# GregoryFaust/yaha

Hardware: AMD Instinct MI355X
Metric: aligned reads/s (whole node), 1 000 bp reads, OQC mode hot path (higher is better)
Workload: dtype int16

## Files before the change

yaha_amd/csrc/device/abi.hip:

```cpp
#include "ctx.h"
#include <memory>

std::atomic<int> gCtxPerDevice[64];
std::mutex gRowsMu[64];
hipEvent_t gRowsEv[64][4];
bool gRowsEvValid[64][4];
unsigned long long gRowsSeq[64];
std::atomic<int> gActiveRuns[64];
const char *const kStageNames[T_N] = {"seed_lookup", "hit_sort", "fragments_regions", "chain", "align_dp", "layout", "align_p1_gapfill", "ext_rows", "ext_trace",
                                      "align_p3_score_split", "ext_rows_device_clock", "ext_rows_packed16"};
thread_local const ygpu_ctx *tlsPfFailed = nullptr;

int runTo(ygpu_ctx *ctx, int stage)
{
    int rc;
    HIPCHK(hipSetDevice(ctx->device));
    if (ctx->stageDone < 1) {
        rc = stageSeed(ctx); if (rc) return rc;
        EV0(T_FRAGS); rc = buildFrags(ctx);
        if (rc == YD_RESORT) { rc = stageSeed(ctx); if (rc) return rc; EV0(T_FRAGS); rc = buildFrags(ctx);
            if (rc == YD_RESORT) { ctx->err = "hit sort: the sorted keys are not in ascending order"; rc = YGPU_EINTERNAL; } }
        if (rc) return rc;
        if (!ctx->nFrags) EV1(T_FRAGS);
        ctx->stageDone = 1;
    }
    if (stage >= 2 && ctx->stageDone < 2) { if (ctx->nFrags) { rc = stageChain(ctx); if (rc) return rc; } ctx->stageDone = 2; }
    if (stage >= 3 && ctx->stageDone < 3) { rc = stageAlign(ctx); if (rc) return rc; ctx->stageDone = 3; }
    uint32_t scanFail = 0; rc = fetchU32(ctx, ctx->counters.as<uint32_t>() + CNT_SCANFAIL, &scanFail); if (rc) return rc;
    if (scanFail) { if (ctx->scanState.p) HIPCHK(hipMemsetAsync(ctx->scanState.p, 0, ctx->scanState.cap, ctx->stream));
        ctx->err = "exclusive sum: a tile was not published within 30 s (look-back gave up)"; return YGPU_EINTERNAL; }
    return 0;
}
static int initCommon(ygpu_ctx *ctx, int device)
{
    const bool phases = getenv("YGPU_INIT_PHASES") != nullptr; double tPh = nowMs();
    auto phase = [&](const char *what) { if (phases) { const double t = nowMs(); fprintf(stderr, "[ygpu] ctx %p: %-20s %8.1f ms\n", (void *)ctx, what, t - tPh); tPh = t; } };
    HIPCHK(hipSetDevice(device));
    HIPCHK(hipStreamCreate(&ctx->stream)); HIPCHK(hipStreamCreate(&ctx->stream2));
    phase("two streams");
    for (int i = 0; i < YD_MAX_CHUNK_EV; i++) HIPCHK(hipEventCreateWithFlags(&ctx->evChunk[i], hipEventDisableTiming));
    HIPCHK(hipEventCreateWithFlags(&ctx->evTail, hipEventDisableTiming));
    if (const char *e = getenv("YGPU_LANE_CHUNKS")) ctx->laneChunks = atoi(e);
    if (const char *e = getenv("YGPU_TRACE_BUDGET_BLOCKS")) ctx->traceBudgetBlocks = atoll(e);
    ctx->segSortMax = ydSegSortMax();
    if (const char *e = getenv("YGPU_SEGSORT_MAX")) { long v = atol(e); if (v >= 1 && v <= (long)ydSegSortMax()) ctx->segSortMax = (uint32_t)v; }
    if (const char *e = getenv("YGPU_SPLIT_LANES")) ctx->splitLanes = atoi(e);
    if (const char *e = getenv("YGPU_ROWS2_PER_CU")) ctx->rows2PerCU = atoi(e);
    if (const char *e = getenv("YGPU_ALIGN_WAVES")) ctx->alignWavesPerCU = atoi(e);
    gCtxPerDevice[device & 63]++; ctx->counted = true;
    { int cu = 0; if (hipDeviceGetAttribute(&cu, hipDeviceAttributeMultiprocessorCount, device) != hipSuccess) { cu = 0; (void)hipGetLastError(); } ctx->nCU = cu > 0 ? cu : 256; }
    phase("device attribute");
    for (int t = 0; t < T_N; t++) { HIPCHK(hipEventCreate(&ctx->ev[t][0])); HIPCHK(hipEventCreate(&ctx->ev[t][1])); ctx->names[t] = kStageNames[t]; }
    if (hipEventCreateWithFlags(&ctx->evSync, hipEventBlockingSync | hipEventDisableTiming) != hipSuccess) { ctx->evSync = nullptr; (void)hipGetLastError(); }
    phase("events");
    if (hipHostMalloc((void **)&ctx->pinned, 256, hipHostMallocDefault) != hipSuccess) { ctx->pinned = nullptr; (void)hipGetLastError(); }
    ctx->pf.stream = ctx->stream2; ctx->pf.device = device;
    if (hipHostMalloc((void **)&ctx->pf.pinned, 256, hipHostMallocDefault) != hipSuccess) { ctx->pf.pinned = nullptr; (void)hipGetLastError(); }
    if (hipEventCreateWithFlags(&ctx->pf.evSync, hipEventBlockingSync | hipEventDisableTiming) != hipSuccess) { ctx->pf.evSync = nullptr; (void)hipGetLastError(); }
    HIPCHK(hipEventCreateWithFlags(&ctx->evSnap, hipEventDisableTiming));
    if (hipHostMalloc((void **)&ctx->snapCtr, sizeof(DevCounters), hipHostMallocDefault) != hipSuccess) { ctx->snapCtr = nullptr; (void)hipGetLastError(); }
    if (ctx->pf.counters.ensure(4 * CNT_N)) { ctx->err = "hipMalloc failed"; return YGPU_ENOMEM; }
    HIPCHK(hipMemsetAsync(ctx->pf.counters.p, 0, 4 * CNT_N, ctx->stream2));
    phase("pinned words");
    return 0;
}


namespace {
struct ImagePiece { size_t part; size_t off, bytes; };
struct ImagePlan {
    const char *src[3]; size_t bytes[3]; std::vector<ImagePiece> pieces;
    void build(const ygpu_index_view *ix, size_t pieceBytes)
    {
        const uint64_t HT = 1ull << (2 * ix->wordLen);
        src[0] = (const char *)ix->bases; bytes[0] = (size_t)ix->n_base_bytes; src[1] = (const char *)ix->startingOffs; bytes[1] = (size_t)(4 * (HT + 1));
            src[2] = (const char *)ix->ROA; bytes[2] = (size_t)(4ull * ix->totalMatches);
        for (size_t part = 0; part < 3; part++) for (size_t o = 0; o < bytes[part]; o += pieceBytes) pieces.push_back({part, o, std::min(pieceBytes, bytes[part] - o)});
    }
};
struct ImageState {
    std::unique_ptr<std::atomic<int>[]> done; std::atomic<int> failed{0}; char *dst[3] = {nullptr, nullptr, nullptr};
};

static void uploadFromHost(int device, const ImagePlan &plan, ImageState &me, int nt, bool staged)
{
    std::atomic<size_t> next(0);
    auto work = [&]() {
        if (hipSetDevice(device) != hipSuccess) { me.failed = 1; return; }
        hipStream_t st; if (hipStreamCreate(&st) != hipSuccess) { me.failed = 1; return; }
        char *buf[2] = {nullptr, nullptr}; hipEvent_t ev[2] = {nullptr, nullptr}; bool used[2] = {false, false}; size_t pend[2] = {0, 0}; size_t maxPiece = 0;
            for (auto &q : plan.pieces) maxPiece = std::max(maxPiece, q.bytes);
        if (staged) for (int k = 0; k < 2; k++) {
            if (hipHostMalloc((void **)&buf[k], maxPiece, hipHostMallocDefault) != hipSuccess) { buf[k] = nullptr; me.failed = 1; }
            if (hipEventCreateWithFlags(&ev[k], hipEventDisableTiming) != hipSuccess) { ev[k] = nullptr; me.failed = 1; }
        }
        for (int k = 0; !me.failed; k ^= 1) {
            const size_t i = next.fetch_add(1); if (i >= plan.pieces.size()) break;
            if (me.done[i].load(std::memory_order_acquire)) continue;
            const ImagePiece &q = plan.pieces[i]; char *d = me.dst[q.part] + q.off; const char *sp = plan.src[q.part] + q.off;
// ... 161 lines not shown
    std::vector<int> srcIndex(n, -1); const bool peer = !(getenv("YGPU_PEER_COPY") && atoi(getenv("YGPU_PEER_COPY")) == 0);
    for (int k = 1; k < n && peer; k++) {
        int can = devices[k] == devices[k - 1] ? 1 : 0;
        if (!can && hipDeviceCanAccessPeer(&can, devices[k], devices[k - 1]) != hipSuccess) { can = 0; (void)hipGetLastError(); }
        if (can && devices[k] != devices[k - 1]) { if (hipSetDevice(devices[k]) == hipSuccess) { const hipError_t e = hipDeviceEnablePeerAccess(devices[k - 1], 0);
            if (e != hipSuccess && e != hipErrorPeerAccessAlreadyEnabled) can = 0; } else can = 0; (void)hipGetLastError(); }
        if (can) srcIndex[k] = k - 1;
    }
    if (getenv("YGPU_INIT_PHASES")) { fprintf(stderr, "[ygpu] init: image sources:");
        for (int k = 0; k < n; k++) { if (srcIndex[k] < 0) fprintf(stderr, " device %d <- host;", devices[k]);
        else fprintf(stderr, " device %d <- device %d;", devices[k], devices[srcIndex[k]]); } fprintf(stderr, " %zu pieces\n", plan.pieces.size()); }
    std::vector<std::thread> th;
    for (int k = 1; k < n; k++) th.emplace_back([&, k]() { rcs[k] = initDevice(out[k], devices[k], srcIndex[k], srcIndex[k] >= 0 ? devices[srcIndex[k]] : -1, ix, plan,
        states.data(), k, ready.get(), all + k * cpd + 1, cpd - 1); });
    rcs[0] = initDevice(out[0], devices[0], -1, -1, ix, plan, states.data(), 0, ready.get(), all + 1, cpd - 1);
    for (auto &x : th) x.join();
    int rc = 0; for (int k = 0; k < n; k++) { if (rc_each) rc_each[k] = rcs[k]; if (rcs[k] && !rc) rc = rcs[k];
        if (rcs[k]) for (int j = 1; j < cpd; j++) if (all[k * cpd + j]->err.empty()) all[k * cpd + j]->err = "the device's first context failed: " + out[k]->err; }
    return rc;
}

int ygpu_device_count(void) { int n = 0; if (hipGetDeviceCount(&n) != hipSuccess) { (void)hipGetLastError(); return 0; } return n; }

int ygpu_init(int device, const ygpu_index_view *ix, const ygpu_params *p, ygpu_ctx **out)
{
    if (!out) return YGPU_EINVAL;
    return ygpu_init_multi(&device, 1, 1, ix, p, out, nullptr);
}

int ygpu_clone(const ygpu_ctx *parent, ygpu_ctx **out)
{
    *out = nullptr;
    if (!parent || !parent->stream) return YGPU_EINVAL;
    ygpu_ctx *ctx = new ygpu_ctx; *out = ctx; ctx->device = parent->device;
    int rc = initCommon(ctx, parent->device); if (rc) return rc;
    shareImage(ctx, parent);
    ENSURE(ctx->counters, 4 * CNT_N); ENSURE(ctx->ctr, sizeof(DevCounters)); ENSURE(ctx->errFlag, 64);
    HIPCHK(hipMemsetAsync(ctx->counters.p, 0, 4 * CNT_N, ctx->stream));
    HIPCHK(streamSync(ctx));
    return 0;
}

}
std::vector<DevBuf *> allBuffers(ygpu_ctx *ctx)
{
    DevBuf *all[] = {&ctx->dBases, &ctx->dSO, &ctx->dROA, &ctx->dLow, &ctx->dFwd, &ctx->dRev, &ctx->dFwd4, &ctx->dRev4, &ctx->dReadOff, &ctx->dKmerOff, &ctx->posS, &ctx->posC,
        &ctx->posRsI, &ctx->hitOff, &ctx->expandStart, &ctx->keysA, &ctx->keysB, &ctx->segOff, &ctx->bigB, &ctx->bigE, &ctx->isHead, &ctx->tileState,
                         &ctx->frags, &ctx->regStart, &ctx->multiList, &ctx->smallList, &ctx->bigList, &ctx->regionCount, &ctx->regionBase, &ctx->clumps, &ctx->clumpFrags,
                             &ctx->clumpFrags0, &ctx->order, &ctx->clumpsSorted, &ctx->rootPush, &ctx->rootBase, &ctx->outClumps,
                         &ctx->outClumps2, &ctx->outOps, &ctx->outRoot, &ctx->outPush, &ctx->dstIdx, &ctx->readCount, &ctx->readStart, &ctx->counters, &ctx->ctr, &ctx->errFlag,
                             &ctx->scanState, &ctx->bucketWork, &ctx->scratchAlign,
                         &ctx->segLists, &ctx->subB, &ctx->subE, &ctx->subLists, &ctx->subBigB, &ctx->subBigE, &ctx->sub2B, &ctx->sub2E, &ctx->sub2Lists, &ctx->sub3B, &ctx->sub3E,
                             &ctx->sub3Lists, &ctx->kmerParts, &ctx->scratchChain, &ctx->dpProbs, &ctx->dpRes, &ctx->dpOps, &ctx->rootState, &ctx->stateOps, &ctx->extProbs,
                             &ctx->rowsBound, &ctx->stripOff, &ctx->extRes, &ctx->extTrace, &ctx->chunkCnt, &ctx->memoKeys, &ctx->memoCount, &ctx->probs2, &ctx->rowsBound2,
                             &ctx->stripOff2, &ctx->extRes2, &ctx->extTrace2, &ctx->rowsClock, &ctx->splitScratch, &ctx->fallList, &ctx->keys2a, &ctx->keys2b, &ctx->vals2a,
                             &ctx->vals2b, &ctx->extKeys, &ctx->extVals, &ctx->extKeys2, &ctx->extOrder, &ctx->slowList, &ctx->gapScratch, &ctx->jointCount, &ctx->jointBase,
                             &ctx->joints, &ctx->sortKeys, &ctx->sortVals, &ctx->sortKeys2, &ctx->sortVals2, &ctx->gapOps, &ctx->waveChunks, &ctx->extOps, &ctx->traceCnt,
                         &ctx->oqCs, &ctx->oqCl, &ctx->oqOpsIn, &ctx->oqSeeds, &ctx->oqQlen, &ctx->pf.scanState, &ctx->pf.counters, &ctx->oqProf, &ctx->oqLists, &ctx->oqClsCnt,
                             &ctx->oqThr, &ctx->oqSeqStart, &ctx->oqSeqLen, &ctx->oqNeed, &ctx->oqPoolOff, &ctx->oqKeys, &ctx->oqStack, &ctx->oqNodes, &ctx->oqPrim, &ctx->oqPA,
                             &ctx->oqPfx, &ctx->oqPath, &ctx->oqPool, &ctx->oqPush, &ctx->oqOut, &ctx->oqOutCnt, &ctx->oqOutOps, &ctx->oqPrimCnt, &ctx->oqOutStart,
                             &ctx->oqOpsStart, &ctx->oqFClumps, &ctx->oqFOps};
    return std::vector<DevBuf *>(all, all + sizeof all / sizeof all[0]);
}
extern "C" {

void ygpu_destroy(ygpu_ctx *ctx)
{
    if (!ctx) return;
    if (ctx->worker.joinable()) { { std::lock_guard<std::mutex> lk(ctx->aMu); ctx->aQuit = true; } ctx->aCv.notify_all(); ctx->worker.join(); }
    if (ctx->counted) gCtxPerDevice[ctx->device & 63]--;
    if (ctx->stream) {
        hipSetDevice(ctx->device);
        {
            const int dv = ctx->device & 63; std::lock_guard<std::mutex> lk(gRowsMu[dv]);
            (void)hipStreamSynchronize(ctx->stream);
            if (gCtxPerDevice[dv].load() <= 0) for (int k = 0; k < 4; k++) if (gRowsEvValid[dv][k]) { (void)hipEventDestroy(gRowsEv[dv][k]); gRowsEvValid[dv][k] = false; }
        }
        if (ctx->sharedIndex) { ctx->dBases.p = nullptr; ctx->dBases.cap = 0; ctx->dSO.p = nullptr; ctx->dSO.cap = 0; ctx->dROA.p = nullptr; ctx->dROA.cap = 0;
            ctx->dLow.p = nullptr; ctx->dLow.cap = 0; }
        const std::vector<DevBuf *> all = allBuffers(ctx);
        for (auto b : all) b->release();
        for (int t = 0; t < T_N; t++) { hipEventDestroy(ctx->ev[t][0]); hipEventDestroy(ctx->ev[t][1]); }
        if (ctx->evSync) hipEventDestroy(ctx->evSync);
        if (ctx->pinned) hipHostFree(ctx->pinned);
        if (ctx->pf.pinned) hipHostFree(ctx->pf.pinned);
        if (ctx->snapCtr) hipHostFree(ctx->snapCtr);
        if (ctx->pf.evSync) hipEventDestroy(ctx->pf.evSync);
        if (ctx->evSnap) hipEventDestroy(ctx->evSnap);
        for (int i = 0; i < YD_MAX_CHUNK_EV; i++) hipEventDestroy(ctx->evChunk[i]);
        hipEventDestroy(ctx->evTail); hipStreamDestroy(ctx->stream2);
        hipStreamDestroy(ctx->stream);
    }
    delete ctx;
}
int ygpu_memory(ygpu_ctx *ctx, uint64_t *free_bytes, uint64_t *total_bytes, uint64_t *ctx_bytes)
{
    if (!ctx || !ctx->stream) return YGPU_EINVAL;
    HIPCHK(hipSetDevice(ctx->device));
    size_t fb = 0, tb = 0; HIPCHK(hipMemGetInfo(&fb, &tb));
    uint64_t mine = 0; for (DevBuf *b : allBuffers(ctx)) if (b->p && !(ctx->sharedIndex && (b == &ctx->dBases || b == &ctx->dSO || b == &ctx->dROA
        || b == &ctx->dLow))) mine += b->cap;
    if (free_bytes) *free_bytes = fb; if (total_bytes) *total_bytes = tb; if (ctx_bytes) *ctx_bytes = mine;
    return 0;
}
int ygpu_park(ygpu_ctx *ctx)
{
    if (!ctx || !ctx->stream) return YGPU_EINVAL;
    HIPCHK(hipSetDevice(ctx->device)); HIPCHK(streamSync(ctx));
    for (DevBuf *b : allBuffers(ctx)) if (b != &ctx->dBases && b != &ctx->dSO && b != &ctx->dROA && b != &ctx->dLow) b->release();
    if (ctx->counted) { gCtxPerDevice[ctx->device & 63]--; ctx->counted = false; }
    ctx->stageDone = 0; ctx->parked = true;
    return 0;
}
int ygpu_get_arena_profile(ygpu_ctx *ctx, ygpu_arena_profile *out)
{
    if (!ctx || !ctx->stream || !out) return YGPU_EINVAL;
    memset(out, 0, sizeof *out);
    const std::vector<DevBuf *> all = allBuffers(ctx);
    if (all.size() > sizeof out->cap / sizeof out->cap[0]) { ctx->err = "arena profile: more buffers than the profile holds"; return YGPU_EINTERNAL; }
    out->n = (uint32_t)all.size();
    for (size_t k = 0; k < all.size(); k++) { DevBuf *b = all[k];
        out->cap[k] = (b == &ctx->dBases || b == &ctx->dSO || b == &ctx->dROA || b == &ctx->dLow) ? 0ull : (uint64_t)b->cap; }
    out->trace_ratio = ctx->traceRatio; out->ops_ratio = ctx->opsRatio; out->last_clump_slots = ctx->lastClumpSlots; out->last_fall = ctx->lastFall; out->bases = ctx->totalBases;
    return 0;
}
int ygpu_presize(ygpu_ctx *ctx, const ygpu_arena_profile *prof)
{
    if (!ctx || !ctx->stream || !prof) return YGPU_EINVAL;
    if (ctx->parked) { ctx->err = "the context was parked (ygpu_park)"; return YGPU_EINVAL; }
    HIPCHK(hipSetDevice(ctx->device));
    const std::vector<DevBuf *> all = allBuffers(ctx);
    if (prof->n != all.size()) { ctx->err = "arena profile of another build"; return YGPU_EINVAL; }
    for (size_t k = 0; k < all.size(); k++) {
        DevBuf *b = all[k];
        if (b == &ctx->dBases || b == &ctx->dSO || b == &ctx->dROA || b == &ctx->dLow || b == &ctx->counters || b == &ctx->ctr || b == &ctx->errFlag
            || b == &ctx->pf.counters) continue;
        if (prof->cap[k] > b->cap && b->ensureExact((size_t)prof->cap[k])) { (void)hipGetLastError(); ctx->err = "hipMalloc failed while presizing the arenas"; return YGPU_ENOMEM;
            }
    }
    if (ctx->scanState.p) HIPCHK(hipMemsetAsync(ctx->scanState.p, 0, ctx->scanState.cap, ctx->stream));
    if (ctx->bucketWork.p) HIPCHK(hipMemsetAsync(ctx->bucketWork.p, 0, ctx->bucketWork.cap, ctx->stream));
    if (ctx->pf.scanState.p) HIPCHK(hipMemsetAsync(ctx->pf.scanState.p, 0, ctx->pf.scanState.cap, ctx->stream));
    if (ctx->runsDone == 0) { ctx->traceRatio = prof->trace_ratio; ctx->opsRatio = prof->ops_ratio > 0 ? prof->ops_ratio : ctx->opsRatio;
        ctx->lastClumpSlots = prof->last_clump_slots; ctx->lastFall = (long long)prof->last_fall; }
    HIPCHK(streamSync(ctx));
    return 0;
}
const char *ygpu_last_error(const ygpu_ctx *ctx) { return !ctx ? "null context" : (tlsPfFailed == ctx && !ctx->pf.err.empty()) ? ctx->pf.err.c_str() : ctx->err.c_str(); }

}
extern "C" {

int ygpu_run(ygpu_ctx *ctx)
{
    if (!ctx || !ctx->stream) return YGPU_EINVAL;
    ctx->stageDone = 0; const double t0 = nowMs(); ctx->statAttempts = 0; ctx->statRanges = 0;
    struct Active { int d; explicit Active(int dv) : d(dv) { gActiveRuns[d]++; } ~Active() { gActiveRuns[d]--; } } active(ctx->device & 63);
    int rc = runTo(ctx, 3);
    if (kStats) { size_t fb = 0, tb = 0; hipMemGetInfo(&fb, &tb);
        fprintf(stderr, "[ygpu] ctx %p run: %u reads, rc %d, %.1f ms; align attempts %d, ranges %d, trace arena %.2f GB (ratio %.3f), free %.1f GB\n", (void *)ctx, ctx->nReads, rc,
        nowMs() - t0, ctx->statAttempts, ctx->statRanges, ctx->extTrace.cap / 1e9, ctx->traceRatio, fb / 1e9); }
    if (rc) { (void)hipStreamSynchronize(ctx->stream); (void)hipGetLastError(); return rc; }
    if (ydCheckStateOn()) {
        if (getenv("YGPU_CHECK_STATE_INJECT") && ctx->scanState.p) (void)hipMemsetAsync((char *)ctx->scanState.p + 8, 0x01, 4, ctx->stream);
        const DevBuf *const bufs[2] = {&ctx->scanState, &ctx->bucketWork}; static const char *const names[2] = {"the sums' look-back state", "the orderings' bucket counters"};
        rc = ydCheckZero(ctx->stream, ctx->err, (unsigned int *)ctx->errFlag.p + 2, bufs, names, 2, "after ygpu_run");
        if (rc) { if (ctx->scanState.p) (void)hipMemsetAsync(ctx->scanState.p, 0, ctx->scanState.cap, ctx->stream); return rc; }
    }
    ctx->runsDone++;
    ctx->totalMs = 0;
    for (int t = 0; t < T_N; t++) {
        float m = 0; ctx->ms[t] = (ctx->evUsed[t] && hipEventElapsedTime(&m, ctx->ev[t][0], ctx->ev[t][1]) == hipSuccess) ? m : 0;
        if (t == T_XROWS_DEV) ctx->ms[t] = (ctx->evUsed[T_XROWS] && ctx->hRowsClock[1] > ctx->hRowsClock[0] && ctx->hRowsClock[0] != ~0ull)
            ? (float)((double)(ctx->hRowsClock[1] - ctx->hRowsClock[0]) / 1.0e5) : 0;
        if (t == T_XROWS_PK) ctx->ms[t] = ctx->rowsPacked ? 1.0f : 0.0f;
        if (t < T_TOP) ctx->totalMs += ctx->ms[t];
    }
    return 0;
}
void *ygpu_host_alloc(size_t bytes)
{
    void *p = nullptr;
    if (hipHostMalloc(&p, bytes ? bytes : 1, hipHostMallocDefault) != hipSuccess) { (void)hipGetLastError(); return nullptr; }
    return p;
}
void ygpu_host_free(void *p) { if (p) (void)hipHostFree(p); }
static void asyncWorker(ygpu_ctx *ctx)
{
    std::unique_lock<std::mutex> lk(ctx->aMu);
    for (;;) {
        ctx->aCv.wait(lk, [&] { return ctx->aQuit || (ctx->aOpen && !ctx->aDone && ctx->aBatch); });
        if (ctx->aQuit) return;
        const ygpu_read_batch *b = ctx->aBatch; ctx->aBatch = nullptr;
        lk.unlock();
        int rc = ygpu_upload(ctx, b); if (rc == 0) rc = ygpu_run(ctx); if (rc == 0) rc = ygpu_collect(ctx, &ctx->aOut);
        lk.lock();
        ctx->aRc = rc; ctx->aDone = true; ctx->aCv.notify_all();
    }
}
int ygpu_submit(ygpu_ctx *ctx, const ygpu_read_batch *batch, ygpu_ticket *ticket)
{
    if (!ctx || !ctx->stream || !batch || !ticket) return YGPU_EINVAL;
    std::unique_lock<std::mutex> lk(ctx->aMu);
    if (ctx->aOpen) return YGPU_EBUSY;
    if (!ctx->worker.joinable()) ctx->worker = std::thread(asyncWorker, ctx);
    ctx->aBatch = batch; ctx->aOpen = true; ctx->aDone = false; ctx->aRc = 0; *ticket = ++ctx->aTicket;
    ctx->aCv.notify_all();
    return 0;
}
int ygpu_poll(ygpu_ctx *ctx, ygpu_ticket ticket)
{
    if (!ctx) return YGPU_EINVAL;
    std::lock_guard<std::mutex> lk(ctx->aMu);
    if (!ctx->aOpen || ticket != ctx->aTicket) return YGPU_EINVAL;
    return ctx->aDone ? 1 : 0;
}
int ygpu_wait(ygpu_ctx *ctx, ygpu_ticket ticket, ygpu_result_batch *out)
{
    if (!ctx || !out) return YGPU_EINVAL;
    std::unique_lock<std::mutex> lk(ctx->aMu);
    if (!ctx->aOpen || ctx->aWaiting || ticket != ctx->aTicket) return YGPU_EINVAL;
    ctx->aWaiting = true;
    ctx->aCv.wait(lk, [&] { return ctx->aDone; });
    ctx->aOpen = false; ctx->aWaiting = false; *out = ctx->aOut;
    return ctx->aRc;
}

int ygpu_last_timing(ygpu_ctx *ctx, float *total_ms, int *n_stages, const char *const **names, const float **ms)
// ... 49 lines not shown
```

yaha_amd/csrc/device/ctx.h:

```cpp
#pragma once
#include <hip/hip_runtime.h>
#include <string>
#include <vector>
#include <cstring>
#include <cstdio>
#include <cstdlib>
#include <algorithm>
#include <array>
#include <atomic>
#include <chrono>
#include <thread>
#include <mutex>
#include <condition_variable>
#include <memory>
#include "common.h"
#include "../oqc_core.h"

#define HIPCHK(call) do { hipError_t e_ = (call); \
    if (e_ != hipSuccess) { ctx->err = std::string(#call) + ": " + hipGetErrorString(e_); return YGPU_ENODEV; } } while (0)

#define KL(kern, grid, block, shmem, st, ...) do { hipLaunchKernelGGL(kern, grid, block, shmem, st, __VA_ARGS__); hipError_t e_ = hipGetLastError(); \
    if (e_ != hipSuccess) { ctx->err = std::string("launch of " #kern " failed: ") + hipGetErrorString(e_); return YGPU_ENODEV; } } while (0)

#define YD_MAX_CHUNK_EV 16

struct DevBuf {
    void *p = nullptr;
    size_t cap = 0;
    int ensure(size_t bytes, bool keep = false, hipStream_t st = 0)
    {
        if (bytes <= cap) return 0;
        size_t ncap = bytes + bytes / 4 + 256; void *np = nullptr;
        if (hipMalloc(&np, ncap) != hipSuccess) return -1;
        if (keep && p && cap) { hipMemcpyAsync(np, p, cap, hipMemcpyDeviceToDevice, st); hipStreamSynchronize(st); }
        if (p) hipFree(p);
        p = np; cap = ncap; return 0;
    }
    void release() { if (p) hipFree(p); p = nullptr; cap = 0; }
    int ensureExact(size_t bytes)
    {
        if (bytes <= cap) return 0;
        release();
        void *np = nullptr;
        if (hipMalloc(&np, bytes) != hipSuccess) return -1;
        p = np; cap = bytes; return 0;
    }
    template <class T> T *as() const { return (T *)p; }
};

enum {
    CNT_NMULTI = 0, CNT_MAXN, CNT_CLUMPS, CNT_CFRAGS, CNT_QCHAIN, CNT_QALIGN, CNT_OUTCLUMPS, CNT_OUTOPS, CNT_QDP, CNT_DPOPS, CNT_NBIG, CNT_QBIG,
    CNT_STATEOPS, CNT_EXTOPS, CNT_QEXT, CNT_SLOW, CNT_NDP, CNT_NDP16, CNT_GAPOPS, CNT_PAD_EVEN, CNT_NMULTI2 ,
        CNT_NTINY, CNT_NSMALL, CNT_NMID, CNT_NB12, CNT_NB16,
        CNT_NB24,
    CNT_SEGC,
    CNT_NFRAGS = CNT_SEGC + 16,
    CNT_NREG = CNT_NFRAGS + 3,
    CNT_SCANFAIL = CNT_NREG + 2,
    CNT_N = CNT_NREG + 4
};
enum { T_SEED = 0, T_SORT, T_FRAGS, T_CHAIN, T_ALIGN, T_LAYOUT, T_TOP, T_P1 = T_TOP, T_XROWS, T_XTRACE, T_P3, T_XROWS_DEV, T_XROWS_PK, T_N };

extern std::atomic<int> gCtxPerDevice[64];
extern std::mutex gRowsMu[64];
extern hipEvent_t gRowsEv[64][4];
extern bool gRowsEvValid[64][4];
extern unsigned long long gRowsSeq[64];
extern std::atomic<int> gActiveRuns[64];
extern const char *const kStageNames[T_N];

struct PfSide {
    std::string err;
    hipStream_t stream = nullptr;
    uint32_t *pinned = nullptr;
    hipEvent_t evSync = nullptr;
    DevBuf scanState, counters;
    int device = 0;
};

struct DepthImage {
    int device = 0;
    DevBuf cov, stats, seqStart, seqLength, binBase;
    uint64_t nBins = 0;
    uint32_t bin = 0, minMapq = 0;
    std::vector<uint32_t> hSeqStart, hSeqLength;
    ~DepthImage() { (void)hipSetDevice(device); cov.release(); stats.release(); seqStart.release(); seqLength.release(); binBase.release(); }
};

struct EventsImage {
    int device = 0;
    DevBuf ev, stats, seqStart, seqLength, binBase;
    uint64_t nBins = 0;
    uint32_t bin = 0, minMapq = 0, minClip = 0;
    std::vector<uint32_t> hSeqStart, hSeqLength;
    ~EventsImage() { (void)hipSetDevice(device); ev.release(); stats.release(); seqStart.release(); seqLength.release(); binBase.release(); }
};

struct ygpu_ctx {
    int device = 0;
    hipStream_t stream = nullptr;
    DevParams P{};
    std::string err;
    int nCU = 256;
    DevBuf dBases, dSO, dROA, dLow;
    bool sharedIndex = false;
    uint32_t nReads = 0;
    int maxQ = 0;
    uint64_t totalBases = 0;
    uint32_t nKmers = 0;
    std::vector<uint32_t> hReadOff, hKmerOff;
    DevBuf dFwd, dRev, dFwd4, dRev4, dReadOff, dKmerOff;
    DevBuf bigB, bigE;
    DevBuf posS, posC, posRsI, hitOff, expandStart, keysA, keysB, segOff, isHead, tileState, frags;
    DevBuf segLists, subB, subE, subLists, subBigB, subBigE, sub2B, sub2E, sub2Lists, sub3B, sub3E, sub3Lists, kmerParts;
    DevBuf regStart, multiList, smallList, bigList, regionCount, regionBase;
    DevBuf clumps, clumpFrags, clumpFrags0, order, clumpsSorted, scratchChain;
    DevBuf rootPush, rootBase, outClumps, outClumps2, outOps, outRoot, outPush, dstIdx, readCount, readStart;
    DevBuf scratchAlign, dpProbs, dpRes, dpOps;
    DevBuf rootState, stateOps, extProbs, rowsBound, stripOff, extRes, extTrace, chunkCnt;
    DevBuf memoKeys, memoCount, probs2, rowsBound2, stripOff2, extRes2, extTrace2, splitScratch, fallList;
    DevBuf keys2a, keys2b, vals2a, vals2b, extKeys, extVals, extKeys2, extOrder, slowList;
    DevBuf gapScratch, jointCount, jointBase, joints, sortKeys, sortVals, sortKeys2, sortVals2, gapOps;
    DevBuf waveChunks, extOps, traceCnt, rowsClock;
    DevBuf counters, ctr, errFlag, scanState, bucketWork;
    bool evUsed[16] = {false};
    double traceT = 0;
    hipStream_t stream2 = nullptr;
    hipEvent_t evChunk[YD_MAX_CHUNK_EV], evTail;
    bool counted = false;
    bool parked = false;
    long long traceBudgetBlocks = 0;
    uint32_t lastClumpSlots = 0;
    bool keepAllFrags = false;
    unsigned long long hRowsClock[2] = {0, 0};
    int laneChunks = 0;
    uint32_t segSortMax = 0;
    int splitLanes = 1;
    int rows2PerCU = 0;
    int alignWavesPerCU = 0;
    int laneExt = 1;
    std::vector<unsigned long long> hStripOff;
    int runsDone = 0;
    double traceRatio = 0.0, opsRatio = 0.03;
    int statRanges = 0, statAttempts = 0;
    double statT0 = 0;
    DevBuf oqProf, oqLists, oqClsCnt, oqThr, oqSeqStart, oqSeqLen, oqNeed, oqPoolOff, oqKeys, oqStack, oqNodes, oqPrim, oqPA, oqPfx, oqPath, oqPool;
    DevBuf oqPush, oqOut, oqOutCnt, oqOutOps, oqPrimCnt, oqOutStart, oqOpsStart, oqFClumps, oqFOps;
    bool oqSet = false, oqDone = false;
    yoqc::Params oqP{};
    yoqc::Seqs oqG{};
    uint32_t nFOut = 0, nFOps = 0;
    PfSide pf;
    std::atomic<bool> pfSnap{false};
    hipEvent_t evSnap = nullptr;
    uint32_t snapN = 0, snapC = 0, snapOps = 0, pfN = 0;
    unsigned long long runGen = 0, snapGen = 0, filtGen = 0;
    ygpu_counters pfCounters{};
    DevCounters *snapCtr = nullptr;
    DevCounters snapCtrPlain{};
    unsigned long long snapHits = 0, snapFrags = 0, snapRegions = 0;
    DevBuf oqCs, oqCl, oqOpsIn, oqSeeds, oqQlen;
    std::shared_ptr<DepthImage> depth;
    std::shared_ptr<EventsImage> events;
    uint32_t hOutCounts[2] = {0, 0}, hOutEf = 0;
    bool hOutValid = false;
    uint32_t nHits = 0, nFrags = 0, nRegions = 0, nMulti = 0, nTiny = 0, nSmall = 0, nMid = 0, nBig = 0, maxN = 0;
    int sortRankUsed = 0;
    bool sortRankForced = false;
    uint32_t nClumpSlots = 0, nClumps = 0, nClumpFrags = 0, nOut = 0, nOutOps = 0;
    int stageDone = 0;
    std::vector<uint32_t> hClumpStart, hOps, hClumpFragStart, hClumpRS, hDpOps;
    std::vector<ygpu_clump> hClumps;
// ... 99 lines not shown
```

yaha_amd/csrc/device/ext_lanes.h:

```cpp
#pragma once
#include "align.h"

#define YD_REFILL_MIN 4
#define YD_LW 21
#define YD_LWORST (-(1 << 28))
#define YD_CHUNK_FLUSHES 16
#define YD_LANE_DWORDS (YD_CHUNK_FLUSHES * 32)
#define YD_CHUNK_DWORDS (64 * YD_LANE_DWORDS)
#define YD_LDS_STRIDE 33

typedef uint32_t yd_u32x4 __attribute__((ext_vector_type(4)));
struct ExtProb { uint32_t qBase, rOff; uint16_t qOff, qLen; uint32_t flags; };
enum { XP_STRAND = 1, XP_REV = 2, XP_VALID = 4 };
struct ExtRes { int score, maxi, maxj; uint32_t opsOff, nOps, where, rows, cells; };
static_assert(sizeof(ExtProb) == 16 && sizeof(ExtRes) == 32, "k_ext_rows_pk moves these as 16-byte vectors (non-temporal loads / stores)");
__device__ __forceinline__ const uint32_t *extOpsPtr(const uint32_t *traceBase, const ExtRes &r) {
    return traceBase + (long long)(((unsigned long long)r.where << 32) | (unsigned long long)r.opsOff); }

struct ExtArgs {
    DevParams P; const uint8_t *bases; const uint8_t *fwd, *rev;
    const uint8_t *fwd4, *rev4;
    const ExtProb *probs; uint32_t nProb;
    const uint32_t *order;
    unsigned long long *clock;
    uint32_t *trace; uint32_t nChunks;
    unsigned int *chunkCount;
    uint32_t *waveChunks; uint32_t maxCh;
    uint32_t *ops; unsigned int *opsCount; uint32_t opsCap;
    ExtRes *res; unsigned int *queue; DevCounters *ctr;
    int *errFlag; int dbgMode;
};
enum { YERR_TRACEMEM = 9 };

template <bool CAPS, bool SECOND>
__global__ void __launch_bounds__(256) __attribute__((amdgpu_waves_per_eu(CAPS ? 2 : 3, CAPS ? 2 : 3))) k_ext_rows(ExtArgs A)
{
    __shared__ uint32_t sBlk[256 * YD_LDS_STRIDE];
    if (!SECOND && A.clock && threadIdx.x == 0) atomicMin(&A.clock[0], (unsigned long long)wall_clock64());
    const int lane = laneId();
    const int GO = A.P.GO, GE = A.P.GE, GOE = A.P.GO + A.P.GE, XC = A.P.X, maxIntron = A.P.maxIntron, maxGap = A.P.maxGap;
    const int MSG = A.P.MS + GOE, RCG = GOE - A.P.RC, LWG = YD_LWORST - GOE;
    constexpr int bandwidth = YD_LBAND, leftR = YD_LBAND;
    const uint32_t maxROff = A.P.maxROff;
    YD_GLOBAL const uint8_t *gBases = toGlobal(A.bases);
    const unsigned long long lanesBelow = (1ull << lane) - 1ull;
    const unsigned wave = blockIdx.x * 4u + (threadIdx.x >> 6);
    uint32_t *const myBlk = &sBlk[threadIdx.x * YD_LDS_STRIDE];

    int PV[YD_LW], PF[YD_LW], PI[YD_LW];
    uint32_t w0 = 0, w1 = 0, w2 = 0;
    int p = -1, i = 0, qLen = 0, rLen = 0, maxScore = YD_LWORST, maxi = 0, maxj = 0, qStep = 0, qcNext = 0;
    uint32_t rOff = 0; bool rev = false, done = false;
    YD_GLOBAL const uint8_t *q = toGlobal(A.fwd);
    unsigned calls = 0, rows = 0, cells = 0;
#pragma unroll
    for (int j = 0; j < YD_LW; j++) { PV[j] = LWG; PF[j] = YD_LWORST; PI[j] = 0; }

    int poolCount = 0, poolNext = 0; bool exhausted = false;
    uint32_t eLens = 0, eROff = 0, eQ = 0, eMisc = 0, eW1 = 0, eW2 = 0, ePidx = 0;
    bool pendFlush = false; int pendRes = -1; unsigned pStart = 0;
    auto storeResult = [&]() {
        const unsigned m = i < leftR ? (unsigned)i : (unsigned)leftR, nCells = (unsigned)YD_LW * (unsigned)i - ((unsigned)(leftR + 1) * m - m * (m + 1u) / 2u);
        rows += (unsigned)i; cells += nCells;
        ExtRes r; r.score = maxScore > 0 ? maxScore : 0; r.maxi = maxi; r.maxj = maxj; r.opsOff = pStart >> 4; r.nOps = 0;
        r.where = (pStart & 15u) | ((uint32_t)lane << 4) | (wave << 10); r.rows = (unsigned)i; r.cells = nCells;
        A.res[pendRes] = r; pendRes = -1; i = 0;
    };
    int wslot = 0; unsigned flush = 0; bool dirty = false, justDone = false;
    YD_GLOBAL uint32_t *chunkPtr = toGlobal(A.trace); bool noMem = false;
    auto takeChunk = [&]() {
        unsigned c = 0;
        if (lane == 0) c = atomicAdd(A.chunkCount, 1u);
        c = uniU(c);
        const unsigned ci = flush / YD_CHUNK_FLUSHES;
        if (c >= A.nChunks || ci >= A.maxCh) { noMem = true; c = 0; if (lane == 0) atomicCAS(A.errFlag, 0, (int)YERR_TRACEMEM); }
        if (lane == 0 && ci < A.maxCh) A.waveChunks[(size_t)wave * A.maxCh + ci] = c;
        chunkPtr = toGlobal(A.trace) + (size_t)c * YD_CHUNK_DWORDS;
    };
    takeChunk();
    auto flushBlocks = [&]() {
        const unsigned long long f = __ballot(pendFlush);
        pendFlush = false;
// ... 126 lines not shown
        if (rv > maxScore) { maxScore = rv; maxi = i; maxj = rj; }
        const uint32_t nb = nbOdd == 2u ? 15u : (nbOdd ? (nbByte & 15u) : (nbByte >> 4));
        w0 = (w0 >> 4) | (w1 << 28); w1 = (w1 >> 4) | (w2 << 28); w2 = (w2 >> 4) | (nb << 16);
        const bool fin = busy && (rv < maxScore - XC || i >= qLen);
        if (busy) dirty = true;
        if (wslot == 9) { pendFlush = dirty; dirty = false; wslot = 0; } else wslot++;
        justDone = fin;
        if (fin) { pendRes = p; p = -1; qStep = 0; rLen = 0; qLen = 0; }
    }
    if (wslot != 0 && dirty) pendFlush = true;
    if (!noMem && __ballot(pendFlush) != 0ull) { flushBlocks(); nextFlush(); }
    if (pendRes >= 0) storeResult();
    if (!SECOND && A.clock && lane == 0) atomicMax(&A.clock[1], (unsigned long long)wall_clock64());
    unsigned c0 = (unsigned)waveSumI((int)calls), c1 = (unsigned)waveSumI((int)rows);
    unsigned long long cc = cells;
#pragma unroll
    for (int d = 32; d >= 1; d >>= 1) { cc += (unsigned long long)__shfl_xor((long long)cc, d, 64); }
    if (lane == 0 && !SECOND && A.ctr) {
        unsigned long long *c = A.ctr->v;
        atomicAdd(&c[C_EXT_CALLS], (unsigned long long)c0); atomicAdd(&c[C_EXT_ROWS], (unsigned long long)c1); atomicAdd(&c[C_EXT_CELLS], cc);
        atomicAdd(&c[C_TOUCHED], (unsigned long long)c1 + (unsigned long long)c0 * (unsigned long long)(4 * A.P.bandWidth + 1));
    }
}

struct ExtRowBits { uint32_t a, b, c; };
__device__ __forceinline__ uint32_t extNib(const ExtRowBits &r, int x) { const uint32_t w = x < 8 ? r.a : (x < 16 ? r.b : r.c); return (w >> ((x & 7) * 4)) & 15u; }

__device__ unsigned int gTraceDbg[8];
struct ExtStrip {
    YD_GLOBAL uint32_t *arena; YD_GLOBAL const uint32_t *tab; unsigned f0, laneOff; int cIdx; YD_GLOBAL uint32_t *cBase; int limit; bool wild;
    __device__ __forceinline__ YD_GLOBAL uint32_t *at(int d)
    {
        if ((unsigned)d >= (unsigned)limit) { wild = true; d = 0; }
        const unsigned f = f0 + (unsigned)(d >> 5); const int ci = (int)(f / YD_CHUNK_FLUSHES);
        if (ci != cIdx) { cIdx = ci; cBase = arena + (size_t)tab[ci] * YD_CHUNK_DWORDS + laneOff; }
        return cBase + (f % YD_CHUNK_FLUSHES) * 32u + (unsigned)(d & 31);
    }
};

__device__ __forceinline__ int extRowWord(int y) { return ((y - 1) / 10) * 32 + ((y - 1) % 10) * 3; }
#define YD_TRACE_DEPTH 8
__global__ void __launch_bounds__(256) k_ext_trace(ExtArgs A)
{
    YD_HIGH_PRIO();
    const uint32_t t = blockIdx.x * blockDim.x + threadIdx.x; const int lane = laneId();
    if (*toGlobal(A.errFlag) != 0) return;
    const bool live = t < A.nProb;
    const uint32_t p = live ? ((A.order && !(A.dbgMode & 2)) ? A.order[t] : t) : 0u;
    ExtRes r; r.score = 0; r.nOps = 0;
    if (live) r = A.res[p];
    const bool walk = live && r.score > 0;
    constexpr int leftR = YD_LBAND;
    int n = 0; bool bad = false; int E = 0;
    ExtStrip S; S.arena = toGlobal(A.trace); S.cIdx = -1; S.cBase = S.arena; S.f0 = 0; S.laneOff = 0; S.tab = toGlobal(A.waveChunks); S.limit = 0; S.wild = false;
    if (walk) {
        const int ph = (int)(r.where & 15u);
        S.f0 = r.opsOff; S.laneOff = ((r.where >> 4) & 63u) * YD_LANE_DWORDS; S.tab = toGlobal(A.waveChunks) + (size_t)(r.where >> 10) * A.maxCh;
        E = extRowWord(r.maxi + 1 + ph) + 3; S.limit = E;
        int y = r.maxi, x = r.maxj, prev = -1, acc = 0;
        struct Cur { YD_GLOBAL uint32_t *cp; int rr, w; unsigned fb; };
        Cur c; c.rr = (y - 1 + ph) % 10; c.w = ((y - 1 + ph) / 10) * 32 + c.rr * 3; c.fb = S.f0 + (unsigned)((y - 1 + ph) / 10); c.cp = S.at(c.w);
        auto stepUp = [&](Cur &u) {
            if (u.rr != 0) { u.rr--; u.w -= 3; u.cp -= 3; return; }
            u.rr = 9; u.w -= 5; u.fb--;
            if (u.fb % YD_CHUNK_FLUSHES == YD_CHUNK_FLUSHES - 1u) u.cp = S.arena + (size_t)S.tab[u.fb / YD_CHUNK_FLUSHES] * YD_CHUNK_DWORDS + S.laneOff + (YD_CHUNK_FLUSHES - 1u) *
                32u + 27u;
            else u.cp -= 5;
        };
        const int row0w = extRowWord(1 + ph) - 3;
        auto flush = [&]() { const int wp = E - 1 - n; if (wp < c.w + 3) bad = true; else *S.at(wp) = opMake(prev, acc); n++; };
        auto put = [&](int code, int len) { if (prev != code) { if (prev >= 0) flush(); prev = code; acc = len; } else acc += len; };
        for (int guard = 0; guard < 70000 && y > 0 && x >= 0 && x < YD_LW; guard++) {
            const int ws = x >> 3, sh = (x & 7) * 4;
            uint32_t d[YD_TRACE_DEPTH];
            int lim = (int)(c.fb % YD_CHUNK_FLUSHES) * 10 + c.rr + 1; lim = lim < y ? lim : y; lim = lim < YD_TRACE_DEPTH ? lim : YD_TRACE_DEPTH;
            { YD_GLOBAL uint32_t *up = c.cp; int ur = c.rr;
#pragma unroll
              for (int k = 0; k < YD_TRACE_DEPTH; k++) { d[k] = up[ws]; const bool go = k + 1 < lim; const int dec = ur == 0 ? 5 : 3; up -= go ? dec : 0;
                  ur = go ? (ur == 0 ? 9 : ur - 1) : ur; } }
            uint32_t nib = (d[0] >> sh) & 15u; int took = 0;
#pragma unroll
            for (int k = 0; k < YD_TRACE_DEPTH; k++) {
                if (k >= lim) break;
                nib = (d[k] >> sh) & 15u;
                const int op = (int)(nib & 3u);
                if (op >= OP_D || y <= 0) break;
                if (prev != op) { if (prev >= 0) flush(); prev = op; acc = 1; } else acc++;
                y--; took++;
                if (took < lim) { const int dec = c.rr == 0 ? 5 : 3; c.cp -= dec; c.w -= dec; c.fb -= c.rr == 0 ? 1u : 0u; c.rr = c.rr == 0 ? 9 : c.rr - 1; }
            }
            if (took == lim) { if (y > 0) stepUp(c); else c.w = row0w; continue; }
            if ((nib & 3u) == (uint32_t)OP_D) {
                ExtRowBits rb; rb.a = c.cp[0]; rb.b = c.cp[1]; rb.c = c.cp[2];
                int run = 1, xx = x;
                while (extNib(rb, xx) & 4u) { xx--; if (xx < 0) break; run++; }
                put(OP_D, run); x -= run;
            } else {
                int run = 1, yy = y, xx = x; Cur u = c; uint32_t nb2 = nib;
                while (nb2 & 8u) {
                    yy--; xx++; if (yy <= 0 || xx >= YD_LW) break;
                    run++; stepUp(u);
                    nb2 = (u.cp[xx >> 3] >> ((xx & 7) * 4)) & 15u;
                }
                put(OP_I, run); y -= run; x += run;
                if (y > 0) { for (int k = 0; k < run; k++) stepUp(c); } else c.w = row0w;
            }
        }
        if (y <= 0 && x > leftR) put(OP_D, x - leftR);
        if (prev >= 0) { const int wp = E - 1 - n; if (wp < 0) bad = true; else *S.at(wp) = opMake(prev, acc); n++; }
        if (bad || S.wild) { bad = true; atomicCAS(A.errFlag, 0, (int)YERR_TRACE); n = 0; if (S.wild && atomicCAS(&gTraceDbg[5], 0u, 1u) == 0u) { gTraceDbg[6] = p;
            gTraceDbg[7] = r.where; } }
    }
    if (A.dbgMode & 1) n = 0;
    const bool inPlace = walk && !bad && n > 0 && (S.f0 + (unsigned)((E - n) >> 5)) / YD_CHUNK_FLUSHES == (S.f0 + (unsigned)((E - 1) >> 5)) / YD_CHUNK_FLUSHES;
    const int nCopy = (walk && !bad && !inPlace) ? n : 0;
    int incl = nCopy;
#pragma unroll
    for (int d2 = 1; d2 < 64; d2 <<= 1) { const int v = __shfl_up(incl, d2, 64); if (lane >= d2) incl += v; }
    const int total = __shfl(incl, 63, 64); unsigned ob = 0;
    if (lane == 63 && total) ob = atomicAdd(A.opsCount, (unsigned)total);
    ob = (unsigned)__shfl((int)ob, 63, 64);
    if (walk && !bad) {
        long long place;
        if (inPlace) place = (long long)(S.at(E - n) - S.arena);
        else {
            const unsigned off = ob + (unsigned)(incl - nCopy);
            if ((unsigned long long)off + (unsigned)n > (unsigned long long)A.opsCap) { atomicCAS(A.errFlag, 0, (int)YERR_OUT); return; }
            YD_GLOBAL uint32_t *dst = toGlobal(A.ops) + off;
            for (int k0 = 0; k0 < n; k0 += 8) {
                uint32_t v[8];
#pragma unroll
                for (int j = 0; j < 8; j++) v[j] = (k0 + j < n) ? *S.at(E - n + k0 + j) : 0u;
#pragma unroll
                for (int j = 0; j < 8; j++) if (k0 + j < n) dst[k0 + j] = v[j];
            }
            place = (long long)(dst - S.arena);
        }
        r.opsOff = (uint32_t)(unsigned long long)place; r.where = (uint32_t)((unsigned long long)place >> 32); r.nOps = (uint32_t)n; A.res[p] = r;
    }
}

__global__ void k_trace_keys(const ExtRes *res, const uint32_t *order, uint32_t n, const uint32_t *waveChunks, uint32_t maxCh, int regionLog, int lenShift, int lenBits,
    uint32_t *keys, uint32_t *vals)
{
    YD_HIGH_PRIO();
    const uint32_t t = blockIdx.x * blockDim.x + threadIdx.x;
    if (t >= n) return;
    const uint32_t p = order ? order[t] : t;
    const ExtRes r = res[p];
    const uint32_t top = (1u << lenBits) - 1u;
    const uint32_t len = r.score > 0 ? min((uint32_t)r.maxi >> lenShift, top) : 0u;
    const uint32_t ci = r.opsOff / YD_CHUNK_FLUSHES;
    const uint32_t phys = (regionLog < 20 && r.score > 0 && ci < maxCh) ? waveChunks[(size_t)(r.where >> 10) * maxCh + ci] : 0u;
    keys[t] = (min(phys >> regionLog, 0xFFFFFFu) << lenBits) | (top - len);
    vals[t] = p;
}

__global__ void __launch_bounds__(256) k_trace_volume(const ExtRes *res, uint32_t n, unsigned long long *out)
{
    const uint32_t t = blockIdx.x * blockDim.x + threadIdx.x;
    unsigned long long w = 0, v = 0, np = 0, nw = 0;
    if (t < n) { const ExtRes r = res[t]; if (r.rows) { w = r.rows + 1ull; np = 1; if (r.score > 0) { v = (unsigned long long)r.maxi + 1ull; nw = 1; } } }
#pragma unroll
    for (int d = 32; d >= 1; d >>= 1) {
        w += (unsigned long long)__shfl_xor((long long)w, d, 64); v += (unsigned long long)__shfl_xor((long long)v, d, 64);
        np += (unsigned long long)__shfl_xor((long long)np, d, 64); nw += (unsigned long long)__shfl_xor((long long)nw, d, 64);
    }
    if ((threadIdx.x & 63u) == 0u && np) { atomicAdd(&out[0], w); atomicAdd(&out[1], v); atomicAdd(&out[2], np); atomicAdd(&out[3], nw); }
}

__global__ void k_rebase_u32(uint32_t *v, uint32_t n, uint32_t sub)
{
    YD_HIGH_PRIO();
    const uint32_t i = blockIdx.x * blockDim.x + threadIdx.x;
    if (i < n) v[i] -= sub;
}

__global__ void k_prob_keys(const ExtProb *probs, uint32_t n, uint32_t *keys, uint32_t *vals)
{
    YD_HIGH_PRIO();
    const uint32_t p = blockIdx.x * blockDim.x + threadIdx.x;
    if (p < n) { keys[p] = (probs[p].flags & XP_VALID) ? 0xFFFFu - probs[p].qLen : 0xFFFFu; vals[p] = p; }
}
```

yaha_amd/csrc/device/ext_lanes_pk.h:

```cpp
#pragma once
#include "ext_lanes.h"

typedef short yd_s16x2 __attribute__((ext_vector_type(2)));
#define YD_LW16 (-16000)
#define YD_NP 11
#define YD_RCREAL 0x7FF0u

__device__ __forceinline__ yd_s16x2 pkS(uint32_t v) { return __builtin_bit_cast(yd_s16x2, v); }
__device__ __forceinline__ uint32_t pkU(yd_s16x2 v) { return __builtin_bit_cast(uint32_t, v); }
__device__ __forceinline__ uint32_t pkAdd(uint32_t a, uint32_t b) { return pkU(__builtin_elementwise_add_sat(pkS(a), pkS(b))); }
__device__ __forceinline__ uint32_t pkSub(uint32_t a, uint32_t b) { return pkU(__builtin_elementwise_sub_sat(pkS(a), pkS(b))); }
__device__ __forceinline__ uint32_t pkMax(uint32_t a, uint32_t b) { return pkU(__builtin_elementwise_max(pkS(a), pkS(b))); }
__device__ __forceinline__ uint32_t pkMin(uint32_t a, uint32_t b) { return pkU(__builtin_elementwise_min(pkS(a), pkS(b))); }
__device__ __forceinline__ uint32_t pkMinU(uint32_t a, uint32_t b) { uint32_t d; asm("v_pk_min_u16 %0, %1, %2" : "=v"(d) : "v"(a), "v"(b)); return d; }
__device__ __forceinline__ uint32_t pkMad(uint32_t a, uint32_t b, uint32_t c) { uint32_t d; asm("v_pk_mad_i16 %0, %1, %2, %3" : "=v"(d) : "v"(a), "v"(b), "v"(c)); return d; }
__device__ __forceinline__ uint32_t pkSignMask(uint32_t a) { return pkU(pkS(a) >> (yd_s16x2)(15)); }
__device__ __forceinline__ uint32_t pkSignMaskAsm(uint32_t a, uint32_t c15) { uint32_t d; asm("v_pk_ashrrev_i16 %0, %1, %2" : "=v"(d) : "v"(c15), "v"(a)); return d; }
__device__ __forceinline__ uint32_t bfi(uint32_t mask, uint32_t a, uint32_t b) { return (a & mask) | (b & ~mask); }
__device__ __forceinline__ uint32_t pk2(int v) { return ((uint32_t)v & 0xFFFFu) * 0x10001u; }

#ifndef YD_ROWS_LDSWIN
#define YD_ROWS_LDSWIN 0
#endif
#ifndef YD_ROWS_RESBATCH
// ... 343 lines not shown
        if (fin) { pendRes = p; p = -1; rowsFin = row; }
#ifdef YD_PROF
        if (__ballot(snap) != 0ull) pfSnap++; pfBusy += (unsigned)__builtin_popcountll(__ballot(busy));
#endif
    }
    if (wslot != 0 && dirty) pendFlush = true;
    { const unsigned long long f = __ballot(pendFlush); if (!noMem && f != 0ull) { flushBlocks(f, chunkPtr + (size_t)(flush % YD_CHUNK_FLUSHES) * 32u); nextFlush(); } }
    if (!SECOND && A.clock && lane == 0) atomicMax(&A.clock[1], (unsigned long long)wall_clock64());
    unsigned c0 = calls, c1 = (unsigned)waveSumI((int)rows);
    unsigned long long cc = cells;
#pragma unroll
    for (int d = 32; d >= 1; d >>= 1) { cc += (unsigned long long)__shfl_xor((long long)cc, d, 64); }
#ifdef YD_PROF
    if (lane == 0 && !SECOND) { const unsigned v[7] = {pfPass, pfRes, pfRefill, pfSnap, pfBusy, pfFlush, pfPool};
        for (int k = 0; k < 7; k++) atomicAdd(&gRowsProf[k], (unsigned long long)v[k]); }
#endif
    if (lane == 0 && !SECOND && A.ctr) {
        unsigned long long *c = A.ctr->v;
        atomicAdd(&c[C_EXT_CALLS], (unsigned long long)c0); atomicAdd(&c[C_EXT_ROWS], (unsigned long long)c1); atomicAdd(&c[C_EXT_CELLS], cc);
        atomicAdd(&c[C_TOUCHED], (unsigned long long)c1 + (unsigned long long)c0 * (unsigned long long)(4 * A.P.bandWidth + 1));
    }
}

struct PkRec { uint32_t a, m, ab2, b; };
__device__ __forceinline__ PkRec pkLoadRec(YD_GLOBAL const uint32_t *cp) { const yd_u32x4 v = *(YD_GLOBAL const yd_u32x4 *)cp; PkRec r; r.ab2 = v.x; r.m = v.y; r.a = v.z;
    r.b = v.w; return r; }
__device__ __forceinline__ int pkRecWord(int n) { return ((n - 1) >> 3) * 32 + ((n - 1) & 7) * 4; }
__device__ __forceinline__ bool pkContE(const PkRec &r, int k, int h) { const uint32_t d = k < 8 ? r.b : r.ab2; const int bit = k < 8 ? k : k - 6;
    return ((d >> (8 * h + bit)) & 1u) == 0u; }
__device__ __forceinline__ bool pkContF(const PkRec &r, int k, int h) { const uint32_t d = k < 8 ? r.b : r.ab2; const int bit = k < 8 ? k : k - 6;
    return ((d >> (16 + 8 * h + bit)) & 1u) == 0u; }
#define YD_TSTRIDE 36
#ifndef YD_TRACE_SWZ
#define YD_TRACE_SWZ 0
#endif
#define YD_TSWZ(problem) (YD_TRACE_SWZ ? (((problem) >> 3) & 3) : 0)
#ifndef YD_TRACE_BS
#define YD_TRACE_BS 256
#endif
__global__ void __launch_bounds__(YD_TRACE_BS) k_ext_trace_pk(ExtArgs A)
{
    YD_HIGH_PRIO();
    __shared__ uint32_t sBlkT[YD_TRACE_BS / 64][64 * YD_TSTRIDE];
    const uint32_t t = blockIdx.x * blockDim.x + threadIdx.x; const int lane = laneId();
    uint32_t *const wBlk = sBlkT[threadIdx.x >> 6]; const uint32_t *const myRec = wBlk + lane * YD_TSTRIDE;
    if (*toGlobal(A.errFlag) != 0) return;
    const bool live = t < A.nProb;
    const uint32_t p = live ? ((A.order && !(A.dbgMode & 2)) ? A.order[t] : t) : 0u;
    ExtRes r; r.score = 0; r.nOps = 0;
    if (live) r = A.res[p];
    const bool walk = live && r.score > 0;
    constexpr int leftR = YD_LBAND;
    int n = 0; bool bad = false; int E = 0;
    ExtStrip S; S.arena = toGlobal(A.trace); S.cIdx = -1; S.cBase = S.arena; S.f0 = 0; S.laneOff = 0; S.tab = toGlobal(A.waveChunks); S.limit = 0; S.wild = false;
    struct Cur { YD_GLOBAL uint32_t *cp; int rr, w; unsigned fb; };
    int y = 0, x = 0, prev = -1, acc = 0, row0w = 0;
    Cur u; u.cp = S.arena; u.rr = 0; u.w = 0; u.fb = 0;
    if (walk) {
        const int ph = (int)(r.where & 15u);
        S.f0 = r.opsOff; S.laneOff = ((r.where >> 4) & 63u) * YD_LANE_DWORDS; S.tab = toGlobal(A.waveChunks) + (size_t)(r.where >> 10) * A.maxCh;
        E = pkRecWord(r.maxi + 2 + ph) + 4; S.limit = E;
        y = r.maxi; x = r.maxj;
        { const int idx = y + (x >= YD_NP ? 1 : 0) - 1 + ph; u.rr = idx & 7; u.w = (idx >> 3) * 32 + u.rr * 4; u.fb = S.f0 + (unsigned)(idx >> 3); u.cp = S.at(u.w); }
        row0w = pkRecWord(1 + ph) - 4;
    }
    {
        auto stepUp = [&](Cur &c) {
            c.w -= 4;
            if (c.rr != 0) { c.rr--; c.cp -= 4; return; }
            c.rr = 7; c.fb--;
            if (c.fb % YD_CHUNK_FLUSHES == YD_CHUNK_FLUSHES - 1u) c.cp = S.arena + (size_t)S.tab[c.fb / YD_CHUNK_FLUSHES] * YD_CHUNK_DWORDS + S.laneOff + (YD_CHUNK_FLUSHES - 1u) *
                32u + 28u;
            else c.cp -= 4;
        };
        auto flush = [&]() { const int wp = E - 1 - n; if (wp < u.w + 8) bad = true; else *S.at(wp) = opMake(prev, acc); n++; };
        auto put = [&](int code, int len) { if (prev != code) { if (prev >= 0) flush(); prev = code; acc = len; } else acc += len; };
#ifdef YD_PROF
        unsigned tpPass = 0, tpAct = 0, tpRounds = 0, tpFlushR = 0, tpDel = 0, tpIns = 0, tpRows = 0; const bool tpWalks = __ballot(walk) != 0ull;
#endif
        for (int guard = 0;; guard++) {
            const bool act = walk && guard < 70000 && y > 0 && x >= 0 && x < YD_LW;
            if (__ballot(act) == 0ull) break;
#ifdef YD_PROF
            tpPass++; tpAct += (unsigned)__builtin_popcountll(__ballot(act));
#endif
            {
                const unsigned long long myBase = (unsigned long long)(act ? u.cp - u.rr * 4 : S.arena);
#pragma unroll
                for (int g = 0; g < 8; g++) {
                    const int src = g * 8 + (lane >> 3);
                    const unsigned long long b = ((unsigned long long)(uint32_t)__shfl((int)(uint32_t)(myBase >> 32), src, 64) << 32) | (uint32_t)__shfl((int)(uint32_t)myBase, src,
                        64);
                    const yd_u32x4 v = *(YD_GLOBAL const yd_u32x4 *)((YD_GLOBAL const uint32_t *)b + (lane & 7) * 4);
                    yd_u32x4 sw; { const uint32_t c[4] = {v.x, v.y, v.z, v.w}; constexpr int z = YD_TRACE_SWZ ? 3 : 0; sw.x = c[(0 ^ g) & z]; sw.y = c[1 ^ (g & z)];
                        sw.z = c[2 ^ (g & z)]; sw.w = c[3 ^ (g & z)]; }
                    *(yd_u32x4 *)(wBlk + src * YD_TSTRIDE + (lane & 7) * 4) = sw;
                }
                __builtin_amdgcn_wave_barrier();
            }
            if (!act) continue;
            const int rr0 = u.rr;
            const int swz = YD_TSWZ(lane);
            auto blkRec = [&](int slot, YD_GLOBAL const uint32_t *cp) -> PkRec {
                if (slot >= 0) { const uint32_t *q = myRec + slot * 4; PkRec r2; r2.ab2 = q[0 ^ swz]; r2.m = q[1 ^ swz]; r2.a = q[2 ^ swz]; r2.b = q[3 ^ swz]; return r2; }
                return pkLoadRec(cp);
            };
            const int h = x >= YD_NP ? 1 : 0, k = x - YD_NP * h;
            const int second = k < 8 ? 0 : 1, bt = k < 8 ? k : k - 3, sT = 8 * h + bt, sU = 16 + sT, sM = 16 * h + 10 - k;
            int lim = u.rr + 1; lim = lim < y ? lim : y;
            uint32_t diag = 0u, mis = 0u;
            const int iTU = (second ? 0 : 2) ^ swz, iM = 1 ^ swz;
#pragma unroll
            for (int d = 0; d < YD_TRACE_DEPTH; d++) {
                const int sl = rr0 - d < 0 ? 0 : rr0 - d;
                const uint32_t tu = myRec[sl * 4 + iTU], mw = myRec[sl * 4 + iM];
                diag |= (((tu >> sT) & (tu >> sU)) & 1u) << d; mis |= ((mw >> sM) & 1u) << d;
            }
            const uint32_t inLim = (1u << lim) - 1u;
            const int took = __builtin_ctz(~diag | ~inLim);
            int op = 0;
            if (took < lim) { const int sl = rr0 - took; const uint32_t tu = myRec[sl * 4 + iTU]; op = ((tu >> sU) & 1u) == 0u ? OP_I : OP_D; }
            y -= took;
            if (took > 0) {
                const int mv = took < lim ? took : took - 1;
                u.cp -= 4 * mv; u.w -= 4 * mv; u.rr -= mv;
            }
            {
                const uint32_t m = mis & ((1u << took) - 1u); int pos = 0;
// ... 2 lines not shown
                    tpRounds++;
#endif
                    const uint32_t cur = (m >> pos) & 1u;
                    const uint32_t same = (cur ? ~m : m) >> pos;
                    const int g = __builtin_ctz(same | (1u << (took - pos)));
                    const int code = cur ? OP_R : OP_M;
                    if (prev != code) { if (prev >= 0) flush(); prev = code; acc = g; } else acc += g;
                    pos += g;
                }
            }
#ifdef YD_PROF
            tpRows += (unsigned)took;
            if (took != lim) { if (op == OP_D) tpDel++; else tpIns++; }
#endif
            if (took == lim) { if (y > 0) stepUp(u); else u.w = row0w; continue; }
            if (op == OP_D) {
                int sl = rr0 - took;
                PkRec rb = blkRec(sl, u.cp);
                int run = 1, xx = x, hh = h; Cur v = u;
                for (;;) {
                    if (!pkContE(rb, xx - YD_NP * hh, hh)) break;
                    xx--; if (xx < 0) break;
                    run++;
                    if (hh && xx < YD_NP) { hh = 0; stepUp(v); rb = blkRec(--sl, v.cp); }
                }
                put(OP_D, run); x -= run;
                if (h && x < YD_NP) stepUp(u);
            } else {
                int run = 1, yy = y, xx = x, hh = h; Cur v = u;
                int sl = rr0 - took;
                PkRec rb = blkRec(sl, v.cp);
                while (pkContF(rb, xx - YD_NP * hh, hh)) {
                    yy--; xx++; if (yy <= 0 || xx >= YD_LW) break;
                    run++;
                    if (!hh && xx >= YD_NP) hh = 1;
                    else { stepUp(v); rb = blkRec(--sl, v.cp); }
                }
                put(OP_I, run); y -= run; x += run;
                const int h2 = x >= YD_NP ? 1 : 0, steps = run - (h2 - h);
                if (y > 0) { for (int s = 0; s < steps; s++) stepUp(u); } else u.w = row0w;
            }
        }
#ifdef YD_PROF
        if (tpWalks) {
            const unsigned r4 = (unsigned)waveSumI((int)tpRounds), d4 = (unsigned)waveSumI((int)tpDel), i4 = (unsigned)waveSumI((int)tpIns), w4 = (unsigned)waveSumI((int)tpRows);
            if (lane == 0) { atomicAdd(&gTraceProf[0], 1ull); atomicAdd(&gTraceProf[1], (unsigned long long)tpPass); atomicAdd(&gTraceProf[2], (unsigned long long)tpAct);
                atomicAdd(&gTraceProf[3], (unsigned long long)r4); atomicAdd(&gTraceProf[5], (unsigned long long)d4); atomicAdd(&gTraceProf[6], (unsigned long long)i4);
                atomicAdd(&gTraceProf[7], (unsigned long long)w4); }
        }
        (void)tpFlushR;
#endif
        if (walk) {
        if (y <= 0 && x > leftR) put(OP_D, x - leftR);
        if (prev >= 0) { const int wp = E - 1 - n; if (wp < 0) bad = true; else *S.at(wp) = opMake(prev, acc); n++; }
        if (bad || S.wild) { bad = true; atomicCAS(A.errFlag, 0, (int)YERR_TRACE); n = 0; }
        }
    }
    if (A.dbgMode & 1) n = 0;
    const bool inPlace = walk && !bad && n > 0 && (S.f0 + (unsigned)((E - n) >> 5)) / YD_CHUNK_FLUSHES == (S.f0 + (unsigned)((E - 1) >> 5)) / YD_CHUNK_FLUSHES;
    const int nCopy = (walk && !bad && !inPlace) ? n : 0;
    int incl = nCopy;
#pragma unroll
    for (int d2 = 1; d2 < 64; d2 <<= 1) { const int v = __shfl_up(incl, d2, 64); if (lane >= d2) incl += v; }
    const int total = __shfl(incl, 63, 64); unsigned ob = 0;
    if (lane == 63 && total) ob = atomicAdd(A.opsCount, (unsigned)total);
    ob = (unsigned)__shfl((int)ob, 63, 64);
    if (walk && !bad) {
        long long place;
        if (inPlace) place = (long long)(S.at(E - n) - S.arena);
        else {
            const unsigned off = ob + (unsigned)(incl - nCopy);
            if ((unsigned long long)off + (unsigned)n > (unsigned long long)A.opsCap) { atomicCAS(A.errFlag, 0, (int)YERR_OUT); return; }
            YD_GLOBAL uint32_t *dst = toGlobal(A.ops) + off;
            for (int k0 = 0; k0 < n; k0 += 8) {
                uint32_t v[8];
#pragma unroll
                for (int j = 0; j < 8; j++) v[j] = (k0 + j < n) ? *S.at(E - n + k0 + j) : 0u;
#pragma unroll
                for (int j = 0; j < 8; j++) if (k0 + j < n) dst[k0 + j] = v[j];
            }
            place = (long long)(dst - S.arena);
        }
        r.opsOff = (uint32_t)(unsigned long long)place; r.where = (uint32_t)((unsigned long long)place >> 32); r.nOps = (uint32_t)n; A.res[p] = r;
    }
}
```

yaha_amd/csrc/device/phase_lanes.h:

```cpp
#pragma once
#include "ext_lanes.h"

struct RootState { uint32_t sro, listOff; int32_t score; uint16_t sqo, eqo, refLen, len; uint8_t status, pad[3]; uint32_t pad2[2]; };
enum { JK_NONE = 0, JK_D, JK_I, JK_R, JK_DIAG, JK_DP };
struct JointRec {
    uint32_t nsro, qBase; uint16_t nsqo, qGap, rGap; uint8_t kind, flags;
    uint32_t opsOff; uint16_t nOps, pad; int32_t score; uint32_t cells;
};
struct PhaseArgs {
    RootState *state; uint32_t *stateOps; unsigned int *stateOpsCount; uint32_t stateOpsCap;
    ExtProb *probs; unsigned long long *rowsBound;
    const ExtRes *res; const uint32_t *extOps;
    uint32_t *slowList; unsigned int *slowCount;
    int useList;
    uint32_t rootBegin;
    const uint32_t *p3Order;
    uint32_t *memoKeys; unsigned int *memoCount; ExtProb *probs2; unsigned long long *rowsBound2; unsigned int *nProb2; uint32_t probs2Cap;
    uint32_t *jointCount; const uint32_t *jointBase; JointRec *joints; uint32_t nJoints;
    uint32_t *sortKeys, *sortVals; const uint32_t *sortedVals; unsigned int *nDP, *nDPb; uint32_t band24;
    uint32_t *gapOps; unsigned int *gapOpsCount; uint32_t gapOpsCap;
    uint32_t *extKeys, *extVals;
    uint8_t *gapScratch;
};

__device__ __forceinline__ unsigned waveSumU(unsigned v) { return (unsigned)waveSumI((int)v); }
__device__ __forceinline__ unsigned waveReserve(unsigned long long mask, unsigned int *counter, int lane, unsigned each = 1u)
{
    if (!mask) return 0u;
    const int first = __builtin_ctzll(mask); unsigned base = 0;
    if (lane == first) base = atomicAdd(counter, each * (unsigned)__builtin_popcountll(mask));
    base = (unsigned)__builtin_amdgcn_readlane((int)base, first);
    return base + each * (unsigned)__builtin_popcountll(mask & ((1ull << lane) - 1ull));
}


template <int N> __device__ __forceinline__ void blockCounters(unsigned long long *const (&dst)[N], const unsigned (&val)[N])
{
    __shared__ unsigned sAcc[N];
    if (threadIdx.x < (unsigned)N) sAcc[threadIdx.x] = 0;
    __syncthreads();
    if (laneId() == 0) { for (int k = 0; k < N; k++) if (val[k]) atomicAdd(&sAcc[k], val[k]); }
    __syncthreads();
    if (threadIdx.x < (unsigned)N && sAcc[threadIdx.x]) atomicAdd(dst[threadIdx.x], (unsigned long long)sAcc[threadIdx.x]);
}

template <int N> __device__ __forceinline__ void blockCountersU32(unsigned int *const (&dst)[N], const unsigned (&val)[N])
{
    __shared__ unsigned sAcc32[N];
    if (threadIdx.x < (unsigned)N) sAcc32[threadIdx.x] = 0;
    __syncthreads();
    if (laneId() == 0) { for (int k = 0; k < N; k++) if (val[k]) atomicAdd(&sAcc32[k], val[k]); }
    __syncthreads();
    if (threadIdx.x < (unsigned)N && sAcc32[threadIdx.x]) atomicAdd(dst[threadIdx.x], sAcc32[threadIdx.x]);
}

__device__ __forceinline__ unsigned blockReserve(unsigned int *counter, unsigned waveTotal)
{
    __shared__ unsigned sTot[4], sBase;
    const int wv = (int)(threadIdx.x >> 6);
    if (laneId() == 0) sTot[wv] = waveTotal;
    __syncthreads();
    if (threadIdx.x == 0) { const unsigned t = sTot[0] + sTot[1] + sTot[2] + sTot[3]; sBase = t ? atomicAdd(counter, t) : 0u; }
    __syncthreads();
    unsigned b = sBase; for (int k = 0; k < wv; k++) b += sTot[k];
    return b;
}

#define YD_GROWS 60
#define YD_GREF 64
// ... 91 lines not shown
#undef GPV
#undef GPF
#undef GPI
    return V;
}

__global__ void k_joint_counts(AlignArgs A, PhaseArgs X)
{
    YD_HIGH_PRIO();
    const uint32_t r = blockIdx.x * blockDim.x + threadIdx.x;
    if (r < A.nRoots) X.jointCount[r] = YD_ROOT_REC(A, r).nFrags - 1u;
    if (r == A.nRoots) X.jointCount[r] = 0u;
}

typedef unsigned long long yd_u64u __attribute__((aligned(1)));
template <int DIR>
__device__ __forceinline__ int matchRun(YD_GLOBAL const uint8_t *q, int qi, YD_GLOBAL const uint8_t *gB, uint32_t ro, int maxLen)
{
    int m = 0;
    while (maxLen - m >= 8) {
        const int qa = DIR > 0 ? qi + m : qi - m - 7; const uint32_t ra = DIR > 0 ? ro + (uint32_t)m : ro - (uint32_t)m - 7u;
        unsigned long long qx = *(YD_GLOBAL const yd_u64u *)(q + qa);
        qx = (qx | (qx >> 4)) & 0x00FF00FF00FF00FFull; qx = (qx | (qx >> 8)) & 0x0000FFFF0000FFFFull;
        const uint32_t qs = (uint32_t)(qx | (qx >> 16));
        unsigned long long rx = *(YD_GLOBAL const yd_u64u *)(gB + (ra >> 1));
        rx = ((rx & 0x0F0F0F0F0F0F0F0Full) << 4) | ((rx >> 4) & 0x0F0F0F0F0F0F0F0Full);
        const uint32_t rs = (uint32_t)(rx >> (4u * (ra & 1u)));
        const uint32_t diff = qs ^ rs;
        if (diff) return m + (DIR > 0 ? (__builtin_ctz(diff) >> 2) : (__builtin_clz(diff) >> 2));
        m += 8;
    }
    for (; m < maxLen; m++) {
        const uint32_t off = DIR > 0 ? ro + (uint32_t)m : ro - (uint32_t)m; const uint32_t b = gB[off >> 1];
        if ((uint32_t)q[DIR > 0 ? qi + m : qi - m] != ((off & 1u) ? (b & 15u) : (b >> 4))) break;
    }
    return m;
}

#define YD_JKEY_NONE 0xFFFu
#define YD_JKEY_BITS 12
__host__ __device__ __forceinline__ uint32_t gapJointClass(uint32_t key) { return key >> 10; }
__host__ __device__ __forceinline__ uint32_t gapJointKey(const DevParams &P, bool banded, int qGap, int rGap)
{
    const int lenDiff = qGap > rGap ? qGap - rGap : rGap - qGap;
    const int W = banded ? 2 * P.bandWidth + lenDiff + 1 : rGap + 1;
    uint32_t cls = W <= 16 ? 2u : 3u;
    const bool lim = banded && P.bandWidth >= 5 && P.maxGap >= 16 && qGap <= YD_GROWS && rGap <= YD_GREF;
    if (lim && W <= 16) cls = W <= 12 ? 0u : 1u;
    uint32_t wf = (uint32_t)(W < 31 ? W : 31);
    if (cls == 3u) wf = (lim && W <= 24) ? (uint32_t)(W - 17) : 8u + (uint32_t)(W - 17 < 23 ? W - 17 : 23);
    return (cls << 10) | (wf << 5) | (uint32_t)((qGap >> 1) < 30 ? (qGap >> 1) : 30);
}
__host__ __device__ __forceinline__ bool gapJointBand24(uint32_t key) { return (key >> 10) == 3u && ((key >> 5) & 31u) < 8u; }

template <int BS = 256>
__device__ __forceinline__ uint32_t wgDeal(uint32_t root, uint32_t cls)
{
    __shared__ uint32_t sHist[65], sOrder[BS];
    const int lane = laneId();
    if (threadIdx.x < 65u) sHist[threadIdx.x] = 0u;
    __syncthreads();
    const uint32_t inCls = atomicAdd(&sHist[cls], 1u);
    __syncthreads();
    if (threadIdx.x < 64u) {
        const uint32_t c = sHist[lane]; uint32_t incl = c;
#pragma unroll
        for (int d = 1; d < 64; d <<= 1) { const uint32_t y = (uint32_t)__shfl_up((int)incl, d, 64); if (lane >= d) incl += y; }
        sHist[lane] = incl - c; if (lane == 63) sHist[64] = incl;
    }
    __syncthreads();
    sOrder[sHist[cls] + inCls] = cls < 64u ? root : 0xFFFFFFFFu;
    __syncthreads();
    return sOrder[threadIdx.x];
}

__global__ void __launch_bounds__(256) k_p1_joints(AlignArgs A, PhaseArgs X)
{
    YD_HIGH_PRIO();
    const uint32_t r = blockIdx.x * blockDim.x + threadIdx.x;
    const bool live = r < A.nRoots; const DevParams &P = A.P;
    unsigned perfect = 0, touched = 0, nDP = 0, nDP16 = 0, nB12 = 0, nB16 = 0, nB24 = 0;
    if (live) {
        const ChainClumpRec rec = YD_ROOT_REC(A, r); const int n = (int)rec.nFrags;
        if (n > 1) {
            const uint32_t read = rec.rs >> 1, r0 = A.B.readOff[read];
            YD_GLOBAL const uint8_t *q = toGlobal((rec.rs & 1u) ? A.B.rev : A.B.fwd) + r0; YD_GLOBAL const uint8_t *gB = toGlobal(A.bases);
            auto refAt = [&](uint32_t off) -> uint32_t { const uint32_t b = gB[off >> 1]; return (off & 1u) ? (b & 15u) : (b >> 4); };
            DevFrag *F = A.clumpFrags + rec.fragOff; const uint32_t jb = X.jointBase[r];
            DevFrag cur = F[0];
            for (int k = 1; k < n; k++) {
                DevFrag nxt = F[k];
                int gap = (int)min(gapI(cur.eqo, nxt.sqo), gapU(cur.sro + (uint32_t)cur.refLen - 1u, nxt.sro));
                { const int c = matchRun<-1>(q, (int)nxt.sqo - 1, gB, nxt.sro - 1u, gap);
                  perfect += c; touched += c + (c < gap);
                  if (c > 0) { nxt.sqo = (uint16_t)(nxt.sqo - c); nxt.sro -= (uint32_t)c; nxt.refLen = (uint16_t)(nxt.refLen + c); } gap -= c; }
                { const uint32_t eRO = cur.sro + (uint32_t)cur.refLen - 1u; const int c = matchRun<1>(q, (int)cur.eqo + 1, gB, eRO + 1u, gap);
                  perfect += c; touched += c + (c < gap);
                  if (c > 0) { cur.eqo = (uint16_t)(cur.eqo + c); cur.refLen = (uint16_t)(cur.refLen + c); } }
                F[k - 1] = cur;
                const uint32_t eRO = cur.sro + (uint32_t)cur.refLen - 1u;
                const int qGap = (int)(gapI(cur.eqo, nxt.sqo) & 0xFFFF), rGap = (int)(gapU(eRO, nxt.sro) & 0xFFFF);
                JointRec j; j.nsro = eRO + 1u; j.qBase = r0; j.nsqo = (uint16_t)((cur.eqo + 1) & 0xFFFF); j.qGap = (uint16_t)qGap; j.rGap = (uint16_t)rGap;
                j.flags = (uint8_t)(rec.rs & 1u); j.opsOff = 0; j.nOps = 0; j.pad = 0; j.score = 0; j.cells = 0; j.kind = JK_NONE;
                uint32_t key = YD_JKEY_NONE;
                if (qGap == 0 && rGap == 0) { }
                else if (qGap == 0) j.kind = JK_D;
                else if (rGap == 0) j.kind = JK_I;
                else if (rGap == 1 && qGap == 1) j.kind = JK_R;
                else {
                    const int lenDiff = qGap > rGap ? qGap - rGap : rGap - qGap;
                    const bool banded = lenDiff + P.bandWidth * 2 + 1 < rGap;
                    j.flags |= banded ? 2u : 0u; j.kind = JK_DP;
                    if (qGap == rGap) {
                        int mm = 0;
                        for (int t = 0; t < qGap; t++) mm += (uint32_t)q[(int)cur.eqo + 1 + t] != refAt(eRO + 1u + (uint32_t)t);
                        if (mm * (P.MS + P.RC) <= P.MS + 2 * (P.GO + P.GE)) { j.kind = JK_DIAG; j.score = P.MS * (qGap - mm) - P.RC * mm; }
                    }
                    if (j.kind == JK_DP) { key = gapJointKey(P, banded, qGap, rGap); const uint32_t cls = gapJointClass(key); nDP++; nDP16 += cls <= 2u; nB12 += cls == 0u;
                        nB16 += cls <= 1u; nB24 += gapJointBand24(key) ? 1u : 0u; }
                }
                X.joints[jb + (uint32_t)(k - 1)] = j; X.sortKeys[jb + (uint32_t)(k - 1)] = key; X.sortVals[jb + (uint32_t)(k - 1)] = jb + (uint32_t)(k - 1);
                cur = nxt;
            }
            F[n - 1] = cur;
        }
    }
    perfect = waveSumU(perfect); touched = waveSumU(touched); nDP = waveSumU(nDP); nDP16 = waveSumU(nDP16); nB12 = waveSumU(nB12); nB16 = waveSumU(nB16); nB24 = waveSumU(nB24);
// ... 47 lines not shown

__global__ void __launch_bounds__(64) k_gap_wave(AlignArgs A, PhaseArgs X)
{
    YD_HIGH_PRIO();
    const int lane = laneId();
    WaveMem M = carveScratch(A.scratch + (size_t)blockIdx.x * A.scratchPerWave, A.maxQ, A.traceRows, A.listCap, A.genCap);
    __shared__ uint16_t sTrace[YD_LDS_CELLS];
    int err = 0; WaveScratch S; S.ldsTrace = sTrace; S.trace = M.trace; S.traceRows = A.traceRows; S.tmpOps = M.tmpOps; S.tmpCap = 2 * A.maxQ + 512; S.gen = M.gen;
        S.genCap = A.genCap; S.err = &err;
    const unsigned n = uniU(*X.slowCount);
    for (;;) {
        if (__ballot(1) != ~0ull) { atomicCAS(A.errFlag, 0, (int)YERR_EXEC); break; }
        unsigned t = 0; if (lane == 0) t = atomicAdd(A.queueHead, 1u);
        const unsigned i = uniU(t);
        if (i >= n) break;
        const uint32_t ji = uniU(X.slowList[i]); const JointRec j = X.joints[ji];
        const uint8_t *q = ((j.flags & 1u) ? A.B.rev : A.B.fwd) + j.qBase;
        DPOut o = dpWave(A.P, A.bases, q, (j.flags & 2u) ? YGPU_DP_BANDED : YGPU_DP_FULL, j.nsro, (int)j.rGap, (int)j.nsqo, (int)j.qGap, S);
        if (UNI_B(err != 0)) { if (lane == 0) atomicCAS(A.errFlag, 0, err); break; }
        const int nT = uni(o.nOps); unsigned ob = 0;
        if (lane == 0) ob = atomicAdd(X.gapOpsCount, (unsigned)nT); ob = uniU(ob);
        if (UNI_B((unsigned long long)ob + (unsigned)nT > (unsigned long long)X.gapOpsCap)) { if (lane == 0) atomicCAS(A.errFlag, 0, (int)YERR_OUT); break; }
        for (int k = lane; k < nT; k += 64) X.gapOps[ob + k] = dpOp(S, o, false, k);
        if (lane == 0) { JointRec *jp = X.joints + ji; jp->opsOff = ob; jp->nOps = (uint16_t)nT; jp->score = uni(o.score); jp->cells = (uint32_t)uni(o.cells); }
    }
}

__global__ void __launch_bounds__(256) k_p1_assemble(AlignArgs A, PhaseArgs X)
{
    YD_HIGH_PRIO();
    const int lane = laneId(); const uint32_t r = blockIdx.x * blockDim.x + threadIdx.x;
    const bool live = r < A.nRoots; const DevParams &P = A.P;
    ChainClumpRec rec; rec.nFrags = 0; rec.rs = 0; rec.fragOff = 0;
    if (live) rec = YD_ROOT_REC(A, r);
    const int n = (int)rec.nFrags; const uint32_t jb = live ? X.jointBase[r] : 0u;
    unsigned want = 0;
    if (live) { want = (unsigned)n + 1u; for (int k = 0; k + 1 < n; k++) { const JointRec &j = X.joints[jb + (uint32_t)k];
        want += j.kind == JK_DP ? (unsigned)j.nOps : (j.kind == JK_DIAG ? (unsigned)j.qGap : (j.kind != JK_NONE ? 1u : 0u)); } }
    unsigned incl = want;
#pragma unroll
    for (int d = 1; d < 64; d <<= 1) { unsigned t = (unsigned)__shfl_up((int)incl, d, 64); if (lane >= d) incl += t; }
    const unsigned total = (unsigned)__shfl((int)incl, 63, 64);
    const unsigned base = blockReserve(X.stateOpsCount, total);
    const unsigned slot = base + incl - want;
    unsigned perfect = 0, touched = 0, gapCalls = 0, gapRows = 0, gapCells = 0;
    if (live) {
        if ((unsigned long long)slot + want > (unsigned long long)X.stateOpsCap) atomicCAS(A.errFlag, 0, (int)YERR_OUT);
        else {
            const uint32_t read = rec.rs >> 1, r0 = A.B.readOff[read]; const int qlen = (int)(A.B.readOff[read + 1] - r0);
            YD_GLOBAL const uint8_t *q = toGlobal((rec.rs & 1u) ? A.B.rev : A.B.fwd) + r0; YD_GLOBAL const uint8_t *gB = toGlobal(A.bases);
            auto refAt = [&](uint32_t off) -> uint32_t { const uint32_t b = gB[off >> 1]; return (off & 1u) ? (b & 15u) : (b >> 4); };
            const DevFrag *F = A.clumpFrags + rec.fragOff;
            uint32_t *ops = X.stateOps + slot; int nOut = 0, pc = -1, pl = 0, score = 0;
            auto put = [&](int code, int len) { if (pc == code) { pl = (pl + len) & 0xFFFF; return; } if (pc >= 0) { ops[nOut] = opMake(pc, pl); nOut++; } pc = code;
                pl = len & 0xFFFF; };
            const DevFrag firstF = F[0]; DevFrag cur = firstF;
            for (int k = 1; k <= n; k++) {
                { const int ql = fragQLen(cur.sqo, cur.eqo); put(OP_M, ql); score += P.MS * ql; }
                if (k == n) break;
                const JointRec j = X.joints[jb + (uint32_t)(k - 1)]; const int qGap = j.qGap, rGap = j.rGap;
                if (j.kind == JK_D) { put(OP_D, rGap); score -= P.GO + rGap * P.GE; }
                else if (j.kind == JK_I) { put(OP_I, qGap); score -= P.GO + qGap * P.GE; }
                else if (j.kind == JK_R) { put(OP_R, 1); score -= P.RC; }
                else if (j.kind == JK_DIAG) {
                    const int g = qGap;
                    for (int t = 0; t < g; t++) put((uint32_t)q[(int)j.nsqo + t] == refAt(j.nsro + (uint32_t)t) ? OP_M : OP_R, 1);
                    score += j.score; gapCalls++; gapRows += (unsigned)g; touched += (unsigned)g;
                    if (P.bandWidth * 2 + 1 < g) { const int bw = P.bandWidth, W = 2 * bw + 1; for (int i = 1; i <= g; i++) { int sc = bw + 1 - i; if (sc < 0) sc = 0;
                        int ec = bw + g - i; if (ec > W - 1) ec = W - 1; if (ec >= sc) gapCells += (unsigned)(ec - sc + 1); } }
                    else gapCells += (unsigned)(g * g);
                } else if (j.kind == JK_DP) {
                    for (int t = 0; t < (int)j.nOps; t++) { const uint32_t op = X.gapOps[j.opsOff + (uint32_t)t]; put(opCode(op), opLen(op)); }
                    score += j.score; gapCalls++; gapRows += (unsigned)qGap; gapCells += j.cells; touched += (unsigned)rGap;
                }
                cur = F[k];
            }
            uint32_t sro = firstF.sro; int sqo = firstF.sqo, eqo = cur.eqo; int refLen = (int)((1u + (cur.sro + (uint32_t)cur.refLen - 1u) - firstF.sro) & 0xFFFFu);
            int firstAdd = 0;
            int backLen = (int)((uint32_t)sqo < sro ? (uint32_t)sqo : sro), forwLen;
            if (backLen > 0) {
                const int m = matchRun<-1>(q, sqo - 1, gB, sro - 1u, backLen);
                perfect += m; touched += m + (m < backLen);
                if (m > 0) { firstAdd = m; score += m * P.MS; backLen -= m; sqo -= m; sro -= (uint32_t)m; refLen = (refLen + m) & 0xFFFF; }
            }
            {
                const uint32_t eRO = sro + (uint32_t)refLen - 1u;
                const uint32_t qrem = (uint32_t)(((qlen - 1) - eqo) & 0xFFFF), rrem = P.maxROff - eRO;
                forwLen = (int)(qrem < rrem ? qrem : rrem);
                if (forwLen > 0) {
                    const int m = matchRun<1>(q, eqo + 1, gB, eRO + 1u, forwLen);
                    perfect += m; touched += m + (m < forwLen);
                    if (m > 0) { pl = (pl + m) & 0xFFFF; score += m * P.MS; forwLen -= m; eqo += m; refLen = (refLen + m) & 0xFFFF; }
                }
            }
            if (nOut == 0) pl = (pl + firstAdd) & 0xFFFF;
            ops[nOut] = opMake(pc, pl); nOut++;
            if (nOut > 1 && firstAdd) ops[0] = opMake(opCode(ops[0]), (opLen(ops[0]) + firstAdd) & 0xFFFF);
            RootState s; memset(&s, 0, sizeof s);
            s.sro = sro; s.sqo = (uint16_t)sqo; s.eqo = (uint16_t)eqo; s.refLen = (uint16_t)refLen; s.score = score; s.status = (rec.rs & 1u) ? stReversed : 0;
                s.len = (uint16_t)nOut;
            s.listOff = slot;
            X.state[r] = s;
            const uint32_t strand = (rec.rs & 1u) ? XP_STRAND : 0u; const bool vb = backLen >= P.minExtLength, vf = forwLen >= P.minExtLength;
            ExtProb pb; pb.qBase = r0; pb.rOff = sro - 1u; pb.qOff = (uint16_t)((sqo - 1) & 0xFFFF); pb.qLen = (uint16_t)(backLen & 0xFFFF);
                pb.flags = strand | XP_REV | (vb ? XP_VALID : 0u);
            ExtProb pf; pf.qBase = r0; pf.rOff = sro + (uint32_t)refLen; pf.qOff = (uint16_t)((eqo + 1) & 0xFFFF); pf.qLen = (uint16_t)(forwLen & 0xFFFF);
                pf.flags = strand | (vf ? XP_VALID : 0u);
            X.probs[2 * (size_t)r] = pb; X.probs[2 * (size_t)r + 1] = pf;
            X.extKeys[2 * (size_t)r] = vb ? 0xFFFFu - pb.qLen : 0xFFFFu; X.extKeys[2 * (size_t)r + 1] = vf ? 0xFFFFu - pf.qLen : 0xFFFFu;
            X.extVals[2 * (size_t)r] = 2u * r; X.extVals[2 * (size_t)r + 1] = 2u * r + 1u;
            X.rowsBound[2 * (size_t)r] = vb ? (unsigned long long)((pb.qLen + 19u) / 10u) : 0ull;
                X.rowsBound[2 * (size_t)r + 1] = vf ? (unsigned long long)((pf.qLen + 19u) / 10u) : 0ull;
        }
    }
    perfect = waveSumU(perfect); touched = waveSumU(touched); gapCalls = waveSumU(gapCalls); gapRows = waveSumU(gapRows); gapCells = waveSumU(gapCells);
    { unsigned long long *c = A.ctr->v; unsigned long long *const dst[5] = {&c[C_PERFECT], &c[C_TOUCHED], &c[C_GAP_CALLS], &c[C_GAP_ROWS], &c[C_GAP_CELLS]};
      const unsigned val[5] = {perfect, touched, gapCalls, gapRows, gapCells}; blockCounters<5>(dst, val); }
}

__device__ __forceinline__ int opScore(const DevParams &P, int code, int len) { return len * (code == OP_M ? P.MS : (code == OP_R ? -P.RC : -P.GE)) + (code >= OP_D ? -P.GO : 0); }
#define YD_OP_COUNT(code, len, m, r, i, d) \
    do { m += (code) == OP_M ? (len) : 0; r += (code) == OP_R ? (len) : 0; i += (code) == OP_I ? (len) : 0; d += (code) == OP_D ? (len) : 0; } while (0)
typedef uint32_t yd_u32x4u __attribute__((ext_vector_type(4), aligned(4)));
struct MergedOps {
    const uint32_t *a, *b, *c; int na, nb, nc; int jab, jbc;
    mutable const uint32_t *wp = nullptr; mutable uint32_t w0 = 0, w1 = 0, w2 = 0, w3 = 0;
    __device__ __forceinline__ uint32_t fetch(const uint32_t *seg, int idx) const
    {
        const uint32_t *base = seg + (idx & ~3);
        if (base != wp) { const yd_u32x4u v = *(YD_GLOBAL const yd_u32x4u *)toGlobal(base); w0 = v.x; w1 = v.y; w2 = v.z; w3 = v.w; wp = base; }
        const int sl = idx & 3;
        return sl == 0 ? w0 : (sl == 1 ? w1 : (sl == 2 ? w2 : w3));
    }
    __device__ int count() const { return (na - jab) + nb + (nc - jbc); }
    int lenA0 = 0, lenC0 = 0;
    __device__ __forceinline__ void setJunctions()
    {
        jab = (na > 0 && opCode(a[0]) == opCode(b[0])) ? 1 : 0; lenA0 = jab ? opLen(a[0]) : 0;
        jbc = (nc > 0 && opCode(c[0]) == opCode(b[nb - 1])) ? 1 : 0; lenC0 = jbc ? opLen(c[0]) : 0;
    }
    __device__ uint32_t at(int k) const
    {
        const int ka = na - jab;
        if (k < ka) return fetch(a, na - 1 - k);
        k -= ka;
        if (k < nb) {
            uint32_t op = fetch(b, k); int len = opLen(op);
            if (k == 0 && jab) len += lenA0;
            if (k == nb - 1 && jbc) len += lenC0;
            return opMake(opCode(op), len & 0xFFFF);
// ... 35 lines not shown
            if (maxMatch < P.wordLen || minItem < 0) f.phase = 4;
            else {
                f.minItem = minItem; f.maxItem = maxItem; f.sQO = sQO; f.eQO = eQO; f.sRO = sRO; f.eRO = eRO; f.phase = 1;
                bool has = false;
                if (minItem != 0) for (int k = 0; k < minItem && !has; k++) { const uint32_t op = L.at(f.start + k); has = opCode(op) == OP_M && opLen(op) >= P.wordLen; }
                if (has) {
                    if (depth >= 5) return nOut;
                    PredFrame c; c.start = f.start; c.len = minItem; c.sqo = f.sqo; c.eqo = (sQO - 1) & 0xFFFF; c.sro = f.sro;
                        c.refLen = (int)((1u + (sRO - 1u) - f.sro) & 0xFFFFu); c.phase = 0;
                    st[depth++] = f; f = c;
                }
            }
            continue;
        }
        if (f.phase == 1) {
            f.phase = 2;
            const int t0 = f.maxItem + 1, tl = f.len - t0; bool has = false;
            if (f.maxItem != f.len - 1) for (int k = 0; k < tl && !has; k++) { const uint32_t op = L.at(f.start + t0 + k); has = opCode(op) == OP_M && opLen(op) >= P.wordLen; }
            if (has) {
                if (depth >= 5) return nOut;
                PredFrame c; c.start = f.start + t0; c.len = tl; c.sqo = (f.eQO + 1) & 0xFFFF; c.eqo = f.eqo; c.sro = f.eRO + 1u;
                c.refLen = (int)((1u + (f.sro + (uint32_t)f.refLen - 1u) - (f.eRO + 1u)) & 0xFFFFu); c.phase = 0;
                st[depth++] = f; f = c;
            }
            continue;
        }
        if (f.phase == 2) {
            int sqo = f.sQO, eqo = f.eQO, refLen = (int)((1u + f.eRO - f.sRO) & 0xFFFFu); uint32_t sro = f.sRO;
            const bool cutB = f.sQO != wS, cutF = f.eQO != wE;
            const bool goBack = cutB, goForw = cutF || !cutB;
            if (goBack) {
                int backLen = (int)((uint32_t)sqo < sro ? (uint32_t)sqo : sro);
                if (backLen > 0) { const int m = matchRun<-1>(q, sqo - 1, gB, sro - 1u, backLen); backLen -= m; sqo -= m; sro -= (uint32_t)m; refLen = (refLen + m) & 0xFFFF; }
                if (backLen >= P.minExtLength && nOut < YD_MEMO) { ExtProb p; p.qBase = qBase; p.rOff = sro - 1u; p.qOff = (uint16_t)((sqo - 1) & 0xFFFF);
                    p.qLen = (uint16_t)(backLen & 0xFFFF); p.flags = strand | XP_REV | XP_VALID; out[nOut++] = p; }
            }
            if (goForw) {
                const uint32_t eRO = sro + (uint32_t)refLen - 1u;
                const uint32_t qrem = (uint32_t)(((qlen - 1) - eqo) & 0xFFFF), rrem = P.maxROff - eRO;
                int forwLen = (int)(qrem < rrem ? qrem : rrem);
                if (forwLen > 0) { const int m = matchRun<1>(q, eqo + 1, gB, eRO + 1u, forwLen); forwLen -= m; eqo += m; refLen = (refLen + m) & 0xFFFF; }
                if (forwLen >= P.minExtLength && nOut < YD_MEMO) { ExtProb p; p.qBase = qBase; p.rOff = sro + (uint32_t)refLen; p.qOff = (uint16_t)((eqo + 1) & 0xFFFF);
                    p.qLen = (uint16_t)(forwLen & 0xFFFF); p.flags = strand | XP_VALID; out[nOut++] = p; }
            }
            f.phase = 4; continue;
        }
        if (depth == 0) break;
        f = st[--depth];
    }
    return nOut;
}

struct P3Root { MergedOps L; uint32_t sro; int sqo, eqo, refLen, status, score; };
__device__ __forceinline__ P3Root p3Merged(const PhaseArgs &X, uint32_t r)
{
    P3Root o; MergedOps &L = o.L; L.a = L.b = L.c = nullptr; L.na = L.nb = L.nc = L.jab = L.jbc = 0;
    const RootState S = X.state[r];
    o.sro = S.sro; o.sqo = S.sqo; o.eqo = S.eqo; o.refLen = S.refLen; o.status = S.status; o.score = S.score;
    L.b = X.stateOps + S.listOff; L.nb = S.len;
    const ExtRes rb = X.res[2 * (size_t)r], rf = X.res[2 * (size_t)r + 1];
    if (rb.score > 0) {
        const int aQ = rb.maxi, aR = rb.maxi + (rb.maxj - YD_LBAND);
        L.a = extOpsPtr(X.extOps, rb); L.na = (int)rb.nOps;
        o.score += rb.score; o.sqo = (o.sqo - aQ) & 0xFFFF; o.sro -= (uint32_t)aR; o.refLen = (o.refLen + aR) & 0xFFFF;
    }
    if (rf.score > 0) {
        const int aQ = rf.maxi, aR = rf.maxi + (rf.maxj - YD_LBAND);
        L.c = extOpsPtr(X.extOps, rf); L.nc = (int)rf.nOps;
        o.score += rf.score; o.eqo = (o.eqo + aQ) & 0xFFFF; o.refLen = (o.refLen + aR) & 0xFFFF;
    }
    L.setJunctions();
    return o;
}

__global__ void __launch_bounds__(256) k_p3_keys(PhaseArgs X, uint32_t rootEnd, uint32_t *keys)
{
    YD_HIGH_PRIO();
    const uint32_t r = X.rootBegin + blockIdx.x * blockDim.x + threadIdx.x;
    if (r >= rootEnd) return;
    const RootState S = X.state[r]; const ExtRes rb = X.res[2 * (size_t)r], rf = X.res[2 * (size_t)r + 1];
    const uint32_t n = (uint32_t)S.len + (rb.score > 0 ? rb.nOps : 0u) + (rf.score > 0 ? rf.nOps : 0u);
    keys[r - X.rootBegin] = 4095u - min(n, 4095u);
}

#ifndef YD_P3_LOCAL_SORT
#define YD_P3_LOCAL_SORT 1
#endif
#ifndef YD_P3_BS
#define YD_P3_BS 256
#endif
__global__ void __launch_bounds__(YD_P3_BS) k_p3_lanes(AlignArgs A, PhaseArgs X)
{
    YD_HIGH_PRIO();
    const int lane = laneId(); const uint32_t t = X.rootBegin + blockIdx.x * blockDim.x + threadIdx.x;
    const DevParams &P = A.P;
#if YD_P3_LOCAL_SORT
    uint32_t r; bool live;
    {
        const bool in = t < A.nRoots;
        uint32_t cls = 64u;
        if (in) {
            const RootState S = X.state[t]; const ExtRes rb = X.res[2 * (size_t)t], rf = X.res[2 * (size_t)t + 1];
            const uint32_t n0 = (uint32_t)S.len + (rb.score > 0 ? rb.nOps : 0u) + (rf.score > 0 ? rf.nOps : 0u);
            cls = 63u - min(n0 >> 2, 63u);
        }
        r = wgDeal<YD_P3_BS>(t, cls); live = r != 0xFFFFFFFFu;
    }
#else
    const bool live = t < A.nRoots;
    const uint32_t r = (live && X.p3Order) ? X.p3Order[t - X.rootBegin] : t;
#endif
    int verdict = -1;
    MergedOps L; L.a = L.b = L.c = nullptr; L.na = L.nb = L.nc = L.jab = L.jbc = 0;
    uint32_t sro = 0; int sqo = 0, eqo = 0, refLen = 0, status = 0, n = 0;
    int matches = 0, mism = 0, ins = 0, del = 0, AGS = 0;
    if (live) {
        const P3Root R0 = p3Merged(X, r);
        L = R0.L; sro = R0.sro; sqo = R0.sqo; eqo = R0.eqo; refLen = R0.refLen; status = R0.status; const int score = R0.score;
        status |= stAligned;
        n = L.count(); const int aligned = score; int maxAGS = 0; verdict = 0;
        {
            for (int k = 0; k < n; k++) {
                const uint32_t op = L.atLean(k); const int code = opCode(op), len = opLen(op);
                YD_OP_COUNT(code, len, matches, mism, ins, del);
                AGS += opScore(P, code, len);
                if (AGS <= 0 || (AGS >= aligned && k != n - 1)) { verdict = 1; break; }
                maxAGS = AGS > maxAGS ? AGS : maxAGS;
            }
        }
        if (verdict == 0) {
            if (matches >= P.minRawScore && maxAGS > AGS) verdict = 1;
            else if (matches >= P.minRawScore) {
                const int tot = (matches + mism + ins + del) & 0xFFFF;
                const double percent = (double)(matches & 0xFFFF) / (double)tot;
                if (!(percent < (double)P.minIdentity)) verdict = 2;
            }
        }
    }
    { const unsigned long long sm = __ballot(verdict == 1); const unsigned slot = waveReserve(sm, X.slowCount, lane); if (verdict == 1) X.slowList[slot] = r; }
    const bool acc = verdict == 2;
    const unsigned long long am = __ballot(acc);
    unsigned nOpsTot = 0;
    if (am) {
        const unsigned ci = waveReserve(am, &A.outCounts[0], lane);
        int incl = acc ? n : 0;
#pragma unroll
        for (int d = 1; d < 64; d <<= 1) { int t = __shfl_up(incl, d, 64); if (lane >= d) incl += t; }
        const int total = __shfl(incl, 63, 64); unsigned ob = 0;
        if (lane == 63) ob = atomicAdd(&A.outCounts[1], (unsigned)total);
        ob = (unsigned)__shfl((int)ob, 63, 64);
        const unsigned oi = ob + (unsigned)(incl - (acc ? n : 0));
        if (acc) {
            if (ci >= A.outClumpCap || (unsigned long long)oi + (unsigned)n > (unsigned long long)A.outOpsCap) atomicCAS(A.errFlag, 0, (int)YERR_OUT);
            else {
                const char codes[4] = {'M', 'R', 'D', 'I'};
                for (int k = 0; k < n; k++) { const uint32_t op = L.atLean(k); A.outOps[oi + k] = ((uint32_t)(uint8_t)codes[opCode(op) & 3] << 16) | (uint32_t)opLen(op); }
                ygpu_clump c; c.sro = sro; c.sqo = (uint16_t)sqo; c.eqo = (uint16_t)eqo; c.refLen = (uint16_t)refLen; c.totScore = (uint16_t)(AGS & 0xFFFF);
                c.totLength = (uint16_t)((matches + mism + ins + del) & 0xFFFF); c.matchedBases = (uint16_t)(matches & 0xFFFF); c.mismatchedBases = (uint16_t)(mism & 0xFFFF);
                c.gapBases = (uint16_t)((ins + del) & 0xFFFF); c.status = (uint8_t)(status | stScored); c.reserved = 0; c.op_start = oi; c.n_ops = (uint32_t)n;
                A.outClumps[ci] = c; A.outRoot[ci] = r; A.outPush[ci] = 0;
                A.rootPushCount[r] = 1; nOpsTot = (unsigned)n;
            }
        }
    }
    const unsigned nAcc = (unsigned)__builtin_popcountll(am); nOpsTot = waveSumU(nOpsTot);
    if (lane == 0 && nAcc) { atomicAdd(&A.ctr->v[C_SCORED], (unsigned long long)nAcc); atomicAdd(&A.ctr->v[C_OPS], (unsigned long long)nOpsTot); }
}


__global__ void __launch_bounds__(64) k_p3_predict(AlignArgs A, PhaseArgs X)
{
    YD_HIGH_PRIO();
    const int lane = laneId(); const DevParams &P = A.P; const uint32_t nSlow = *X.slowCount;
    for (uint32_t base = blockIdx.x * 64u; base < nSlow; base += gridDim.x * 64u) {
        const uint32_t slot = base + (uint32_t)lane; const bool live = slot < nSlow;
        ExtProb pp[YD_MEMO]; int np = 0;
        if (live) {
            const uint32_t r = X.slowList[slot]; const P3Root R0 = p3Merged(X, r);
            const ChainClumpRec rec = YD_ROOT_REC(A, r); const uint32_t r0 = A.B.readOff[rec.rs >> 1]; const int qlen = (int)(A.B.readOff[(rec.rs >> 1) + 1] - r0);
            np = predictCarefulDPs(P, R0.L, R0.L.count(), R0.sqo, R0.eqo, R0.sro, R0.refLen, toGlobal((rec.rs & 1u) ? A.B.rev : A.B.fwd) + r0, qlen, toGlobal(A.bases), pp, r0,
                (rec.rs & 1u) ? XP_STRAND : 0u);
        }
        int incl = np;
#pragma unroll
        for (int d = 1; d < 64; d <<= 1) { int t = __shfl_up(incl, d, 64); if (lane >= d) incl += t; }
        const int total = __shfl(incl, 63, 64); unsigned pb = 0;
        if (lane == 63 && total) pb = atomicAdd(X.nProb2, (unsigned)total);
        pb = (unsigned)__shfl((int)pb, 63, 64);
        if (live) {
            const unsigned first = pb + (unsigned)(incl - np); int kept = 0;
            for (int k = 0; k < np; k++) {
                const unsigned idx = first + (unsigned)k; if (idx >= X.probs2Cap) break;
                X.probs2[idx] = pp[k]; X.rowsBound2[idx] = (unsigned long long)((pp[k].qLen + 19u) / 10u);
                uint32_t *key = X.memoKeys + ((size_t)slot * YD_MEMO + (size_t)k) * 3;
                key[0] = pp[k].rOff; key[1] = (uint32_t)pp[k].qOff | ((uint32_t)pp[k].qLen << 16); key[2] = ((pp[k].flags & XP_REV) ? 1u : 0u) | (idx << 1);
                kept++;
            }
            X.memoCount[slot] = (unsigned)kept;
        }
    }
}

__global__ void __launch_bounds__(64) k_align_p3(AlignArgs A, PhaseArgs X)
{
    YD_HIGH_PRIO();
    const unsigned wave = blockIdx.x; const int lane = laneId();
    WaveMem M = carveScratch(A.scratch + (size_t)wave * A.scratchPerWave, A.maxQ, A.traceRows, A.listCap, A.genCap);
    __shared__ uint16_t sTrace[YD_LDS_CELLS];
    Aligner al(A, M, sTrace);
    PROF_INIT();
    const unsigned nRoots = X.useList ? uniU(*X.slowCount) : uniU(A.nRoots);
    for (;;) {
        if (__ballot(1) != ~0ull) { atomicCAS(A.errFlag, 0, (int)YERR_EXEC); break; }
        unsigned t = 0;
        if (lane == 0) t = atomicAdd(A.queueHead, 4u);
        const unsigned r0 = uniU(t);
        if (r0 >= nRoots) break;
        const unsigned r1 = min(r0 + 4u, nRoots);
        for (unsigned ri = r0; ri < r1; ri++) {
// ... 33 lines not shown
```

yaha_amd/csrc/device/stage_align.hip:

```cpp
#include "ctx.h"
#include "phase_lanes.h"
#include "gap_band_lanes.h"
#include "gap_band_pk.h"
#include "ext_lanes_pk.h"
#include "split_lanes.h"
#include "dp_stage.h"
#include "align_kernels.h"
#include "layout.h"

static bool extRowsPacked(const ygpu_ctx *ctx, bool caps)
{
    const bool force32 = getenv("YGPU_EXT32") != nullptr;
    const DevParams &P = ctx->P;
    return !force32 && !caps && P.MS >= 0 && (long long)P.MS * std::max(1, ctx->maxQ) <= 15000 && P.RC >= 0 && P.GO >= 0 && P.GE >= 0 && P.X >= 0
        && (long long)P.RC + P.X + P.GO + 21ll * P.GE <= 4000;
}

static bool gapBandPacked(const ygpu_ctx *ctx)
{
    const DevParams &P = ctx->P;
    return getenv("YGPU_EXT32") == nullptr && getenv("YGPU_GAP32") == nullptr && P.MS >= 0 && P.RC >= 0 && P.GO >= 0 && P.GE >= 0 && 64ll * std::max(P.MS,
        P.RC) + P.GO + 64ll * P.GE <= 12000;
}

static void alignDims(ygpu_ctx *ctx, int &listCap, int &front, int &genCap, int &traceRows)
{
    front = 2 * ctx->maxQ + 8 * ctx->P.bandWidth + 64; listCap = 2 * front + 3 * ctx->maxQ + 1024;
    const long long md = std::min<long long>(ctx->P.maxDesert, 32000), g = std::min<long long>(ctx->P.maxGap, 32000), wMax = md + g + 2 * ctx->P.bandWidth + 3;
    genCap = (int)std::max<long long>(1024, wMax + 1);
    const long long wExt = 4ll * ctx->P.bandWidth + 1;
    traceRows = (int)std::max<long long>((ctx->maxQ + 2) * ((wExt + 63) / 64), ((md + 2) * wMax + 63) / 64 + 1);
}


static int alignWithLaneExtensions(ygpu_ctx *ctx, AlignArgs &A, unsigned waves, uint32_t stateOpsCap, uint32_t gapOpsPerJoint)
{
    const uint32_t NC = ctx->nClumps; const uint32_t nProb = 2 * NC; int rc;
    uint32_t *cnt = ctx->counters.as<uint32_t>();
    ENSURE(ctx->rootState, sizeof(RootState) * (uint64_t)NC); ENSURE(ctx->stateOps, 4ull * stateOpsCap); ENSURE(ctx->extProbs, sizeof(ExtProb) * (uint64_t)nProb);
    ENSURE(ctx->rowsBound, 8ull * (nProb + 1)); ENSURE(ctx->stripOff, 8ull * (nProb + 1)); ENSURE(ctx->extRes, sizeof(ExtRes) * (uint64_t)nProb);
    ENSURE(ctx->slowList, 4ull * (NC + 1));
    HIPCHK(hipMemsetAsync(cnt + CNT_STATEOPS, 0, 16, ctx->stream));
    HIPCHK(hipMemsetAsync(cnt + CNT_QALIGN, 0, 4, ctx->stream));
    HIPCHK(hipMemsetAsync((unsigned long long *)ctx->rowsBound.p + nProb, 0, 8, ctx->stream));
    PhaseArgs X; X.state = ctx->rootState.as<RootState>(); X.stateOps = ctx->stateOps.as<uint32_t>(); X.stateOpsCount = cnt + CNT_STATEOPS; X.stateOpsCap = stateOpsCap;
    X.probs = ctx->extProbs.as<ExtProb>(); X.rowsBound = ctx->rowsBound.as<unsigned long long>(); X.res = ctx->extRes.as<ExtRes>(); X.extOps = nullptr; X.rootBegin = 0;
        X.p3Order = nullptr; X.band24 = 0;
    TRACE("lanes: ensure");
    X.slowList = ctx->slowList.as<uint32_t>(); X.slowCount = cnt + CNT_SLOW; X.useList = 1;
    EV0(T_P1);
    ENSURE(ctx->jointCount, 4ull * (NC + 2)); ENSURE(ctx->jointBase, 4ull * (NC + 2));
    X.jointCount = ctx->jointCount.as<uint32_t>(); X.jointBase = ctx->jointBase.as<uint32_t>();
    KL(k_joint_counts, dim3(gridFor(NC + 1, 256)), dim3(256), 0, ctx->stream, A, X);
    rc = cubScan(ctx, ctx->jointCount.as<uint32_t>(), ctx->jointBase.as<uint32_t>(), NC + 1); if (rc) return rc;
    uint32_t J = 0; rc = fetchU32(ctx, ctx->jointBase.as<uint32_t>() + NC, &J); if (rc) return rc;
    const uint32_t gapOpsCap = (uint32_t)std::min<uint64_t>(0x7FFFFFF0ull, (uint64_t)gapOpsPerJoint * J + (1u << 20));
    ENSURE(ctx->joints, sizeof(JointRec) * (uint64_t)(J + 1)); ENSURE(ctx->sortKeys, 4ull * (J + 1)); ENSURE(ctx->sortVals, 4ull * (J + 1)); ENSURE(ctx->sortKeys2, 4ull * (J + 1));
        ENSURE(ctx->sortVals2, 4ull * (J + 1));
    ENSURE(ctx->gapOps, 4ull * gapOpsCap); ENSURE(ctx->slowList, 4ull * (std::max(NC, J) + 1));
    X.slowList = ctx->slowList.as<uint32_t>();
    X.joints = ctx->joints.as<JointRec>(); X.nJoints = J; X.sortKeys = ctx->sortKeys.as<uint32_t>(); X.sortVals = ctx->sortVals.as<uint32_t>();
        X.sortedVals = ctx->sortVals2.as<uint32_t>();
    X.nDP = cnt + CNT_NDP; X.nDPb = cnt + CNT_NB12; X.gapOps = ctx->gapOps.as<uint32_t>(); X.gapOpsCount = cnt + CNT_GAPOPS; X.gapOpsCap = gapOpsCap;
    HIPCHK(hipMemsetAsync(cnt + CNT_NDP, 0, 12, ctx->stream)); HIPCHK(hipMemsetAsync(cnt + CNT_NB12, 0, 12, ctx->stream));
    if (J) {
        KL(k_p1_joints, dim3(gridFor(NC, 256)), dim3(256), 0, ctx->stream, A, X);
        rc = bucketOrder(ctx, X.sortKeys, X.sortVals, 0, J, 0, 0, 1u << YD_JKEY_BITS, ctx->sortVals2.as<uint32_t>(), ctx->stream); if (rc) return rc;
        const unsigned gBlocks16 = (unsigned)std::min<uint64_t>(gridFor(J, 64), (uint64_t)ctx->nCU * 9), gBlocks32 = (unsigned)std::min<uint64_t>(gridFor(J, 64),
            (uint64_t)ctx->nCU * 6);
        ENSURE(ctx->gapScratch, (size_t)YD_GAP_SCRATCH * 64 * std::max(gBlocks16, gBlocks32)); X.gapScratch = ctx->gapScratch.as<uint8_t>();
        X.band24 = (gapBandPacked(ctx) && !getenv("YGPU_GAP24_OFF")) ? 1u : 0u;
        if (gapBandPacked(ctx)) {
            KL(k_gap_band_pk<12>, dim3(gBlocks16), dim3(64), 0, ctx->stream, A, X); KL(k_gap_band_pk<16>, dim3(gBlocks16), dim3(64), 0, ctx->stream, A, X);
            if (X.band24) KL(k_gap_band_pk<24>, dim3(gBlocks16), dim3(64), 0, ctx->stream, A, X);
        }
        else { KL(k_gap_band<12>, dim3(gBlocks16), dim3(64), 0, ctx->stream, A, X); KL(k_gap_band<16>, dim3(gBlocks16), dim3(64), 0, ctx->stream, A, X); }
        KL(k_gap_lanes<16>, dim3(gBlocks16), dim3(64), 0, ctx->stream, A, X);
        KL(k_gap_lanes<32>, dim3(gBlocks32), dim3(64), 0, ctx->stream, A, X);
        KL(k_gap_wave, dim3(std::min(waves, 512u)), dim3(64), 0, ctx->stream, A, X);
    }
    ENSURE(ctx->extKeys, 4ull * (nProb + 1)); ENSURE(ctx->extVals, 4ull * (nProb + 1)); ENSURE(ctx->extKeys2, 4ull * (nProb + 1)); ENSURE(ctx->extOrder, 4ull * (nProb + 1));
    X.extKeys = ctx->extKeys.as<uint32_t>(); X.extVals = ctx->extVals.as<uint32_t>();
    KL(k_p1_assemble, dim3(gridFor(NC, 256)), dim3(256), 0, ctx->stream, A, X);
    rc = cubScan64(ctx, ctx->rowsBound.as<unsigned long long>(), ctx->stripOff.as<unsigned long long>(), nProb + 1); if (rc) return rc;
    EV1(T_P1);
    TRACE("lanes: p1+scan");
    if (kTrace) { uint32_t v[3] = {0, 0, 0}; fetchU32(ctx, cnt + CNT_SLOW, &v[0]); uint32_t w[3] = {0, 0, 0}; fetchU32(ctx, cnt + CNT_NDP, w, 3); v[1] = w[0]; v[2] = w[2];
        fprintf(stderr, "[ygpu] roots %u, joints %u, DP joints %u (W<=16: %u, wave fallback %u), gap ops %u\n", NC, J, v[1], w[1], v[0], v[2]); }
    if (kTrace && getenv("YGPU_JOINT_HIST")) {
        std::vector<JointRec> hj(J); hipMemcpy(hj.data(), ctx->joints.p, sizeof(JointRec) * (size_t)J, hipMemcpyDeviceToHost);
        unsigned long long nj[4] = {0, 0, 0, 0}, cj[4] = {0, 0, 0, 0}, b3 = 0, b3lim = 0, c3lim = 0, f3 = 0, wh[5] = {0, 0, 0, 0, 0};
        for (auto &j : hj) if (j.kind == JK_DP) {
            const bool banded = (j.flags & 2u) != 0; const int q = j.qGap, r = j.rGap, ld = q > r ? q - r : r - q, W = banded ? 2 * ctx->P.bandWidth + ld + 1 : r + 1;
            const uint32_t cls = gapJointClass(gapJointKey(ctx->P, banded, q, r)); nj[cls]++; cj[cls] += (unsigned long long)q * (unsigned long long)std::min(W, r + 1);
            if (cls == 3) { if (banded) { b3++; if (W <= 32 && q <= YD_GROWS - 1 && r <= YD_GREF) { b3lim++; c3lim += (unsigned long long)q * W; } } else f3++;
                wh[std::min(4, (W - 17) / 8)]++; }
        }
        fprintf(stderr, "[ygpu] DP joints by class (band <= 12 / band <= 16 / other W <= 16 / the rest): %llu %llu %llu %llu; strip cells %llu %llu %llu %llu; "
                        "the rest: banded %llu (W <= 32 within the band kernels' limits: %llu, %llu cells), full %llu; "
                        "W 17-24 / 25-32 / 33-40 / 41-48 / more: %llu %llu %llu %llu %llu\n",
// ... 54 lines not shown
                while (lo < hi) { uint32_t mid = lo + (hi - lo + 1) / 2; if ((double)(ctx->hStripOff[2 * (size_t)mid] - ctx->hStripOff[2 * (size_t)r0]) <= perRange) lo = mid;
                    else hi = mid - 1; }
                cuts.push_back(lo); r0 = lo;
            }
        }
        nRanges = cuts.size() - 1;
        const unsigned long long minChunks = maxWavesK + 64ull;
        nChunksArena = std::min<unsigned long long>(std::max<unsigned long long>(nChunksArena, minChunks), 0xFFFFFFF0ull);
        {
            const unsigned long long capChunks = ctx->extTrace.cap > 256 ? (unsigned long long)((ctx->extTrace.cap - 256) / (YD_CHUNK_DWORDS * 4ull)) : 0ull;
            if (nRanges == 1 && capChunks > minChunks && nChunksArena > capChunks && (double)nChunksArena <= 1.3 * (double)capChunks) nChunksArena = capChunks;
        }
        if (ctx->extTrace.ensureExact((size_t)nChunksArena * YD_CHUNK_DWORDS * 4ull + 256) == 0) break;
        (void)hipGetLastError();
        if (nChunksArena <= minChunks) { ctx->err = "hipMalloc failed for the extension trace arena (not even one chunk per wave fits)"; return YGPU_ENOMEM; }
        budgetChunks = std::max<unsigned long long>(minChunks, nChunksArena / 2);
        if (kTrace) fprintf(stderr, "[ygpu] trace arena of %llu chunks refused by the device: retrying with %llu and ranges\n", nChunksArena, budgetChunks);
    }
    ctx->statRanges = (int)nRanges;
    nChunksArena = std::min<unsigned long long>(0xFFFFFFF0ull, (unsigned long long)((ctx->extTrace.cap - 256) / (YD_CHUNK_DWORDS * 4ull)));
    const uint32_t maxCh = (uint32_t)std::min<unsigned long long>(nChunksArena, std::max<unsigned long long>(64ull, 4ull * nChunksArena / std::max(1u, maxWavesK) + 64ull));
    ENSURE(ctx->waveChunks, 4ull * (size_t)maxWavesK * maxCh + 64);
    const uint32_t extOpsCap = (uint32_t)std::min<double>(2.0e9, (double)boundBlocks * 10.0 * ctx->opsRatio + 4.0e6);
    ENSURE(ctx->extOps, 4ull * extOpsCap + 64);
    ENSURE(ctx->chunkCnt, 32ull * (nRanges + 2));
    HIPCHK(hipMemsetAsync(ctx->chunkCnt.p, 0, 32ull * (nRanges + 2), ctx->stream));
    ENSURE(ctx->traceCnt, 64); HIPCHK(hipMemsetAsync(ctx->traceCnt.p, 0, 64, ctx->stream));
    TRACE("lanes: trace arena");
    if (kTrace && getenv("YGPU_COUNT_DUPS")) {
        std::vector<ExtProb> hp(nProb); hipMemcpy(hp.data(), ctx->extProbs.p, sizeof(ExtProb) * (size_t)nProb, hipMemcpyDeviceToHost);
        std::vector<std::array<uint32_t, 4>> keys; keys.reserve(nProb);
        for (auto &e : hp) if (e.flags & XP_VALID) keys.push_back({e.qBase, e.rOff, (uint32_t)e.qOff | ((uint32_t)e.qLen << 16), e.flags & 3u});
        std::sort(keys.begin(), keys.end()); size_t dup = 0, sameStart = 0;
        for (size_t k = 1; k < keys.size(); k++) { dup += keys[k] == keys[k - 1];
            sameStart += keys[k][0] == keys[k - 1][0] && keys[k][1] == keys[k - 1][1] && (keys[k][2] & 0xFFFF) == (keys[k - 1][2] & 0xFFFF) && keys[k][3] == keys[k - 1][3]; }
        fprintf(stderr, "[ygpu] extension problems: %zu valid, %zu exact duplicates (%.2f%%), %zu share (read, strand, direction, rOff, qOff) with their predecessor (%.2f%%)\n",
            keys.size(), dup, 100.0 * dup / std::max<size_t>(1, keys.size()), sameStart, 100.0 * sameStart / std::max<size_t>(1, keys.size()));
    }
    if (kTrace) fprintf(stderr, "[ygpu] trace bound %.2f GB, arena %.2f GB (%llu chunks, ratio %.3f), %zu range(s); ext ops cap %u\n", boundBlocks * 128.0 / 1e9,
        nChunksArena * (YD_CHUNK_DWORDS * 4.0) / 1e9, nChunksArena, ctx->traceRatio, nRanges, extOpsCap);
    ENSURE(ctx->rowsClock, 16); { const unsigned long long init[2] = {~0ull, 0ull}; HIPCHK(hipMemcpyAsync(ctx->rowsClock.p, init, 16, hipMemcpyHostToDevice, ctx->stream)); }
    E.clock = ctx->rowsClock.as<unsigned long long>();
    E.trace = ctx->extTrace.as<uint32_t>(); E.nChunks = (uint32_t)nChunksArena; E.chunkCount = ctx->traceCnt.as<unsigned int>(); E.waveChunks = ctx->waveChunks.as<uint32_t>();
        E.maxCh = maxCh;
    E.ops = ctx->extOps.as<uint32_t>(); E.opsCount = ctx->traceCnt.as<unsigned int>() + 1; E.opsCap = extOpsCap;
    E.ctr = ctx->ctr.as<DevCounters>(); E.errFlag = ctx->errFlag.as<int>(); E.dbgMode = getenv("YGPU_TRACE_MODE") ? atoi(getenv("YGPU_TRACE_MODE")) : 0;
    X.extOps = ctx->extTrace.as<uint32_t>();
    uint32_t *cc = ctx->chunkCnt.as<uint32_t>();
    unsigned long long usedChunksMax = 0;
    EV0(T_XROWS);
    for (size_t c = 0; c < nRanges; c++) {
        const uint32_t r0 = cuts[c], r1 = cuts[c + 1], p0 = 2 * r0, np = 2 * (r1 - r0);
        E.probs = ctx->extProbs.as<ExtProb>() + p0; E.nProb = np; E.res = ctx->extRes.as<ExtRes>() + p0;
        E.queue = cc + 8 * c;
        HIPCHK(hipMemsetAsync(ctx->traceCnt.p, 0, 4, ctx->stream));
        HIPCHK(hipMemsetAsync(E.res, 0, sizeof(ExtRes) * (uint64_t)np, ctx->stream));
        {
            const uint32_t sub = 0xFFFFu - (uint32_t)std::min(ctx->maxQ, 0xFFFF); int shift = 0; while (((uint32_t)ctx->maxQ >> shift) >= kBucketMax - 1u) shift++;
            uint32_t *v1 = ctx->extOrder.as<uint32_t>() + p0;
            rc = bucketOrder(ctx, ctx->extKeys.as<uint32_t>() + p0, nullptr, 0, np, sub, shift, ((uint32_t)ctx->maxQ >> shift) + 2u, v1, ctx->stream); if (rc) return rc;
            E.order = v1;
        }
        const unsigned blocks = (unsigned)std::min<uint64_t>(((uint64_t)np + rowsBS - 1) / rowsBS, (uint64_t)maxBlocksK);
        static const int rowsSerial = getenv("YGPU_ROWS_SERIAL") ? atoi(getenv("YGPU_ROWS_SERIAL")) : 1;
        if (rowsSerial && rowsShare && ctx->maxQ <= 4096) {
            std::lock_guard<std::mutex> lk(gRowsMu[ctx->device & 63]); const int dv = ctx->device & 63;
            const int depth = std::min(4, std::max(1, rowsSerial)); const int slot = (int)(gRowsSeq[dv]++ % (unsigned long long)depth);
            if (!gRowsEvValid[dv][slot]) { if (hipEventCreateWithFlags(&gRowsEv[dv][slot], hipEventDisableTiming) == hipSuccess) gRowsEvValid[dv][slot] = true; }
            else HIPCHK(hipStreamWaitEvent(ctx->stream, gRowsEv[dv][slot], 0));
            KL(rowsKernel, dim3(blocks), dim3(rowsBS), 0, ctx->stream, E);
            if (gRowsEvValid[dv][slot]) HIPCHK(hipEventRecord(gRowsEv[dv][slot], ctx->stream));
        } else
        KL(rowsKernel, dim3(blocks), dim3(rowsBS), 0, ctx->stream, E);
        if (c + 1 == nRanges) EV1(T_XROWS);
        TRACE("lanes: ext_rows");
        if (c == 0) { ctx->evUsed[T_XTRACE] = true; hipEventRecord(ctx->ev[T_XTRACE][0], ctx->stream); }
        if (kTrace && getenv("YGPU_TRACE_LENS")) {
            HIPCHK(streamSync(ctx));
            std::vector<ExtRes> hr(np); std::vector<uint32_t> ho(np);
            hipMemcpy(hr.data(), E.res, sizeof(ExtRes) * (size_t)np, hipMemcpyDeviceToHost); hipMemcpy(ho.data(), E.order, 4ull * np, hipMemcpyDeviceToHost);
            unsigned long long walkers = 0, sumLen = 0, sumWaveMax = 0, sumRows = 0, hist[8] = {0}; std::vector<uint32_t> lens; lens.reserve(np);
            for (uint32_t w = 0; w < np; w += 64) { uint32_t mx = 0; for (uint32_t k = w; k < std::min(np, w + 64); k++) { const ExtRes &r = hr[ho[k]];
                const uint32_t len = r.score > 0 ? (uint32_t)r.maxi : 0u; walkers += r.score > 0; sumLen += len; sumRows += r.rows; mx = std::max(mx, len); int b = 0;
                while (b < 7 && (len >> (b + 3))) b++; hist[len ? b : 0] += 1; } sumWaveMax += mx; }
            fprintf(stderr, "[ygpu] traceback: %u problems, %llu walk (%.1f%%), mean walk %.1f rows (all) / %.1f (walkers), rows computed mean %.1f; sum over waves of "
                "the longest walk %llu = %.1f x the lanes' mean\n",
                    np, walkers, 100.0 * walkers / np, (double)sumLen / np, (double)sumLen / std::max(1ull, walkers), (double)sumRows / np, sumWaveMax,
                        (double)sumWaveMax * 64.0 / std::max(1ull, sumLen));
            fprintf(stderr, "[ygpu] walk length histogram (0..7, 8.., 16.., 32.., 64.., 128.., 256.., 512..):"); for (int b = 0; b < 8; b++) fprintf(stderr, " %llu", hist[b]);
                fprintf(stderr, "\n");
        }
        if (traceSort > 0 && np > 4096u) {
            uint32_t *k0 = ctx->extKeys.as<uint32_t>() + p0, *v0 = ctx->extVals.as<uint32_t>() + p0, *v1 = ctx->extKeys2.as<uint32_t>() + p0;
            static const int lenBits = getenv("YGPU_TRACE_LENBITS") ? std::min(8, std::max(1, atoi(getenv("YGPU_TRACE_LENBITS")))) : 7;
            int lenShift = 0; while ((ctx->maxQ >> lenShift) > (1 << lenBits) - 1) lenShift++;
            int keyBits = lenBits; while (keyBits < 32 && ((unsigned long long)E.nChunks >> std::min(traceSort, 31)) >> (keyBits - lenBits)) keyBits++;
            KL(k_trace_keys, dim3(gridFor(np, 256)), dim3(256), 0, ctx->stream, E.res, E.order, np, E.waveChunks, E.maxCh, std::min(traceSort, 31), lenShift, lenBits, k0, v0);
            rc = bucketOrder(ctx, k0, v0, 0, np, 0, std::max(0, keyBits - 12), 1u << std::min(keyBits, 12), v1, ctx->stream); if (rc) return rc;
            E.order = v1;
        }
        KL(traceKernel, dim3(gridFor(np, traceBS)), dim3(traceBS), 0, ctx->stream, E);
        if (c + 1 == nRanges) hipEventRecord(ctx->ev[T_XTRACE][1], ctx->stream);
        TRACE("lanes: ext_trace");
        if (kTrace) { unsigned w8[8]; hipMemcpyFromSymbol(w8, HIP_SYMBOL(gTraceDbg), sizeof w8); if (w8[0]) { ExtRes rr;
            hipMemcpy(&rr, E.res + w8[6], sizeof rr, hipMemcpyDeviceToHost); ExtProb pp; hipMemcpy(&pp, E.probs + w8[6], sizeof pp, hipMemcpyDeviceToHost);
            fprintf(stderr, "[ygpu] k_ext_trace left its strip: dword %d of %u, f0 %u, laneOff %u; problem %u where %08x (wave %u lane %u phase %u) score %d maxi %d maxj "
                "%d rows %u qLen %u flags %u\n", (int)w8[1], w8[2], w8[3], w8[4], w8[6], w8[7], w8[7] >> 10, (w8[7] >> 4) & 63, w8[7] & 15, rr.score, rr.maxi, rr.maxj, rr.rows,
                    pp.qLen, pp.flags);
            memset(w8, 0, sizeof w8); hipMemcpyToSymbol(HIP_SYMBOL(gTraceDbg), w8, sizeof w8); } }
        AlignArgs Ac = A; Ac.nRoots = r1; Ac.queueHead = cc + 8 * c + 1;
        PhaseArgs Xc = X; Xc.rootBegin = r0; Xc.slowList = ctx->slowList.as<uint32_t>() + r0; Xc.slowCount = cc + 8 * c + 2; Xc.useList = 1;
        if (c == 0) { ctx->evUsed[T_P3] = true; hipEventRecord(ctx->ev[T_P3][0], ctx->stream); }
        const uint32_t nr = r1 - r0, cap2 = nr / 4 + 1024;
        if (ctx->splitLanes) {
            ENSURE(ctx->memoKeys, 12ull * YD_MEMO * (nr + 1)); ENSURE(ctx->memoCount, 4ull * (nr + 1)); ENSURE(ctx->probs2, sizeof(ExtProb) * (uint64_t)cap2);
            ENSURE(ctx->rowsBound2, 8ull * (cap2 + 1)); ENSURE(ctx->extRes2, sizeof(ExtRes) * (uint64_t)cap2); ENSURE(ctx->fallList, 4ull * (nr + 1));
            HIPCHK(hipMemsetAsync(ctx->memoCount.p, 0, 4ull * (nr + 1), ctx->stream)); HIPCHK(hipMemsetAsync(ctx->rowsBound2.p, 0, 8ull * (cap2 + 1), ctx->stream));
            Xc.memoKeys = ctx->memoKeys.as<uint32_t>(); Xc.memoCount = ctx->memoCount.as<unsigned int>(); Xc.probs2 = ctx->probs2.as<ExtProb>();
                Xc.rowsBound2 = ctx->rowsBound2.as<unsigned long long>();
            Xc.nProb2 = cc + 8 * c + 3; Xc.probs2Cap = cap2;
        } else { Xc.memoKeys = nullptr; Xc.memoCount = nullptr; Xc.probs2 = nullptr; Xc.rowsBound2 = nullptr; Xc.nProb2 = nullptr; Xc.probs2Cap = 0; }
        {
            static const bool p3Sort = getenv("YGPU_P3_SORT") && atoi(getenv("YGPU_P3_SORT")) != 0;
            Xc.p3Order = nullptr;
            if (p3Sort && nr > 4096u) {
                uint32_t *kk = ctx->extKeys.as<uint32_t>() + p0, *oo = ctx->extVals.as<uint32_t>() + p0;
                KL(k_p3_keys, dim3(gridFor(nr, 256)), dim3(256), 0, ctx->stream, Xc, r1, kk);
                rc = bucketOrder(ctx, kk, nullptr, r0, nr, 0, 0, 4096u, oo, ctx->stream); if (rc) return rc;
                Xc.p3Order = oo;
            }
        }
        KL(k_p3_lanes, dim3(gridFor(nr, YD_P3_BS)), dim3(YD_P3_BS), 0, ctx->stream, Ac, Xc);
        if (ctx->splitLanes) KL(k_p3_predict, dim3((unsigned)std::min<uint64_t>(gridFor(nr, 64), (uint64_t)ctx->nCU * 8)), dim3(64), 0, ctx->stream, Ac, Xc);
        PhaseArgs Xw = Xc;
        unsigned int used[2] = {0, 0}; uint32_t three[3] = {0, 0, 0};
        HIPCHK(hipMemcpyAsync(used, ctx->traceCnt.p, 8, hipMemcpyDeviceToHost, ctx->stream));
        if (ctx->splitLanes) HIPCHK(hipMemcpyAsync(three, cc + 8 * c + 2, 8, hipMemcpyDeviceToHost, ctx->stream));
        HIPCHK(streamSync(ctx));
        usedChunksMax = std::max<unsigned long long>(usedChunksMax, used[0]);
        if (ctx->splitLanes) {
            const uint32_t nSlow = three[0], n2 = std::min(three[1], cap2);
            if (kTrace) fprintf(stderr, "[ygpu] range %zu: chunks used %u, ext ops %u; split roots %u, careful extensions listed %u\n", c, used[0], used[1], nSlow, n2);
            if (nSlow) {
                ExtArgs E2 = E;
                if (n2) {
                    E2.probs = ctx->probs2.as<ExtProb>(); E2.nProb = n2;
                    HIPCHK(hipMemsetAsync(ctx->extRes2.p, 0, sizeof(ExtRes) * (uint64_t)n2, ctx->stream));
                    {
                        ENSURE(ctx->keys2a, 4ull * (cap2 + 1)); ENSURE(ctx->keys2b, 4ull * (cap2 + 1)); ENSURE(ctx->vals2a, 4ull * (cap2 + 1));
                            ENSURE(ctx->vals2b, 4ull * (cap2 + 1));
                        KL(k_prob_keys, dim3(gridFor(n2, 256)), dim3(256), 0, ctx->stream, ctx->probs2.as<ExtProb>(), n2, ctx->keys2a.as<uint32_t>(), ctx->vals2a.as<uint32_t>());
                        { const uint32_t sub = 0xFFFFu - (uint32_t)std::min(ctx->maxQ, 0xFFFF); int shift = 0; while (((uint32_t)ctx->maxQ >> shift) >= kBucketMax - 1u) shift++;
                          rc = bucketOrder(ctx, ctx->keys2a.as<uint32_t>(), nullptr, 0, n2, sub, shift, ((uint32_t)ctx->maxQ >> shift) + 2u, ctx->vals2b.as<uint32_t>(),
                              ctx->stream); if (rc) return rc; }
                    }
                    E2.order = ctx->vals2b.as<uint32_t>(); E2.res = ctx->extRes2.as<ExtRes>(); E2.queue = cc + 8 * c + 4; E2.ctr = nullptr;
                    {
                        const uint64_t blocks2 = ctx->rows2PerCU > 0 ? (uint64_t)ctx->rows2PerCU : (uint64_t)ctx->nCU;
                        const uint64_t b2 = rows2BS == 512u ? std::max<uint64_t>(1, blocks2 / 2) : blocks2;
                        KL(rowsKernel2, dim3((unsigned)std::min<uint64_t>(std::min<uint64_t>(((uint64_t)n2 + rows2BS - 1) / rows2BS, b2), (uint64_t)maxBlocksK)), dim3(rows2BS), 0,
                            ctx->stream, E2); }
                    KL(traceKernel, dim3(gridFor(n2, traceBS)), dim3(traceBS), 0, ctx->stream, E2);
                }
                ENSURE(ctx->splitScratch, (size_t)YD_SL_BYTES * (((size_t)nSlow + 63) / 64 * 64));
                SplitArgs Sx; Sx.scratch = ctx->splitScratch.as<uint8_t>(); Sx.memoKeys = ctx->memoKeys.as<uint32_t>(); Sx.memoCount = ctx->memoCount.as<unsigned int>();
                Sx.res2 = ctx->extRes2.as<ExtRes>(); Sx.ops2 = ctx->extTrace.as<uint32_t>(); Sx.nProb2 = n2;
                Sx.fallList = ctx->fallList.as<uint32_t>(); Sx.fallCount = cc + 8 * c + 5; Sx.nSlots = nSlow;
                KL(k_split_lanes, dim3(gridFor(nSlow, 64)), dim3(64), 0, ctx->stream, Ac, Xc, Sx);
                Xw.slowList = ctx->fallList.as<uint32_t>(); Xw.slowCount = cc + 8 * c + 5;
                if (kTrace) { uint32_t fc = 0; HIPCHK(hipMemcpyAsync(&fc, cc + 8 * c + 5, 4, hipMemcpyDeviceToHost, ctx->stream)); HIPCHK(streamSync(ctx)); unsigned w8[8];
                    hipMemcpyFromSymbol(w8, HIP_SYMBOL(gFallWhy), sizeof w8);
                    fprintf(stderr, "[ygpu] roots left to the wave kernel %u (other %u, DP not listed %u, second split %u, depth/list %u)\n", fc, w8[0], w8[1], w8[2], w8[3]);
                    memset(w8, 0, sizeof w8); hipMemcpyToSymbol(HIP_SYMBOL(gFallWhy), w8, sizeof w8); }
            }
        }
        {
            unsigned p3Waves = std::min<unsigned>(waves, std::max<unsigned>(64u, (r1 - r0) / 8u));
            if (ctx->splitLanes && ctx->lastFall >= 0) p3Waves = std::min<unsigned>(p3Waves, std::max<unsigned>(64u, (unsigned)std::min<long long>(1ll << 20,
                2ll * ctx->lastFall)));
            KL(k_align_p3, dim3(p3Waves), dim3(64), 0, ctx->stream, Ac, Xw);
            if (ctx->splitLanes && c + 1 == nRanges) HIPCHK(hipMemcpyAsync(&ctx->hFall, Xw.slowCount, 4, hipMemcpyDeviceToHost, ctx->stream));
        }
        if (c + 1 == nRanges) hipEventRecord(ctx->ev[T_P3][1], ctx->stream);
        TRACE("lanes: p3");
        if (kTrace && getenv("YGPU_LIST_HIST")) {
            const uint32_t nr2 = r1 - r0; std::vector<ExtRes> hr2(2 * (size_t)nr2); std::vector<RootState> hs(nr2);
            hipMemcpy(hr2.data(), ctx->extRes.as<ExtRes>() + 2 * (size_t)r0, sizeof(ExtRes) * hr2.size(), hipMemcpyDeviceToHost);
                hipMemcpy(hs.data(), ctx->rootState.as<RootState>() + r0, sizeof(RootState) * nr2, hipMemcpyDeviceToHost);
            unsigned long long hx[8] = {0}, hb[8] = {0}, ht[8] = {0}, sumx = 0, sumb = 0; const unsigned edges[7] = {0, 1, 2, 4, 8, 16, 32};
            auto bin = [&](unsigned v) { int k = 0; while (k < 7 && v > edges[k]) k++; return k; };
            for (uint32_t k = 0; k < nr2; k++) {
                const unsigned a = hr2[2 * k].score > 0 ? hr2[2 * k].nOps : 0u, c2 = hr2[2 * k + 1].score > 0 ? hr2[2 * k + 1].nOps : 0u, b = hs[k].len; hx[bin(a)]++;
                hx[bin(c2)]++; hb[bin(b)]++; ht[bin(a + b + c2)]++; sumx += a + c2; sumb += b; }
            fprintf(stderr, "[ygpu] list lengths over %u roots (bins: 0, 1, 2, 3-4, 5-8, 9-16, 17-32, more): extension lists", nr2);
                for (int k = 0; k < 8; k++) fprintf(stderr, " %llu", hx[k]);
            fprintf(stderr, "; phase-1 lists"); for (int k = 0; k < 8; k++) fprintf(stderr, " %llu", hb[k]); fprintf(stderr, "; merged");
                for (int k = 0; k < 8; k++) fprintf(stderr, " %llu", ht[k]);
// ... 135 lines not shown
    uint32_t no = 0, ef = 0; int rc = fetchU32(ctx, cnt + CNT_DPOPS, &no); if (rc) return rc; rc = fetchU32(ctx, ctx->errFlag.p, &ef); if (rc) return rc;
    if (ef) { char b[64]; snprintf(b, sizeof b, "dp batch failed with device error %u", ef); ctx->err = b; return YGPU_EINTERNAL; }
    ctx->hDpRes.resize(n); ctx->hDpOps.resize(no);
    if (n) HIPCHK(hipMemcpy(ctx->hDpRes.data(), ctx->dpRes.p, sizeof(ygpu_dp_result) * (uint64_t)n, hipMemcpyDeviceToHost));
    if (no) HIPCHK(hipMemcpy(ctx->hDpOps.data(), ctx->dpOps.p, 4ull * no, hipMemcpyDeviceToHost));
    *results = ctx->hDpRes.data(); *ops = ctx->hDpOps.data(); *n_ops = no;
    return 0;
}

static int dpBatchLanes(ygpu_ctx *ctx, const ygpu_dp_problem *problems, uint32_t n, bool second, const ygpu_dp_result **results, const uint32_t **ops, uint64_t *n_ops)
{
    std::vector<ExtProb> xp; std::vector<uint32_t> xdst; std::vector<unsigned long long> xrows; std::vector<JointRec> jp; std::vector<uint32_t> jdst;
    uint64_t gapOpsBound = 64;
    for (uint32_t k = 0; k < n; k++) {
        const ygpu_dp_problem &p = problems[k]; const uint32_t base = ctx->hReadOff[p.read];
        if (p.mode >= YGPU_DP_EXT_FWD) {
            ExtProb e; e.qBase = base; e.rOff = p.rOff; e.qOff = p.qOff; e.qLen = p.qLen;
                e.flags = (p.strand ? XP_STRAND : 0u) | (p.mode == YGPU_DP_EXT_REV ? XP_REV : 0u) | XP_VALID;
            xp.push_back(e); xdst.push_back(k); xrows.push_back((unsigned long long)((p.qLen + 19u) / 10u));
        } else {
            JointRec j; memset(&j, 0, sizeof j); j.nsro = p.rOff; j.qBase = base; j.nsqo = p.qOff; j.qGap = p.qLen; j.rGap = p.rLen; j.kind = JK_DP;
                j.flags = (uint8_t)((p.strand ? 1u : 0u) | (p.mode == YGPU_DP_BANDED ? 2u : 0u));
            jp.push_back(j); jdst.push_back(k); gapOpsBound += (uint64_t)p.qLen + p.rLen + 2;
        }
    }
    const uint32_t nX = (uint32_t)xp.size(), nJ = (uint32_t)jp.size(); int rc;
    uint32_t *cnt = ctx->counters.as<uint32_t>(); DevBatch B = devBatch(ctx);
    HIPCHK(hipMemsetAsync(ctx->errFlag.p, 0, 4, ctx->stream));
    std::vector<ExtRes> hres(nX); std::vector<JointRec> hj(nJ); std::vector<uint32_t> xOff(nX + 1, 0), jOff(nJ + 1, 0);
    if (nX) {
        ENSURE(ctx->extProbs, sizeof(ExtProb) * (uint64_t)nX); ENSURE(ctx->extRes, sizeof(ExtRes) * (uint64_t)nX); ENSURE(ctx->chunkCnt, 64);
        HIPCHK(hipMemcpyAsync(ctx->extProbs.p, xp.data(), sizeof(ExtProb) * (uint64_t)nX, hipMemcpyHostToDevice, ctx->stream));
        HIPCHK(hipMemsetAsync(ctx->chunkCnt.p, 0, 64, ctx->stream)); HIPCHK(hipMemsetAsync(ctx->extRes.p, 0, sizeof(ExtRes) * (uint64_t)nX, ctx->stream));
        unsigned long long blocks = 0, opsBound = 64; for (uint32_t k = 0; k < nX; k++) { blocks += xrows[k]; opsBound += 2ull * xp[k].qLen + 4; }
        const bool caps = ctx->P.maxGap < YD_LW || ctx->P.maxIntron < YD_LW;
        const bool pk = extRowsPacked(ctx, caps);
        auto rowsKernel = pk ? k_ext_rows_pk<false> : (caps ? k_ext_rows<true, false> : k_ext_rows<false, false>);
        auto rowsKernel2 = pk ? k_ext_rows_pk<true> : (caps ? k_ext_rows<true, true> : k_ext_rows<false, true>);
        auto traceKernel = pk ? k_ext_trace_pk : k_ext_trace;
        int perCU = 2; if (hipOccupancyMaxActiveBlocksPerMultiprocessor(&perCU, rowsKernel, 256, 0) != hipSuccess || perCU < 1) perCU = 2;
        const unsigned blocksK = (unsigned)std::min<uint64_t>(((uint64_t)nX + 255) / 256, (uint64_t)ctx->nCU * (second ? 1 : perCU)), wavesK = blocksK * 4u;
        for (unsigned long long mult = 2;; mult *= 8) {
        const unsigned long long nCh = mult * blocks / (YD_CHUNK_FLUSHES * 64ull) + 2ull * wavesK + 64ull;
        if (nCh * (YD_CHUNK_DWORDS * 4ull) > (64ull << 30) || opsBound > 0x7FFFFFF0ull) { ctx->err = "too many extension rows in one ygpu_dp_batch call"; return YGPU_EINVAL; }
        const uint32_t maxCh = (uint32_t)nCh;
        ENSURE(ctx->extTrace, nCh * (YD_CHUNK_DWORDS * 4ull) + 256); ENSURE(ctx->waveChunks, 4ull * (size_t)wavesK * maxCh + 64); ENSURE(ctx->extOps, 4ull * opsBound + 64);
            ENSURE(ctx->traceCnt, 64);
        HIPCHK(hipMemsetAsync(ctx->traceCnt.p, 0, 64, ctx->stream));
        ExtArgs E; E.P = ctx->P; E.bases = ctx->dBases.as<uint8_t>(); E.fwd = ctx->dFwd.as<uint8_t>(); E.rev = ctx->dRev.as<uint8_t>(); E.fwd4 = ctx->dFwd4.as<uint8_t>();
            E.rev4 = ctx->dRev4.as<uint8_t>(); E.probs = ctx->extProbs.as<ExtProb>(); E.nProb = nX;
        E.order = nullptr; E.clock = nullptr; E.trace = ctx->extTrace.as<uint32_t>(); E.nChunks = (uint32_t)nCh; E.chunkCount = ctx->traceCnt.as<unsigned int>();
            E.waveChunks = ctx->waveChunks.as<uint32_t>(); E.maxCh = maxCh;
        E.ops = ctx->extOps.as<uint32_t>(); E.opsCount = ctx->traceCnt.as<unsigned int>() + 1; E.opsCap = (uint32_t)opsBound; E.res = ctx->extRes.as<ExtRes>();
        E.queue = ctx->chunkCnt.as<unsigned int>(); E.ctr = nullptr; E.errFlag = ctx->errFlag.as<int>(); E.dbgMode = 0;
        if (second) KL(rowsKernel2, dim3(blocksK), dim3(256), 0, ctx->stream, E); else KL(rowsKernel, dim3(blocksK), dim3(256), 0, ctx->stream, E);
        { const unsigned tbs = pk ? (unsigned)YD_TRACE_BS : 256u; KL(traceKernel, dim3(gridFor(nX, tbs)), dim3(tbs), 0, ctx->stream, E); }
        uint32_t ef2 = 0; rc = fetchU32(ctx, ctx->errFlag.p, &ef2); if (rc) return rc;
        if (ef2 != YERR_TRACEMEM) break;
        if (mult >= 1024) { ctx->err = "extension trace arena overflows"; return YGPU_ENOMEM; }
        HIPCHK(hipMemsetAsync(ctx->errFlag.p, 0, 4, ctx->stream)); HIPCHK(hipMemsetAsync(ctx->chunkCnt.p, 0, 64, ctx->stream));
            HIPCHK(hipMemsetAsync(ctx->extRes.p, 0, sizeof(ExtRes) * (uint64_t)nX, ctx->stream));
        }
        HIPCHK(hipMemcpyAsync(hres.data(), ctx->extRes.p, sizeof(ExtRes) * (uint64_t)nX, hipMemcpyDeviceToHost, ctx->stream)); HIPCHK(streamSync(ctx));
        for (uint32_t k = 0; k < nX; k++) xOff[k + 1] = xOff[k] + (hres[k].score > 0 ? hres[k].nOps : 0u);
    }
    if (nJ) {
        const uint32_t gapOpsCap = (uint32_t)std::min<uint64_t>(0x7FFFFFF0ull, gapOpsBound);
        ENSURE(ctx->joints, sizeof(JointRec) * (uint64_t)(nJ + 1)); ENSURE(ctx->sortKeys, 4ull * (nJ + 1)); ENSURE(ctx->sortVals, 4ull * (nJ + 1));
            ENSURE(ctx->sortVals2, 4ull * (nJ + 1));
        ENSURE(ctx->gapOps, 4ull * gapOpsCap); ENSURE(ctx->slowList, 4ull * (nJ + 1));
        HIPCHK(hipMemcpyAsync(ctx->joints.p, jp.data(), sizeof(JointRec) * (uint64_t)nJ, hipMemcpyHostToDevice, ctx->stream));
        KL(k_dp_classify, dim3(gridFor(nJ, 256)), dim3(256), 0, ctx->stream, ctx->P, ctx->dBases.as<uint8_t>(), ctx->dFwd.as<uint8_t>(), ctx->dRev.as<uint8_t>(),
            ctx->joints.as<JointRec>(), nJ, ctx->sortKeys.as<uint32_t>(), ctx->sortVals.as<uint32_t>());
        std::vector<uint32_t> keys(nJ), idx(nJ);
        rc = fetchU32(ctx, ctx->sortKeys.p, keys.data(), nJ); if (rc) return rc;
        for (uint32_t k = 0; k < nJ; k++) idx[k] = k;
        std::stable_sort(idx.begin(), idx.end(), [&](uint32_t a, uint32_t b) { return keys[a] < keys[b]; });
        uint32_t nd[3] = {0, 0, 0}, nb[3] = {0, 0, 0}; for (uint32_t k = 0; k < nJ; k++) if (keys[k] != YD_JKEY_NONE) { const uint32_t cls = gapJointClass(keys[k]); nd[0]++;
            nd[1] += cls <= 2u; nb[0] += cls == 0u; nb[1] += cls <= 1u; nb[2] += gapJointBand24(keys[k]) ? 1u : 0u; }
        HIPCHK(hipMemcpyAsync(cnt + CNT_NB12, nb, 12, hipMemcpyHostToDevice, ctx->stream));
        HIPCHK(hipMemcpyAsync(ctx->sortVals2.p, idx.data(), 4ull * nJ, hipMemcpyHostToDevice, ctx->stream));
        HIPCHK(hipMemcpyAsync(cnt + CNT_NDP, nd, 12, hipMemcpyHostToDevice, ctx->stream));
        HIPCHK(hipMemsetAsync(cnt + CNT_SLOW, 0, 4, ctx->stream)); HIPCHK(hipMemsetAsync(cnt + CNT_QALIGN, 0, 4, ctx->stream));
        int listCap, front, genCap, traceRows; alignDims(ctx, listCap, front, genCap, traceRows); listCap = 64;
        const size_t per = alignScratchBytes(ctx->maxQ, traceRows, listCap, genCap); const unsigned waves = 512;
        ENSURE(ctx->scratchAlign, per * waves);
        AlignArgs A; memset(&A, 0, sizeof A); A.P = ctx->P; A.bases = ctx->dBases.as<uint8_t>(); A.B = B; A.queueHead = cnt + CNT_QALIGN;
            A.scratch = ctx->scratchAlign.as<uint8_t>(); A.scratchPerWave = per;
        A.maxQ = ctx->maxQ; A.listCap = listCap; A.front = front; A.genCap = genCap; A.traceRows = traceRows; A.ctr = ctx->ctr.as<DevCounters>();
            A.errFlag = ctx->errFlag.as<int>();
        PhaseArgs X; memset(&X, 0, sizeof X); X.joints = ctx->joints.as<JointRec>(); X.nJoints = nJ; X.sortedVals = ctx->sortVals2.as<uint32_t>(); X.nDP = cnt + CNT_NDP;
            X.nDPb = cnt + CNT_NB12;
        X.gapOps = ctx->gapOps.as<uint32_t>(); X.gapOpsCount = cnt + CNT_GAPOPS; X.gapOpsCap = gapOpsCap; X.slowList = ctx->slowList.as<uint32_t>(); X.slowCount = cnt + CNT_SLOW;
        const unsigned gBlocks16 = (unsigned)std::min<uint64_t>(gridFor(nJ, 64), (uint64_t)ctx->nCU * 9), gBlocks32 = (unsigned)std::min<uint64_t>(gridFor(nJ, 64),
            (uint64_t)ctx->nCU * 6);
        ENSURE(ctx->gapScratch, (size_t)YD_GAP_SCRATCH * 64 * std::max(gBlocks16, gBlocks32)); X.gapScratch = ctx->gapScratch.as<uint8_t>();
        X.band24 = (gapBandPacked(ctx) && !getenv("YGPU_GAP24_OFF")) ? 1u : 0u;
        if (gapBandPacked(ctx)) {
            KL(k_gap_band_pk<12>, dim3(gBlocks16), dim3(64), 0, ctx->stream, A, X); KL(k_gap_band_pk<16>, dim3(gBlocks16), dim3(64), 0, ctx->stream, A, X);
            if (X.band24) KL(k_gap_band_pk<24>, dim3(gBlocks16), dim3(64), 0, ctx->stream, A, X);
        }
        else { KL(k_gap_band<12>, dim3(gBlocks16), dim3(64), 0, ctx->stream, A, X); KL(k_gap_band<16>, dim3(gBlocks16), dim3(64), 0, ctx->stream, A, X); }
        KL(k_gap_lanes<16>, dim3(gBlocks16), dim3(64), 0, ctx->stream, A, X);
        KL(k_gap_lanes<32>, dim3(gBlocks32), dim3(64), 0, ctx->stream, A, X);
        KL(k_gap_wave, dim3(waves), dim3(64), 0, ctx->stream, A, X);
        HIPCHK(hipMemcpyAsync(hj.data(), ctx->joints.p, sizeof(JointRec) * (uint64_t)nJ, hipMemcpyDeviceToHost, ctx->stream)); HIPCHK(streamSync(ctx));
        for (uint32_t k = 0; k < nJ; k++) jOff[k + 1] = jOff[k] + hj[k].nOps;
// ... 63 lines not shown
```

Measured before the change: 422,600.

## Score phase-3 roots from per-segment op-list summaries instead of walking merged ops

Phase 1 and the extension trace kernels now build a compact per-segment summary while emitting ops: match, mismatch and gap counts, running score extremes, and first and last op. Phase 3 can then combine three summaries algebraically to decide reject, split or accept, without walking the merged op lists, falling back to the walk when needed. This removes per-root traversal of op arrays in global memory, at the cost of extra 32-byte summary stores per extension and per root, plus more registers in the trace kernels. The unused P3 sort path and wgDeal helper are removed, and counters for summary-scored versus walked roots are added.

Result: slower. 405,100 (-4.1%).

```diff
diff --git a/yaha_amd/csrc/device/abi.hip b/yaha_amd/csrc/device/abi.hip
--- a/yaha_amd/csrc/device/abi.hip
+++ b/yaha_amd/csrc/device/abi.hip
@@ -8,7 +8,8 @@
 unsigned long long gRowsSeq[64];
 std::atomic<int> gActiveRuns[64];
 const char *const kStageNames[T_N] = {"seed_lookup", "hit_sort", "fragments_regions", "chain", "align_dp", "layout", "align_p1_gapfill", "ext_rows", "ext_trace",
-                                      "align_p3_score_split", "ext_rows_device_clock", "ext_rows_packed16"};
+                                      "align_p3_score_split", "ext_rows_device_clock", "ext_rows_packed16", "p3_roots_by_summary",
+                                      "p3_roots_walked"};
 thread_local const ygpu_ctx *tlsPfFailed = nullptr;
 
 int runTo(ygpu_ctx *ctx, int stage)
@@ -45,6 +46,7 @@
     ctx->segSortMax = ydSegSortMax();
     if (const char *e = getenv("YGPU_SEGSORT_MAX")) { long v = atol(e); if (v >= 1 && v <= (long)ydSegSortMax()) ctx->segSortMax = (uint32_t)v; }
     if (const char *e = getenv("YGPU_SPLIT_LANES")) ctx->splitLanes = atoi(e);
+    if (const char *e = getenv("YGPU_P3_SUMMARY")) ctx->p3Summary = atoi(e);
     if (const char *e = getenv("YGPU_ROWS2_PER_CU")) ctx->rows2PerCU = atoi(e);
     if (const char *e = getenv("YGPU_ALIGN_WAVES")) ctx->alignWavesPerCU = atoi(e);
     gCtxPerDevice[device & 63]++; ctx->counted = true;
@@ -312,7 +314,8 @@
                              &ctx->scanState, &ctx->bucketWork, &ctx->scratchAlign,
                          &ctx->segLists, &ctx->subB, &ctx->subE, &ctx->subLists, &ctx->subBigB, &ctx->subBigE, &ctx->sub2B, &ctx->sub2E, &ctx->sub2Lists, &ctx->sub3B, &ctx->sub3E,
                              &ctx->sub3Lists, &ctx->kmerParts, &ctx->scratchChain, &ctx->dpProbs, &ctx->dpRes, &ctx->dpOps, &ctx->rootState, &ctx->stateOps, &ctx->extProbs,
-                             &ctx->rowsBound, &ctx->stripOff, &ctx->extRes, &ctx->extTrace, &ctx->chunkCnt, &ctx->memoKeys, &ctx->memoCount, &ctx->probs2, &ctx->rowsBound2,
+                             &ctx->rowsBound, &ctx->stripOff, &ctx->extRes, &ctx->stateSum, &ctx->extSum, &ctx->extTrace, &ctx->chunkCnt, &ctx->memoKeys, &ctx->memoCount,
+                                 &ctx->probs2, &ctx->rowsBound2,
                              &ctx->stripOff2, &ctx->extRes2, &ctx->extTrace2, &ctx->rowsClock, &ctx->splitScratch, &ctx->fallList, &ctx->keys2a, &ctx->keys2b, &ctx->vals2a,
                              &ctx->vals2b, &ctx->extKeys, &ctx->extVals, &ctx->extKeys2, &ctx->extOrder, &ctx->slowList, &ctx->gapScratch, &ctx->jointCount, &ctx->jointBase,
                              &ctx->joints, &ctx->sortKeys, &ctx->sortVals, &ctx->sortKeys2, &ctx->sortVals2, &ctx->gapOps, &ctx->waveChunks, &ctx->extOps, &ctx->traceCnt,
@@ -414,12 +417,13 @@
 int ygpu_run(ygpu_ctx *ctx)
 {
     if (!ctx || !ctx->stream) return YGPU_EINVAL;
-    ctx->stageDone = 0; const double t0 = nowMs(); ctx->statAttempts = 0; ctx->statRanges = 0;
+    ctx->stageDone = 0; const double t0 = nowMs(); ctx->statAttempts = 0; ctx->statRanges = 0; ctx->p3BySummary = ctx->p3Walked = 0;
     struct Active { int d; explicit Active(int dv) : d(dv) { gActiveRuns[d]++; } ~Active() { gActiveRuns[d]--; } } active(ctx->device & 63);
     int rc = runTo(ctx, 3);
     if (kStats) { size_t fb = 0, tb = 0; hipMemGetInfo(&fb, &tb);
-        fprintf(stderr, "[ygpu] ctx %p run: %u reads, rc %d, %.1f ms; align attempts %d, ranges %d, trace arena %.2f GB (ratio %.3f), free %.1f GB\n", (void *)ctx, ctx->nReads, rc,
-        nowMs() - t0, ctx->statAttempts, ctx->statRanges, ctx->extTrace.cap / 1e9, ctx->traceRatio, fb / 1e9); }
+        fprintf(stderr, "[ygpu] ctx %p run: %u reads, rc %d, %.1f ms; align attempts %d, ranges %d, trace arena %.2f GB (ratio %.3f), free %.1f GB; "
+            "roots scored from summaries %llu, walked %llu\n", (void *)ctx, ctx->nReads, rc,
+        nowMs() - t0, ctx->statAttempts, ctx->statRanges, ctx->extTrace.cap / 1e9, ctx->traceRatio, fb / 1e9, ctx->p3BySummary, ctx->p3Walked); }
     if (rc) { (void)hipStreamSynchronize(ctx->stream); (void)hipGetLastError(); return rc; }
     if (ydCheckStateOn()) {
         if (getenv("YGPU_CHECK_STATE_INJECT") && ctx->scanState.p) (void)hipMemsetAsync((char *)ctx->scanState.p + 8, 0x01, 4, ctx->stream);
@@ -434,6 +438,8 @@
         if (t == T_XROWS_DEV) ctx->ms[t] = (ctx->evUsed[T_XROWS] && ctx->hRowsClock[1] > ctx->hRowsClock[0] && ctx->hRowsClock[0] != ~0ull)
             ? (float)((double)(ctx->hRowsClock[1] - ctx->hRowsClock[0]) / 1.0e5) : 0;
         if (t == T_XROWS_PK) ctx->ms[t] = ctx->rowsPacked ? 1.0f : 0.0f;
+        if (t == T_P3_BYSUM) ctx->ms[t] = (float)ctx->p3BySummary;
+        if (t == T_P3_WALKED) ctx->ms[t] = (float)ctx->p3Walked;
         if (t < T_TOP) ctx->totalMs += ctx->ms[t];
     }
     return 0;
diff --git a/yaha_amd/csrc/device/ctx.h b/yaha_amd/csrc/device/ctx.h
--- a/yaha_amd/csrc/device/ctx.h
+++ b/yaha_amd/csrc/device/ctx.h
@@ -59,7 +59,7 @@
     CNT_SCANFAIL = CNT_NREG + 2,
     CNT_N = CNT_NREG + 4
 };
-enum { T_SEED = 0, T_SORT, T_FRAGS, T_CHAIN, T_ALIGN, T_LAYOUT, T_TOP, T_P1 = T_TOP, T_XROWS, T_XTRACE, T_P3, T_XROWS_DEV, T_XROWS_PK, T_N };
+enum { T_SEED = 0, T_SORT, T_FRAGS, T_CHAIN, T_ALIGN, T_LAYOUT, T_TOP, T_P1 = T_TOP, T_XROWS, T_XTRACE, T_P3, T_XROWS_DEV, T_XROWS_PK, T_P3_BYSUM, T_P3_WALKED, T_N };
 
 extern std::atomic<int> gCtxPerDevice[64];
 extern std::mutex gRowsMu[64];
@@ -118,6 +118,10 @@
     DevBuf rootPush, rootBase, outClumps, outClumps2, outOps, outRoot, outPush, dstIdx, readCount, readStart;
     DevBuf scratchAlign, dpProbs, dpRes, dpOps;
     DevBuf rootState, stateOps, extProbs, rowsBound, stripOff, extRes, extTrace, chunkCnt;
+    DevBuf stateSum, extSum;
+    uint32_t sumEpoch = 0;
+    int p3Summary = 1;
+    unsigned long long p3BySummary = 0, p3Walked = 0;
     DevBuf memoKeys, memoCount, probs2, rowsBound2, stripOff2, extRes2, extTrace2, splitScratch, fallList;
     DevBuf keys2a, keys2b, vals2a, vals2b, extKeys, extVals, extKeys2, extOrder, slowList;
     DevBuf gapScratch, jointCount, jointBase, joints, sortKeys, sortVals, sortKeys2, sortVals2, gapOps;
diff --git a/yaha_amd/csrc/device/ext_lanes.h b/yaha_amd/csrc/device/ext_lanes.h
--- a/yaha_amd/csrc/device/ext_lanes.h
+++ b/yaha_amd/csrc/device/ext_lanes.h
@@ -1,4 +1,5 @@
 #pragma once
+#include "../p3_summary_core.h"
 #include "align.h"
 
 #define YD_REFILL_MIN 4
@@ -16,6 +17,17 @@
 static_assert(sizeof(ExtProb) == 16 && sizeof(ExtRes) == 32, "k_ext_rows_pk moves these as 16-byte vectors (non-temporal loads / stores)");
 __device__ __forceinline__ const uint32_t *extOpsPtr(const uint32_t *traceBase, const ExtRes &r) {
     return traceBase + (long long)(((unsigned long long)r.where << 32) | (unsigned long long)r.opsOff); }
+
+__device__ __forceinline__ void extSumStore(yd_u32x4 *dst, const yp3::Rec &o, uint32_t tag)
+{
+    const yd_u32x4 lo = {(uint32_t)o.m, (uint32_t)o.r, (uint32_t)o.g, (uint32_t)o.tot}, hi = {(uint32_t)o.lo, (uint32_t)o.hi, o.op0, o.tag | tag};
+    YD_GLOBAL yd_u32x4 *d = (YD_GLOBAL yd_u32x4 *)toGlobal(dst); d[0] = lo; d[1] = hi;
+}
+__device__ __forceinline__ yp3::Rec extSumLoad(const yd_u32x4 *src)
+{
+    YD_GLOBAL const yd_u32x4 *s = (YD_GLOBAL const yd_u32x4 *)toGlobal(src); const yd_u32x4 lo = s[0], hi = s[1];
+    yp3::Rec o; o.m = (int)lo.x; o.r = (int)lo.y; o.g = (int)lo.z; o.tot = (int)lo.w; o.lo = (int)hi.x; o.hi = (int)hi.y; o.op0 = hi.z; o.tag = hi.w; return o;
+}
 
 struct ExtArgs {
     DevParams P; const uint8_t *bases; const uint8_t *fwd, *rev;
@@ -28,6 +40,7 @@
     uint32_t *waveChunks; uint32_t maxCh;
     uint32_t *ops; unsigned int *opsCount; uint32_t opsCap;
     ExtRes *res; unsigned int *queue; DevCounters *ctr;
+    yd_u32x4 *sum; uint32_t sumTag;
     int *errFlag; int dbgMode;
 };
 enum { YERR_TRACEMEM = 9 };
@@ -260,6 +273,7 @@
     const bool walk = live && r.score > 0;
     constexpr int leftR = YD_LBAND;
     int n = 0; bool bad = false; int E = 0;
+    yp3::Acc sum; const yp3::Scoring SC = {A.P.MS, A.P.RC, A.P.GO, A.P.GE};
     ExtStrip S; S.arena = toGlobal(A.trace); S.cIdx = -1; S.cBase = S.arena; S.f0 = 0; S.laneOff = 0; S.tab = toGlobal(A.waveChunks); S.limit = 0; S.wild = false;
     if (walk) {
         const int ph = (int)(r.where & 15u);
@@ -276,7 +290,7 @@
             else u.cp -= 5;
         };
         const int row0w = extRowWord(1 + ph) - 3;
-        auto flush = [&]() { const int wp = E - 1 - n; if (wp < c.w + 3) bad = true; else *S.at(wp) = opMake(prev, acc); n++; };
+        auto flush = [&]() { const int wp = E - 1 - n; if (wp < c.w + 3) bad = true; else *S.at(wp) = opMake(prev, acc); n++; sum.add(SC, prev, acc & 0xFFFF); };
         auto put = [&](int code, int len) { if (prev != code) { if (prev >= 0) flush(); prev = code; acc = len; } else acc += len; };
         for (int guard = 0; guard < 70000 && y > 0 && x >= 0 && x < YD_LW; guard++) {
             const int ws = x >> 3, sh = (x & 7) * 4;
@@ -315,7 +329,7 @@
             }
         }
         if (y <= 0 && x > leftR) put(OP_D, x - leftR);
-        if (prev >= 0) { const int wp = E - 1 - n; if (wp < 0) bad = true; else *S.at(wp) = opMake(prev, acc); n++; }
+        if (prev >= 0) { const int wp = E - 1 - n; if (wp < 0) bad = true; else *S.at(wp) = opMake(prev, acc); n++; sum.add(SC, prev, acc & 0xFFFF); }
         if (bad || S.wild) { bad = true; atomicCAS(A.errFlag, 0, (int)YERR_TRACE); n = 0; if (S.wild && atomicCAS(&gTraceDbg[5], 0u, 1u) == 0u) { gTraceDbg[6] = p;
             gTraceDbg[7] = r.where; } }
     }
@@ -345,6 +359,7 @@
             place = (long long)(dst - S.arena);
         }
         r.opsOff = (uint32_t)(unsigned long long)place; r.where = (uint32_t)((unsigned long long)place >> 32); r.nOps = (uint32_t)n; A.res[p] = r;
+        if (A.sum) extSumStore(A.sum + 2 * (size_t)p, sum.extension(), A.sumTag);
     }
 }
 
diff --git a/yaha_amd/csrc/device/ext_lanes_pk.h b/yaha_amd/csrc/device/ext_lanes_pk.h
--- a/yaha_amd/csrc/device/ext_lanes_pk.h
+++ b/yaha_amd/csrc/device/ext_lanes_pk.h
@@ -419,6 +419,7 @@
     const bool walk = live && r.score > 0;
     constexpr int leftR = YD_LBAND;
     int n = 0; bool bad = false; int E = 0;
+    yp3::Acc sum; const yp3::Scoring SC = {A.P.MS, A.P.RC, A.P.GO, A.P.GE};
     ExtStrip S; S.arena = toGlobal(A.trace); S.cIdx = -1; S.cBase = S.arena; S.f0 = 0; S.laneOff = 0; S.tab = toGlobal(A.waveChunks); S.limit = 0; S.wild = false;
     struct Cur { YD_GLOBAL uint32_t *cp; int rr, w; unsigned fb; };
     int y = 0, x = 0, prev = -1, acc = 0, row0w = 0;
@@ -440,7 +441,7 @@
                 32u + 28u;
             else c.cp -= 4;
         };
-        auto flush = [&]() { const int wp = E - 1 - n; if (wp < u.w + 8) bad = true; else *S.at(wp) = opMake(prev, acc); n++; };
+        auto flush = [&]() { const int wp = E - 1 - n; if (wp < u.w + 8) bad = true; else *S.at(wp) = opMake(prev, acc); n++; sum.add(SC, prev, acc & 0xFFFF); };
         auto put = [&](int code, int len) { if (prev != code) { if (prev >= 0) flush(); prev = code; acc = len; } else acc += len; };
 #ifdef YD_PROF
         unsigned tpPass = 0, tpAct = 0, tpRounds = 0, tpFlushR = 0, tpDel = 0, tpIns = 0, tpRows = 0; const bool tpWalks = __ballot(walk) != 0ull;
@@ -549,7 +550,7 @@
 #endif
         if (walk) {
         if (y <= 0 && x > leftR) put(OP_D, x - leftR);
-        if (prev >= 0) { const int wp = E - 1 - n; if (wp < 0) bad = true; else *S.at(wp) = opMake(prev, acc); n++; }
+        if (prev >= 0) { const int wp = E - 1 - n; if (wp < 0) bad = true; else *S.at(wp) = opMake(prev, acc); n++; sum.add(SC, prev, acc & 0xFFFF); }
         if (bad || S.wild) { bad = true; atomicCAS(A.errFlag, 0, (int)YERR_TRACE); n = 0; }
         }
     }
@@ -579,5 +580,6 @@
             place = (long long)(dst - S.arena);
         }
         r.opsOff = (uint32_t)(unsigned long long)place; r.where = (uint32_t)((unsigned long long)place >> 32); r.nOps = (uint32_t)n; A.res[p] = r;
+        if (A.sum) extSumStore(A.sum + 2 * (size_t)p, sum.extension(), A.sumTag);
     }
 }
diff --git a/yaha_amd/csrc/device/phase_lanes.h b/yaha_amd/csrc/device/phase_lanes.h
--- a/yaha_amd/csrc/device/phase_lanes.h
+++ b/yaha_amd/csrc/device/phase_lanes.h
@@ -14,7 +14,7 @@
     uint32_t *slowList; unsigned int *slowCount;
     int useList;
     uint32_t rootBegin;
-    const uint32_t *p3Order;
+    yd_u32x4 *stateSum; const yd_u32x4 *extSum; uint32_t sumTag; int p3Summary; unsigned int *p3Count;
     uint32_t *memoKeys; unsigned int *memoCount; ExtProb *probs2; unsigned long long *rowsBound2; unsigned int *nProb2; uint32_t probs2Cap;
     uint32_t *jointCount; const uint32_t *jointBase; JointRec *joints; uint32_t nJoints;
     uint32_t *sortKeys, *sortVals; const uint32_t *sortedVals; unsigned int *nDP, *nDPb; uint32_t band24;
@@ -212,27 +212,6 @@
     return (cls << 10) | (wf << 5) | (uint32_t)((qGap >> 1) < 30 ? (qGap >> 1) : 30);
 }
 __host__ __device__ __forceinline__ bool gapJointBand24(uint32_t key) { return (key >> 10) == 3u && ((key >> 5) & 31u) < 8u; }
-
-template <int BS = 256>
-__device__ __forceinline__ uint32_t wgDeal(uint32_t root, uint32_t cls)
-{
-    __shared__ uint32_t sHist[65], sOrder[BS];
-    const int lane = laneId();
-    if (threadIdx.x < 65u) sHist[threadIdx.x] = 0u;
-    __syncthreads();
-    const uint32_t inCls = atomicAdd(&sHist[cls], 1u);
-    __syncthreads();
-    if (threadIdx.x < 64u) {
-        const uint32_t c = sHist[lane]; uint32_t incl = c;
-#pragma unroll
-        for (int d = 1; d < 64; d <<= 1) { const uint32_t y = (uint32_t)__shfl_up((int)incl, d, 64); if (lane >= d) incl += y; }
-        sHist[lane] = incl - c; if (lane == 63) sHist[64] = incl;
-    }
-    __syncthreads();
-    sOrder[sHist[cls] + inCls] = cls < 64u ? root : 0xFFFFFFFFu;
-    __syncthreads();
-    return sOrder[threadIdx.x];
-}
 
 __global__ void __launch_bounds__(256) k_p1_joints(AlignArgs A, PhaseArgs X)
 {
@@ -386,8 +365,9 @@
             auto refAt = [&](uint32_t off) -> uint32_t { const uint32_t b = gB[off >> 1]; return (off & 1u) ? (b & 15u) : (b >> 4); };
             const DevFrag *F = A.clumpFrags + rec.fragOff;
             uint32_t *ops = X.stateOps + slot; int nOut = 0, pc = -1, pl = 0, score = 0;
-            auto put = [&](int code, int len) { if (pc == code) { pl = (pl + len) & 0xFFFF; return; } if (pc >= 0) { ops[nOut] = opMake(pc, pl); nOut++; } pc = code;
-                pl = len & 0xFFFF; };
+            yp3::Acc sum; const yp3::Scoring SC = {P.MS, P.RC, P.GO, P.GE};
+            auto put = [&](int code, int len) { if (pc == code) { pl = (pl + len) & 0xFFFF; return; } if (pc >= 0) { ops[nOut] = opMake(pc, pl); nOut++; sum.add(SC, pc, pl); }
+                pc = code; pl = len & 0xFFFF; };
             const DevFrag firstF = F[0]; DevFrag cur = firstF;
             for (int k = 1; k <= n; k++) {
                 { const int ql = fragQLen(cur.sqo, cur.eqo); put(OP_M, ql); score += P.MS * ql; }
@@ -428,8 +408,9 @@
                 }
             }
             if (nOut == 0) pl = (pl + firstAdd) & 0xFFFF;
-            ops[nOut] = opMake(pc, pl); nOut++;
-            if (nOut > 1 && firstAdd) ops[0] = opMake(opCode(ops[0]), (opLen(ops[0]) + firstAdd) & 0xFFFF);
+            ops[nOut] = opMake(pc, pl); nOut++; sum.add(SC, pc, pl);
+            if (nOut > 1 && firstAdd) { ops[0] = opMake(opCode(ops[0]), (opLen(ops[0]) + firstAdd) & 0xFFFF); sum.growFirstM(SC, firstAdd); }
+            extSumStore(X.stateSum + 2 * (size_t)r, sum.list(), 0u);
             RootState s; memset(&s, 0, sizeof s);
             s.sro = sro; s.sqo = (uint16_t)sqo; s.eqo = (uint16_t)eqo; s.refLen = (uint16_t)refLen; s.score = score; s.status = (rec.rs & 1u) ? stReversed : 0;
                 s.len = (uint16_t)nOut;
@@ -571,7 +552,7 @@
 }
 
 struct P3Root { MergedOps L; uint32_t sro; int sqo, eqo, refLen, status, score; };
-__device__ __forceinline__ P3Root p3Merged(const PhaseArgs &X, uint32_t r)
+__device__ __forceinline__ P3Root p3Frame(const PhaseArgs &X, uint32_t r)
 {
     P3Root o; MergedOps &L = o.L; L.a = L.b = L.c = nullptr; L.na = L.nb = L.nc = L.jab = L.jbc = 0;
     const RootState S = X.state[r];
@@ -588,69 +569,60 @@
         L.c = extOpsPtr(X.extOps, rf); L.nc = (int)rf.nOps;
         o.score += rf.score; o.eqo = (o.eqo + aQ) & 0xFFFF; o.refLen = (o.refLen + aR) & 0xFFFF;
     }
-    L.setJunctions();
     return o;
 }
-
-__global__ void __launch_bounds__(256) k_p3_keys(PhaseArgs X, uint32_t rootEnd, uint32_t *keys)
-{
-    YD_HIGH_PRIO();
-    const uint32_t r = X.rootBegin + blockIdx.x * blockDim.x + threadIdx.x;
-    if (r >= rootEnd) return;
-    const RootState S = X.state[r]; const ExtRes rb = X.res[2 * (size_t)r], rf = X.res[2 * (size_t)r + 1];
-    const uint32_t n = (uint32_t)S.len + (rb.score > 0 ? rb.nOps : 0u) + (rf.score > 0 ? rf.nOps : 0u);
-    keys[r - X.rootBegin] = 4095u - min(n, 4095u);
-}
-
-#ifndef YD_P3_LOCAL_SORT
-#define YD_P3_LOCAL_SORT 1
-#endif
+__device__ __forceinline__ P3Root p3Merged(const PhaseArgs &X, uint32_t r) { P3Root o = p3Frame(X, r); o.L.setJunctions(); return o; }
+
 #ifndef YD_P3_BS
 #define YD_P3_BS 256
 #endif
 __global__ void __launch_bounds__(YD_P3_BS) k_p3_lanes(AlignArgs A, PhaseArgs X)
 {
     YD_HIGH_PRIO();
-    const int lane = laneId(); const uint32_t t = X.rootBegin + blockIdx.x * blockDim.x + threadIdx.x;
+    const int lane = laneId(); const uint32_t r = X.rootBegin + blockIdx.x * blockDim.x + threadIdx.x;
     const DevParams &P = A.P;
-#if YD_P3_LOCAL_SORT
-    uint32_t r; bool live;
-    {
-        const bool in = t < A.nRoots;
-        uint32_t cls = 64u;
-        if (in) {
-            const RootState S = X.state[t]; const ExtRes rb = X.res[2 * (size_t)t], rf = X.res[2 * (size_t)t + 1];
-            const uint32_t n0 = (uint32_t)S.len + (rb.score > 0 ? rb.nOps : 0u) + (rf.score > 0 ? rf.nOps : 0u);
-            cls = 63u - min(n0 >> 2, 63u);
-        }
-        r = wgDeal<YD_P3_BS>(t, cls); live = r != 0xFFFFFFFFu;
-    }
-#else
-    const bool live = t < A.nRoots;
-    const uint32_t r = (live && X.p3Order) ? X.p3Order[t - X.rootBegin] : t;
-#endif
+    const bool live = r < A.nRoots;
     int verdict = -1;
     MergedOps L; L.a = L.b = L.c = nullptr; L.na = L.nb = L.nc = L.jab = L.jbc = 0;
-    uint32_t sro = 0; int sqo = 0, eqo = 0, refLen = 0, status = 0, n = 0;
-    int matches = 0, mism = 0, ins = 0, del = 0, AGS = 0;
+    uint32_t sro = 0; int sqo = 0, eqo = 0, refLen = 0, status = 0, n = 0, aligned = 0;
+    int matches = 0, mism = 0, gaps = 0, AGS = 0;
+    bool walkIt = false;
     if (live) {
-        const P3Root R0 = p3Merged(X, r);
-        L = R0.L; sro = R0.sro; sqo = R0.sqo; eqo = R0.eqo; refLen = R0.refLen; status = R0.status; const int score = R0.score;
+        const P3Root R0 = p3Frame(X, r);
+        L = R0.L; sro = R0.sro; sqo = R0.sqo; eqo = R0.eqo; refLen = R0.refLen; status = R0.status; aligned = R0.score;
         status |= stAligned;
-        n = L.count(); const int aligned = score; int maxAGS = 0; verdict = 0;
-        {
-            for (int k = 0; k < n; k++) {
-                const uint32_t op = L.atLean(k); const int code = opCode(op), len = opLen(op);
-                YD_OP_COUNT(code, len, matches, mism, ins, del);
-                AGS += opScore(P, code, len);
-                if (AGS <= 0 || (AGS >= aligned && k != n - 1)) { verdict = 1; break; }
-                maxAGS = AGS > maxAGS ? AGS : maxAGS;
-            }
-        }
+        walkIt = true;
+        if (X.p3Summary) {
+            const yp3::Rec sb = extSumLoad(X.stateSum + 2 * (size_t)r);
+            yp3::Rec sa = sb, sc = sb; const uint32_t want = (uint32_t)yp3::VALID | X.sumTag;
+            bool have = (sb.tag & (uint32_t)yp3::VALID) != 0u;
+            if (L.na > 0) { sa = extSumLoad(X.extSum + 4 * (size_t)r); have = have && sa.tag == want; }
+            if (L.nc > 0) { sc = extSumLoad(X.extSum + 4 * (size_t)r + 2); have = have && sc.tag == want; }
+            if (have) {
+                const yp3::Scoring SC = {P.MS, P.RC, P.GO, P.GE};
+                const yp3::Verdict v = yp3::compose(SC, aligned, P.minRawScore, P.minIdentity, sa, L.na, sb, L.nb, sc, L.nc);
+                verdict = v.verdict; n = v.nOps; AGS = v.totScore; matches = v.matched; mism = v.mismatched; gaps = v.gapBases;
+                L.jab = v.jab; L.jbc = v.jbc; L.lenA0 = v.jab ? yp3::len(sa.op0) : 0; L.lenC0 = v.jbc ? yp3::len(sc.op0) : 0;
+                walkIt = false;
+            }
+        }
+    }
+    const unsigned long long walkMask = __ballot(walkIt);
+    if (walkIt) {
+        L.setJunctions();
+        n = L.count(); int maxAGS = 0, ins = 0, del = 0; verdict = 0;
+        for (int k = 0; k < n; k++) {
+            const uint32_t op = L.atLean(k); const int code = opCode(op), len = opLen(op);
+            YD_OP_COUNT(code, len, matches, mism, ins, del);
+            AGS += opScore(P, code, len);
+            if (AGS <= 0 || (AGS >= aligned && k != n - 1)) { verdict = 1; break; }
+            maxAGS = AGS > maxAGS ? AGS : maxAGS;
+        }
+        gaps = ins + del;
         if (verdict == 0) {
             if (matches >= P.minRawScore && maxAGS > AGS) verdict = 1;
             else if (matches >= P.minRawScore) {
-                const int tot = (matches + mism + ins + del) & 0xFFFF;
+                const int tot = (matches + mism + gaps) & 0xFFFF;
                 const double percent = (double)(matches & 0xFFFF) / (double)tot;
                 if (!(percent < (double)P.minIdentity)) verdict = 2;
             }
@@ -669,21 +641,48 @@
         if (lane == 63) ob = atomicAdd(&A.outCounts[1], (unsigned)total);
         ob = (unsigned)__shfl((int)ob, 63, 64);
         const unsigned oi = ob + (unsigned)(incl - (acc ? n : 0));
+        bool copyIt = false;
         if (acc) {
             if (ci >= A.outClumpCap || (unsigned long long)oi + (unsigned)n > (unsigned long long)A.outOpsCap) atomicCAS(A.errFlag, 0, (int)YERR_OUT);
             else {
-                const char codes[4] = {'M', 'R', 'D', 'I'};
-                for (int k = 0; k < n; k++) { const uint32_t op = L.atLean(k); A.outOps[oi + k] = ((uint32_t)(uint8_t)codes[opCode(op) & 3] << 16) | (uint32_t)opLen(op); }
                 ygpu_clump c; c.sro = sro; c.sqo = (uint16_t)sqo; c.eqo = (uint16_t)eqo; c.refLen = (uint16_t)refLen; c.totScore = (uint16_t)(AGS & 0xFFFF);
-                c.totLength = (uint16_t)((matches + mism + ins + del) & 0xFFFF); c.matchedBases = (uint16_t)(matches & 0xFFFF); c.mismatchedBases = (uint16_t)(mism & 0xFFFF);
-                c.gapBases = (uint16_t)((ins + del) & 0xFFFF); c.status = (uint8_t)(status | stScored); c.reserved = 0; c.op_start = oi; c.n_ops = (uint32_t)n;
+                c.totLength = (uint16_t)((matches + mism + gaps) & 0xFFFF); c.matchedBases = (uint16_t)(matches & 0xFFFF); c.mismatchedBases = (uint16_t)(mism & 0xFFFF);
+                c.gapBases = (uint16_t)(gaps & 0xFFFF); c.status = (uint8_t)(status | stScored); c.reserved = 0; c.op_start = oi; c.n_ops = (uint32_t)n;
                 A.outClumps[ci] = c; A.outRoot[ci] = r; A.outPush[ci] = 0;
-                A.rootPushCount[r] = 1; nOpsTot = (unsigned)n;
-            }
+                A.rootPushCount[r] = 1; nOpsTot = (unsigned)n; copyIt = true;
+            }
+        }
+        auto opOut = [](uint32_t op, int add) -> uint32_t { const uint32_t len = (op + (uint32_t)add) & 0xFFFFu, code = (op >> 16) & 3u;
+            return ((code == (uint32_t)OP_M ? (uint32_t)'M' : (code == (uint32_t)OP_R ? (uint32_t)'R' : (code == (uint32_t)OP_D ? (uint32_t)'D' : (uint32_t)'I'))) << 16) | len; };
+        for (unsigned long long cm = __ballot(copyIt); cm;) {
+            uint32_t opv[4] = {0u, 0u, 0u, 0u}; int addv[4] = {0, 0, 0, 0}; unsigned dv[4] = {0u, 0u, 0u, 0u}; bool hv[4] = {false, false, false, false};
+#pragma unroll
+            for (int u = 0; u < 4; u++) {
+                if (!cm) break;
+                const int src = __builtin_ctzll(cm); cm &= cm - 1ull;
+#define YD_BC(v) __builtin_amdgcn_readlane((int)(v), src)
+#define YD_BCP(p) ((const uint32_t *)(((unsigned long long)(uint32_t)YD_BC((unsigned long long)(p) >> 32) << 32) | (unsigned long long)(uint32_t)YD_BC((unsigned long long)(p))))
+                const uint32_t *pa = YD_BCP(L.a), *pb = YD_BCP(L.b), *pc = YD_BCP(L.c);
+                const int na = YD_BC(L.na), nb = YD_BC(L.nb), jab = YD_BC(L.jab), jbc = YD_BC(L.jbc), lenA0 = YD_BC(L.lenA0), lenC0 = YD_BC(L.lenC0), nn = YD_BC(n);
+                const unsigned dst = (unsigned)YD_BC(oi);
+#undef YD_BCP
+#undef YD_BC
+                const int ka = na - jab, kb = ka + nb;
+                auto src1 = [&](int k, int &add) -> const uint32_t * {
+                    const bool inA = k < ka, inB = !inA && k < kb;
+                    add = ((inB && k == ka) ? lenA0 : 0) + ((inB && k == kb - 1) ? lenC0 : 0);
+                    return (inA ? pa : (inB ? pb : pc)) + (inA ? na - 1 - k : (inB ? k - ka : k - kb + jbc)); };
+                if (lane < nn) { opv[u] = *toGlobal(src1(lane, addv[u])); dv[u] = dst + (unsigned)lane; hv[u] = true; }
+                for (int k = lane + 64; k < nn; k += 64) { int add; const uint32_t op = *toGlobal(src1(k, add)); A.outOps[dst + (unsigned)k] = opOut(op, add); }
+            }
+#pragma unroll
+            for (int u = 0; u < 4; u++) if (hv[u]) A.outOps[dv[u]] = opOut(opv[u], addv[u]);
         }
     }
     const unsigned nAcc = (unsigned)__builtin_popcountll(am); nOpsTot = waveSumU(nOpsTot);
-    if (lane == 0 && nAcc) { atomicAdd(&A.ctr->v[C_SCORED], (unsigned long long)nAcc); atomicAdd(&A.ctr->v[C_OPS], (unsigned long long)nOpsTot); }
+    { unsigned long long *const dst[2] = {&A.ctr->v[C_SCORED], &A.ctr->v[C_OPS]}; const unsigned val[2] = {nAcc, nOpsTot}; blockCounters<2>(dst, val); }
+    { unsigned int *const dst[2] = {X.p3Count, X.p3Count + 1};
+      const unsigned val[2] = {(unsigned)__builtin_popcountll(__ballot(live) & ~walkMask), (unsigned)__builtin_popcountll(walkMask)}; blockCountersU32<2>(dst, val); }
 }
 
 
diff --git a/yaha_amd/csrc/device/stage_align.hip b/yaha_amd/csrc/device/stage_align.hip
--- a/yaha_amd/csrc/device/stage_align.hip
+++ b/yaha_amd/csrc/device/stage_align.hip
@@ -40,12 +40,16 @@
     ENSURE(ctx->rootState, sizeof(RootState) * (uint64_t)NC); ENSURE(ctx->stateOps, 4ull * stateOpsCap); ENSURE(ctx->extProbs, sizeof(ExtProb) * (uint64_t)nProb);
     ENSURE(ctx->rowsBound, 8ull * (nProb + 1)); ENSURE(ctx->stripOff, 8ull * (nProb + 1)); ENSURE(ctx->extRes, sizeof(ExtRes) * (uint64_t)nProb);
     ENSURE(ctx->slowList, 4ull * (NC + 1));
+    ENSURE(ctx->stateSum, 32ull * NC);
+    { const size_t was = ctx->extSum.cap; ENSURE(ctx->extSum, 32ull * nProb); if (ctx->extSum.cap != was) HIPCHK(hipMemsetAsync(ctx->extSum.p, 0, ctx->extSum.cap, ctx->stream)); }
+    ctx->sumEpoch = (ctx->sumEpoch % 0x7FFFFFFEu) + 1u; ctx->p3BySummary = ctx->p3Walked = 0;
     HIPCHK(hipMemsetAsync(cnt + CNT_STATEOPS, 0, 16, ctx->stream));
     HIPCHK(hipMemsetAsync(cnt + CNT_QALIGN, 0, 4, ctx->stream));
     HIPCHK(hipMemsetAsync((unsigned long long *)ctx->rowsBound.p + nProb, 0, 8, ctx->stream));
     PhaseArgs X; X.state = ctx->rootState.as<RootState>(); X.stateOps = ctx->stateOps.as<uint32_t>(); X.stateOpsCount = cnt + CNT_STATEOPS; X.stateOpsCap = stateOpsCap;
     X.probs = ctx->extProbs.as<ExtProb>(); X.rowsBound = ctx->rowsBound.as<unsigned long long>(); X.res = ctx->extRes.as<ExtRes>(); X.extOps = nullptr; X.rootBegin = 0;
-        X.p3Order = nullptr; X.band24 = 0;
+        X.band24 = 0;
+    X.stateSum = ctx->stateSum.as<yd_u32x4>(); X.extSum = ctx->extSum.as<yd_u32x4>(); X.sumTag = ctx->sumEpoch; X.p3Summary = ctx->p3Summary; X.p3Count = nullptr;
     TRACE("lanes: ensure");
     X.slowList = ctx->slowList.as<uint32_t>(); X.slowCount = cnt + CNT_SLOW; X.useList = 1;
     EV0(T_P1);
@@ -206,6 +210,7 @@
     for (size_t c = 0; c < nRanges; c++) {
         const uint32_t r0 = cuts[c], r1 = cuts[c + 1], p0 = 2 * r0, np = 2 * (r1 - r0);
         E.probs = ctx->extProbs.as<ExtProb>() + p0; E.nProb = np; E.res = ctx->extRes.as<ExtRes>() + p0;
+        E.sum = ctx->extSum.as<yd_u32x4>() + 2 * (size_t)p0; E.sumTag = ctx->sumEpoch;
         E.queue = cc + 8 * c;
         HIPCHK(hipMemsetAsync(ctx->traceCnt.p, 0, 4, ctx->stream));
         HIPCHK(hipMemsetAsync(E.res, 0, sizeof(ExtRes) * (uint64_t)np, ctx->stream));
@@ -263,7 +268,7 @@
                     pp.qLen, pp.flags);
             memset(w8, 0, sizeof w8); hipMemcpyToSymbol(HIP_SYMBOL(gTraceDbg), w8, sizeof w8); } }
         AlignArgs Ac = A; Ac.nRoots = r1; Ac.queueHead = cc + 8 * c + 1;
-        PhaseArgs Xc = X; Xc.rootBegin = r0; Xc.slowList = ctx->slowList.as<uint32_t>() + r0; Xc.slowCount = cc + 8 * c + 2; Xc.useList = 1;
+        PhaseArgs Xc = X; Xc.rootBegin = r0; Xc.slowList = ctx->slowList.as<uint32_t>() + r0; Xc.slowCount = cc + 8 * c + 2; Xc.useList = 1; Xc.p3Count = cc + 8 * c + 6;
         if (c == 0) { ctx->evUsed[T_P3] = true; hipEventRecord(ctx->ev[T_P3][0], ctx->stream); }
         const uint32_t nr = r1 - r0, cap2 = nr / 4 + 1024;
         if (ctx->splitLanes) {
@@ -274,29 +279,20 @@
                 Xc.rowsBound2 = ctx->rowsBound2.as<unsigned long long>();
             Xc.nProb2 = cc + 8 * c + 3; Xc.probs2Cap = cap2;
         } else { Xc.memoKeys = nullptr; Xc.memoCount = nullptr; Xc.probs2 = nullptr; Xc.rowsBound2 = nullptr; Xc.nProb2 = nullptr; Xc.probs2Cap = 0; }
-        {
-            static const bool p3Sort = getenv("YGPU_P3_SORT") && atoi(getenv("YGPU_P3_SORT")) != 0;
-            Xc.p3Order = nullptr;
-            if (p3Sort && nr > 4096u) {
-                uint32_t *kk = ctx->extKeys.as<uint32_t>() + p0, *oo = ctx->extVals.as<uint32_t>() + p0;
-                KL(k_p3_keys, dim3(gridFor(nr, 256)), dim3(256), 0, ctx->stream, Xc, r1, kk);
-                rc = bucketOrder(ctx, kk, nullptr, r0, nr, 0, 0, 4096u, oo, ctx->stream); if (rc) return rc;
-                Xc.p3Order = oo;
-            }
-        }
         KL(k_p3_lanes, dim3(gridFor(nr, YD_P3_BS)), dim3(YD_P3_BS), 0, ctx->stream, Ac, Xc);
         if (ctx->splitLanes) KL(k_p3_predict, dim3((unsigned)std::min<uint64_t>(gridFor(nr, 64), (uint64_t)ctx->nCU * 8)), dim3(64), 0, ctx->stream, Ac, Xc);
         PhaseArgs Xw = Xc;
-        unsigned int used[2] = {0, 0}; uint32_t three[3] = {0, 0, 0};
+        unsigned int used[2] = {0, 0}; uint32_t three[6] = {0, 0, 0, 0, 0, 0};
         HIPCHK(hipMemcpyAsync(used, ctx->traceCnt.p, 8, hipMemcpyDeviceToHost, ctx->stream));
-        if (ctx->splitLanes) HIPCHK(hipMemcpyAsync(three, cc + 8 * c + 2, 8, hipMemcpyDeviceToHost, ctx->stream));
+        HIPCHK(hipMemcpyAsync(three, cc + 8 * c + 2, 24, hipMemcpyDeviceToHost, ctx->stream));
         HIPCHK(streamSync(ctx));
         usedChunksMax = std::max<unsigned long long>(usedChunksMax, used[0]);
+        ctx->p3BySummary += three[4]; ctx->p3Walked += three[5];
         if (ctx->splitLanes) {
             const uint32_t nSlow = three[0], n2 = std::min(three[1], cap2);
             if (kTrace) fprintf(stderr, "[ygpu] range %zu: chunks used %u, ext ops %u; split roots %u, careful extensions listed %u\n", c, used[0], used[1], nSlow, n2);
             if (nSlow) {
-                ExtArgs E2 = E;
+                ExtArgs E2 = E; E2.sum = nullptr;
                 if (n2) {
                     E2.probs = ctx->probs2.as<ExtProb>(); E2.nProb = n2;
                     HIPCHK(hipMemsetAsync(ctx->extRes2.p, 0, sizeof(ExtRes) * (uint64_t)n2, ctx->stream));
@@ -538,7 +534,7 @@
         E.order = nullptr; E.clock = nullptr; E.trace = ctx->extTrace.as<uint32_t>(); E.nChunks = (uint32_t)nCh; E.chunkCount = ctx->traceCnt.as<unsigned int>();
             E.waveChunks = ctx->waveChunks.as<uint32_t>(); E.maxCh = maxCh;
         E.ops = ctx->extOps.as<uint32_t>(); E.opsCount = ctx->traceCnt.as<unsigned int>() + 1; E.opsCap = (uint32_t)opsBound; E.res = ctx->extRes.as<ExtRes>();
-        E.queue = ctx->chunkCnt.as<unsigned int>(); E.ctr = nullptr; E.errFlag = ctx->errFlag.as<int>(); E.dbgMode = 0;
+        E.queue = ctx->chunkCnt.as<unsigned int>(); E.ctr = nullptr; E.errFlag = ctx->errFlag.as<int>(); E.dbgMode = 0; E.sum = nullptr; E.sumTag = 0;
         if (second) KL(rowsKernel2, dim3(blocksK), dim3(256), 0, ctx->stream, E); else KL(rowsKernel, dim3(blocksK), dim3(256), 0, ctx->stream, E);
         { const unsigned tbs = pk ? (unsigned)YD_TRACE_BS : 256u; KL(traceKernel, dim3(gridFor(nX, tbs)), dim3(tbs), 0, ctx->stream, E); }
         uint32_t ef2 = 0; rc = fetchU32(ctx, ctx->errFlag.p, &ef2); if (rc) return rc;
diff --git a/yaha_amd/csrc/p3_summary_core.h b/yaha_amd/csrc/p3_summary_core.h
--- /dev/null
+++ b/yaha_amd/csrc/p3_summary_core.h
@@ -0,0 +1,101 @@
+#pragma once
+#include <stdint.h>
+
+#if defined(__HIPCC__)
+#define YP3_FN __host__ __device__ __forceinline__
+#else
+#define YP3_FN inline
+#endif
+
+namespace yp3 {
+
+struct Scoring { int MS, RC, GO, GE; };
+enum { M = 0, R = 1, D = 2, I = 3 };
+enum { REJECT = 0, SPLIT = 1, ACCEPT = 2 };
+enum { VALID = 0x80000000u, CODE_MASK = 0x7FFF0000u };
+
+YP3_FN int code(uint32_t op) { return (int)((op & (uint32_t)CODE_MASK) >> 16); }
+YP3_FN int len(uint32_t op) { return (int)(op & 0xFFFFu); }
+YP3_FN int score(const Scoring &S, int c, int l) { return l * (c == M ? S.MS : (c == R ? -S.RC : -S.GE)) + (c >= D ? -S.GO : 0); }
+
+struct Rec { int32_t m, r, g, tot, lo, hi; uint32_t op0, tag; };
+
+struct Acc {
+    int m = 0, r = 0, g = 0, n = 0, tot = 0, e1 = 0, e2 = 0, lo = 0x7FFFFFFF, hi = (int)0x80000000; uint32_t first = 0, last = 0;
+    YP3_FN void add(const Scoring &S, int c, int l)
+    {
+        if (n >= 2) { lo = e2 < lo ? e2 : lo; hi = e2 > hi ? e2 : hi; }
+        m += c == M ? l : 0; r += c == R ? l : 0; g += c >= D ? l : 0;
+        tot += score(S, c, l); e2 = e1; e1 = tot;
+        last = ((uint32_t)c << 16) | (uint32_t)l; if (n == 0) first = last;
+        n++;
+    }
+    YP3_FN void growFirstM(const Scoring &S, int more)
+    {
+        const int l0 = len(first), l1 = (l0 + more) & 0xFFFF, d = (l1 - l0) * S.MS;
+        first = (first & 0xFFFF0000u) | (uint32_t)l1; m += l1 - l0; tot += d; e1 += d;
+        if (n >= 2) e2 += d; else last = first;
+        if (n >= 3) { lo += d; hi += d; }
+    }
+    YP3_FN Rec extension() const { Rec o; o.m = m; o.r = r; o.g = g; o.tot = tot; o.lo = lo; o.hi = hi; o.op0 = last; o.tag = (uint32_t)VALID; return o; }
+    YP3_FN Rec list() const
+    {
+        Rec o; o.m = m; o.r = r; o.g = g; o.tot = tot; o.lo = lo; o.hi = hi; o.op0 = first; o.tag = (uint32_t)VALID | last;
+        if (n >= 2) { o.lo = e2 < lo ? e2 : lo; o.hi = e2 > hi ? e2 : hi; }
+        return o;
+    }
+};
+
+struct Verdict { int verdict, totScore, totLength, matched, mismatched, gapBases, nOps, jab, jbc; };
+
+YP3_FN Verdict compose(const Scoring &S, int aligned, int minRawScore, float minIdentity, const Rec &A, int na, const Rec &B, int nb, const Rec &C, int nc)
+{
+    const uint32_t b0 = B.op0, bL = B.tag & ~(uint32_t)VALID;
+    const int jab = (na > 0 && code(A.op0) == code(b0)) ? 1 : 0, jbc = (nc > 0 && code(C.op0) == code(bL)) ? 1 : 0;
+    const int lenA0 = jab ? len(A.op0) : 0, lenC0 = jbc ? len(C.op0) : 0;
+    int cnt[3] = {B.m, B.r, B.g};
+    int lo = 0x7FFFFFFF, hiN = (int)0x80000000;
+#define YP3_PRE(v) do { const int v_ = (v); lo = v_ < lo ? v_ : lo; hiN = v_ > hiN ? v_ : hiN; } while (0)
+    int base = 0;
+    if (na > 0) {
+        const int sA0 = score(S, code(A.op0), len(A.op0));
+        cnt[0] += A.m; cnt[1] += A.r; cnt[2] += A.g;
+        if (na >= 3) { YP3_PRE(A.lo); YP3_PRE(A.hi); }
+        if (na >= 2) YP3_PRE(A.tot - sA0);
+        if (!jab) YP3_PRE(A.tot);
+        base = jab ? A.tot - sA0 : A.tot;
+    }
+    const int cb0 = code(b0), cbL = code(bL);
+    const int l0 = (len(b0) + lenA0 + (nb == 1 ? lenC0 : 0)) & 0xFFFF, d0 = score(S, cb0, l0) - score(S, cb0, len(b0));
+    const int lL = nb == 1 ? l0 : (len(bL) + lenC0) & 0xFFFF, dL = nb == 1 ? 0 : score(S, cbL, lL) - score(S, cbL, len(bL));
+    { const int k0 = cb0 >= D ? 2 : cb0, kL = cbL >= D ? 2 : cbL;
+      cnt[k0] += l0 - len(b0) - lenA0; if (nb > 1) cnt[kL] += lL - len(bL) - lenC0; else cnt[k0] -= lenC0; }
+    if (nb >= 2) { YP3_PRE(base + d0 + B.lo); YP3_PRE(base + d0 + B.hi); }
+    base += B.tot + d0 + dL;
+    const int ncm = nc - jbc;
+    int fin = base;
+    if (nc > 0) { cnt[0] += C.m; cnt[1] += C.r; cnt[2] += C.g; }
+    if (ncm > 0) {
+        const int sC0 = score(S, code(C.op0), len(C.op0)), off = base - (jbc ? sC0 : 0);
+        YP3_PRE(base);
+        if (!jbc && nc >= 2) YP3_PRE(off + sC0);
+        if (nc >= 3) { YP3_PRE(off + C.tot - C.hi); YP3_PRE(off + C.tot - C.lo); }
+        fin = off + C.tot;
+    }
+#undef YP3_PRE
+    Verdict v; v.jab = jab; v.jbc = jbc; v.nOps = (na - jab) + nb + ncm;
+    const int matches = cnt[0], mism = cnt[1], gaps = cnt[2];
+    v.totScore = fin & 0xFFFF; v.totLength = (matches + mism + gaps) & 0xFFFF; v.matched = matches & 0xFFFF; v.mismatched = mism & 0xFFFF; v.gapBases = gaps & 0xFFFF;
+    const int loAll = fin < lo ? fin : lo;
+    int maxAGS = hiN > fin ? hiN : fin; maxAGS = maxAGS > 0 ? maxAGS : 0;
+    v.verdict = REJECT;
+    if (loAll <= 0 || hiN >= aligned) v.verdict = SPLIT;
+    else if (matches >= minRawScore && maxAGS > fin) v.verdict = SPLIT;
+    else if (matches >= minRawScore) {
+        const double percent = (double)(matches & 0xFFFF) / (double)v.totLength;
+        if (!(percent < (double)minIdentity)) v.verdict = ACCEPT;
+    }
+    return v;
+}
+
+}
```
